# lambdaclass/lambdaworks_kzg

Hardware: AMD Instinct MI355X
Metric: blob_to_kzg_commitment ops/sec (4096-elem blobs) (higher is better)
Workload: dtype u32

## Files before the change

### lambdaworks_kzg_amd/csrc/direct.hip

```cpp
#include <stdlib.h>
#include <chrono>
#include "kernels.h"
#include "knobs.h"

namespace lwk {

template <int C>
struct DirectPlan {
    static constexpr int NW = (255 + C - 1) / C;
    static constexpr int H = 1 << (C - 1);
    static constexpr int WTOP = 255 - C * (NW - 1);
    static constexpr int HTOP = 1 << WTOP;
    static constexpr size_t TOP_BASE = (size_t)(NW - 1) * kBlobElems * H;
    static constexpr size_t ENTRIES = TOP_BASE + (size_t)kBlobElems * HTOP;
};

struct DirectPlanRt {
    int c, nw, wtop;
    uint32_t h, htop;
    size_t top_base, entries;
};

static DirectPlanRt make_plan(int bits) {
    DirectPlanRt p{};
    if (bits < kDirectMinBits || bits > kDirectMaxBits) return p;
    p.c = bits;
    p.nw = (255 + bits - 1) / bits;
    p.wtop = 255 - bits * (p.nw - 1);
    p.h = 1u << (bits - 1);
    p.htop = 1u << p.wtop;
    p.top_base = (size_t)(p.nw - 1) * kBlobElems * p.h;
    p.entries = p.top_base + (size_t)kBlobElems * p.htop;
    return p;
}

template <int C>
struct PlanOf {
    __host__ __device__ static constexpr DirectPlanRt get() {
        return DirectPlanRt{C, DirectPlan<C>::NW, DirectPlan<C>::WTOP, (uint32_t)DirectPlan<C>::H, (uint32_t)DirectPlan<C>::HTOP,
                            DirectPlan<C>::TOP_BASE, DirectPlan<C>::ENTRIES};
    }
};

size_t direct_table_entries(int bits) { return make_plan(bits).entries; }
int direct_num_windows(int bits) { return make_plan(bits).nw; }


__global__ __launch_bounds__(64) void k_direct_qbase(const G1Affine *__restrict__ points, G1Affine29 *__restrict__ qbase, int C,
                                                     int NW) {
    int i = blockIdx.x * blockDim.x + threadIdx.x;
    if (i >= kBlobElems) return;
    G1Affine29 a = affine_to_29(points[i]);
    qbase[i] = a;
    G1Xyzz29 cur = G1Xyzz29::from_affine(a.x, a.y);
    for (int j = 1; j < NW; j++) {
        for (int d = 0; d < C; d++) cur = xyzz_dbl(cur);
        qbase[(size_t)j * kBlobElems + i] = xyzz29_to_affine29(cur);
    }
}


constexpr int kChunk = 64;

__global__ __launch_bounds__(256) void k_direct_build(const G1Affine29 *__restrict__ qbase_win0, G1Affine29 *__restrict__ out_win0,
                                                      size_t n_pairs, F29<2> *__restrict__ scratch, size_t n_threads, int M,
                                                      size_t row_bytes) {
    const int K = M < kChunk ? M : kChunk;
    const size_t kChunksPerPair = (size_t)(M / K);
    const size_t gid = (size_t)blockIdx.x * blockDim.x + threadIdx.x;
    const size_t n_work = n_pairs * kChunksPerPair;
    auto slot = [&](int m, int f) -> F29<2> & { return scratch[((size_t)m * 5 + f) * n_threads + gid]; };
    for (size_t w = gid; w < n_work; w += n_threads) {
        const size_t pair = w / kChunksPerPair;
        const uint32_t s0 = (uint32_t)(w % kChunksPerPair) * K + 1;
        const G1Affine29 q = qbase_win0[pair];
        G1Xyzz29 cur = G1Xyzz29::infinity();
        for (int bit = 16; bit >= 0; bit--) {
            cur = xyzz_dbl(cur);
            if ((s0 >> bit) & 1) cur = xyzz_madd(cur, q.x, q.y);
        }
        F29<2> pref = F29<2>::one();
        const F29<1> one = F29<1>::one();
        for (int m = 0; m < K; m++) {
            F29<2> t = cur.zz * cur.zzz;
            pref = (m == 0) ? t : F29<2>(pref * t);
            slot(m, 0) = cur.x * one;
            slot(m, 1) = cur.y * one;
            slot(m, 2) = cur.zz;
            slot(m, 3) = cur.zzz;
            slot(m, 4) = pref;
            if (m < K - 1) cur = xyzz_madd(cur, q.x, q.y);
        }
        F29<2> inv = f29_inv(pref);
        char *rows = (char *)out_win0 + (pair * (size_t)M + (s0 - 1)) * row_bytes;
        for (int m = K - 1; m >= 0; m--) {
            F29<2> zz = slot(m, 2), zzz = slot(m, 3);
            F29<2> tinv = (m > 0) ? F29<2>(inv * slot(m - 1, 4)) : inv;
            inv = inv * (zz * zzz);
            G1Affine29 r;
            r.x = slot(m, 0) * (tinv * zzz);
            r.y = slot(m, 1) * (tinv * zz);
            *(G1Affine29 *)(rows + (size_t)m * row_bytes) = r;
        }
    }
}

static double wall_ms() {
    return std::chrono::duration<double, std::milli>(std::chrono::steady_clock::now().time_since_epoch()).count();
}

void free_direct_table(DirectTable &t) {
    for (int j = 0; j < kDirectMaxWindows; j++)
        if (t.win[j]) {
            hipFree(t.win[j]);
            t.win[j] = nullptr;
        }
    if (t.win_dev) hipFree(t.win_dev);
    t.win_dev = nullptr;
    t.nw = 0;
    t.bytes = 0;
}

hipError_t build_direct_table(int bits, const G1Affine *points, DirectTable &t, size_t row_bytes, hipStream_t st, double *ms, bool in_place) {
    const DirectPlanRt P = make_plan(bits);
    if (!P.entries || P.nw > kDirectMaxWindows) return hipErrorInvalidValue;
    if (in_place && (t.nw != P.nw || t.bytes != P.entries * row_bytes || !t.win_dev)) return hipErrorInvalidValue;
    if (!in_place) free_direct_table(t);
    G1Affine29 *qbase = nullptr;
    F29<2> *scratch = nullptr;
    const double t0 = wall_ms();
    const size_t n_threads = bits >= 14 ? 256 * 1024 : 64 * 1024;
    hipError_t e = hipMalloc((void **)&qbase, (size_t)P.nw * kBlobElems * sizeof(G1Affine29));
    if (e == hipSuccess) e = hipMalloc((void **)&scratch, (size_t)kChunk * 5 * n_threads * sizeof(F29<2>));
    if (e == hipSuccess && !in_place) e = hipMalloc((void **)&t.win_dev, kDirectMaxWindows * sizeof(uint64_t));
    const double t1 = wall_ms();
    double malloc_ms = 0, t_last_malloc = t1;
    if (e == hipSuccess) {
        {
            ProfScope p("k_direct_qbase", st);
            hipLaunchKernelGGL(k_direct_qbase, dim3(kBlobElems / 64), dim3(64), 0, st, points, qbase, P.c, P.nw);
        }
        for (int j = 0; j < P.nw && e == hipSuccess; j++) {
            const bool top = j == P.nw - 1;
            const size_t rows = (size_t)kBlobElems * (top ? P.htop : P.h);
            if (!in_place) {
                const double a0 = wall_ms();
                e = hipMalloc(&t.win[j], rows * row_bytes);
                t_last_malloc = wall_ms();
                malloc_ms += t_last_malloc - a0;
                if (e != hipSuccess) break;
                t.bytes += rows * row_bytes;
            }
            ProfScope p("k_direct_build", st);
            hipLaunchKernelGGL(k_direct_build, dim3((unsigned)(n_threads / 256)), dim3(256), 0, st, qbase + (size_t)j * kBlobElems,
                               (G1Affine29 *)t.win[j], (size_t)kBlobElems, scratch, n_threads, (int)(top ? P.htop : P.h), row_bytes);
        }
        if (e == hipSuccess && !in_place) {
            uint64_t h[kDirectMaxWindows] = {};
            for (int j = 0; j < P.nw; j++) h[j] = (uint64_t)(uintptr_t)t.win[j];
            e = hipMemcpyAsync(t.win_dev, h, sizeof h, hipMemcpyHostToDevice, st);
        }
        const hipError_t es = hipStreamSynchronize(st);
        if (e == hipSuccess) e = es;
    }
    const double t2 = wall_ms();
    if (qbase) hipFree(qbase);
    if (scratch) hipFree(scratch);
    if (e != hipSuccess) {
        free_direct_table(t);
    } else {
        t.nw = P.nw;
    }
    if (ms) {
        ms[0] = t1 - t0;
        ms[1] = malloc_ms;
        ms[2] = t2 - t_last_malloc;
        ms[3] = wall_ms() - t2;
    }
    return e;
}


#ifndef LWK_DIR_THREADS
#define LWK_DIR_THREADS 256
#endif
constexpr int kDirThreads = LWK_DIR_THREADS;

__device__ __forceinline__ G1Xyzz29 wave_fold(const G1Xyzz29 &in, int lane, int width = 64) {
    G1Xyzz29i s = *(const G1Xyzz29i *)&in;
    for (int d = width / 2; d >= 1; d >>= 1) {
        G1Xyzz29i other;
#pragma unroll
        for (int k = 0; k < 14; k++) {
            other.x.l[k] = __shfl_down(s.x.l[k], d, 64);
            other.y.l[k] = __shfl_down(s.y.l[k], d, 64);
            other.zz.l[k] = __shfl_down(s.zz.l[k], d, 64);
            other.zzz.l[k] = __shfl_down(s.zzz.l[k], d, 64);
        }
        if (lane < d) s = xyzz_add(s, other);
    }
    return *(G1Xyzz29 *)&s;
}

template <int CT>
__global__ __launch_bounds__(kDirThreads) void k_direct_accumulate(const uint64_t *__restrict__ win_dev,
                                                                   const uint4 *__restrict__ scalars,
                                                                   G1Xyzz29 *__restrict__ partials, int scalars_per_lane,
                                                                   DirectPlanRt rt, uint32_t row_bytes,
                                                                   const uint32_t *__restrict__ redo) {
    if (redo && !redo[blockIdx.y]) return;
    const DirectPlanRt P = CT ? PlanOf<CT ? CT : 16>::get() : rt;
    const int C = P.c;
    __shared__ uint32_t limbs[8 * kDirThreads];
    __shared__ G1Xyzz29 wave_sum[kDirThreads / 64];
    __shared__ uint64_t win_base[kDirectMaxWindows];
    if (threadIdx.x < kDirectMaxWindows) win_base[threadIdx.x] = win_dev[threadIdx.x];
    __syncthreads();
    const int tid = threadIdx.x, lane = tid & 63, wave = tid >> 6;
    const size_t blob = blockIdx.y;
    const int lanes_per_blob = gridDim.x * kDirThreads;
    const int first = blockIdx.x * kDirThreads + tid;
    const uint4 *sc = scalars + blob * (size_t)kBlobElems * 2;
    const int wper = (P.nw + (int)gridDim.z - 1) / (int)gridDim.z;
    const int w_lo = (int)blockIdx.z * wper, w_hi = w_lo + wper;

    int q = 0, j = 0;
    uint32_t carry = 0, point = 0;
    auto advance = [&](bool &valid, uint32_t &neg, G1Affine29i &row) {
        valid = false;
        while (q < scalars_per_lane) {
            if (j == 0) {
                point = (uint32_t)(first + q * lanes_per_blob);
                uint4 lo = sc[2 * point], hi = sc[2 * point + 1];
                limbs[0 * kDirThreads + tid] = lo.x; limbs[1 * kDirThreads + tid] = lo.y;
                limbs[2 * kDirThreads + tid] = lo.z; limbs[3 * kDirThreads + tid] = lo.w;
                limbs[4 * kDirThreads + tid] = hi.x; limbs[5 * kDirThreads + tid] = hi.y;
                limbs[6 * kDirThreads + tid] = hi.z; limbs[7 * kDirThreads + tid] = hi.w;
                carry = 0;
            }
            const int o = j * C, limb = o >> 5, sh = o & 31;
            uint32_t v = limbs[limb * kDirThreads + tid] >> sh;
            if (sh + C > 32 && limb + 1 < 8) v |= limbs[(limb + 1) * kDirThreads + tid] << (32 - sh);
            const bool top = j == P.nw - 1;
            uint32_t raw = (v & ((top ? (1u << P.wtop) : (1u << C)) - 1u)) + carry;
            uint32_t ng = (!top && raw > P.h) ? 1u : 0u;
            uint32_t mag = ng ? (1u << C) - raw : raw;
            carry = ng;
            const char *wbase = (const char *)(uintptr_t)win_base[j];
            const size_t idx = (size_t)point * (top ? P.htop : P.h) + (mag - 1);
            j++;
            if (j == P.nw) {
                j = 0;
                q++;
            }
            const int jw = (j == 0 ? P.nw : j) - 1;
            if (mag && jw >= w_lo && jw < w_hi) {
                valid = true;
                neg = ng;
                row = *(const G1Affine29i *)(wbase + idx * row_bytes);
                return;
            }
        }
    };

    G1Xyzz29i acc = G1Xyzz29i::infinity();
    bool cv;
    uint32_t cn;
    G1Affine29i cr;
    advance(cv, cn, cr);
    while (cv) {
        const auto qy = cneg(cr.y, cn != 0);
        xyzz_madd_split(acc, cr.x, qy, [&]() { advance(cv, cn, cr); });
    }

    G1Xyzz29 s = wave_fold(*(G1Xyzz29 *)&acc, lane);
    if (lane == 0) wave_sum[wave] = s;
    __syncthreads();
    if (wave == 0) {
        G1Xyzz29 t = lane < kDirThreads / 64 ? wave_sum[lane] : G1Xyzz29::infinity();
        t = wave_fold(t, lane, kDirThreads / 64);
        if (lane == 0) partials[(blob * gridDim.z + blockIdx.z) * gridDim.x + blockIdx.x] = t;
    }
}

constexpr int kLaneWords = 56;

__global__ __launch_bounds__(kDirThreads) void k_direct_accumulate_asm(const uint64_t *__restrict__ win_dev,
                                                                       const uint4 *__restrict__ scalars,
                                                                       uint32_t *__restrict__ lane_out, uint32_t *__restrict__ redo,
                                                                       int scalars_per_lane, DirectPlanRt rt, uint32_t row_bytes) {
#if defined(__HIP_DEVICE_COMPILE__)
    const uint32_t tid = threadIdx.x;
    const uint32_t first = blockIdx.x * blockDim.x + tid;
    const uint4 *sc = scalars + (size_t)blockIdx.y * kBlobElems * 2;
    uint32_t *out = lane_out + ((size_t)blockIdx.y * gridDim.x + blockIdx.x) * (size_t)(blockDim.x * kLaneWords);
    uint32_t *flag = redo + blockIdx.y;
    const uint32_t lanes_per_blob = gridDim.x * blockDim.x;
    asm volatile(
#include "direct_asm.inc"
        :
        : "s"(win_dev), "s"(sc), "s"(out), "s"(flag), "s"(scalars_per_lane), "s"(lanes_per_blob), "s"(rt.c), "s"(rt.nw), "s"(rt.wtop),
          "s"(rt.h), "s"(rt.htop), "s"(row_bytes), "v"(first), "v"(tid)
        :
#include "direct_asm_clobbers.inc"
    );
#endif
}


#ifdef LWK_FOLD_CALL
constexpr bool kFoldInl = false;
typedef G1Xyzz29 FoldPoint;
#else
constexpr bool kFoldInl = true;
typedef G1Xyzz29i FoldPoint;
#endif

__device__ __forceinline__ FoldPoint load_lane_sum(const uint32_t *src) {
    F29<25, kFoldInl, 1> nx;
    F29<17, kFoldInl, 1> ny, zz, zzz;
    FoldPoint acc;
    const uint4 *s4 = (const uint4 *)src;
    uint32_t wds[kLaneWords];
#pragma unroll
    for (int k = 0; k < kLaneWords / 4; k++) {
        uint4 t = s4[k];
        wds[4 * k] = t.x; wds[4 * k + 1] = t.y; wds[4 * k + 2] = t.z; wds[4 * k + 3] = t.w;
    }
#pragma unroll
    for (int i = 0; i < 14; i++) {
        nx.l[i] = wds[i];
        ny.l[i] = wds[14 + i];
        zz.l[i] = wds[28 + i];
        zzz.l[i] = wds[42 + i];
    }
    const F29<1, kFoldInl> one = F29<1, kFoldInl>::one();
    const bool inf = zz.is_literal_zero();
    acc.x = neg(nx) * one;
    acc.y = neg(ny) * one;
    acc.zz = zz * one;
    acc.zzz = zzz * one;
    if (inf) acc = FoldPoint::infinity();
    return acc;
}

__global__ __launch_bounds__(64) void k_direct_fold_lanes(const uint32_t *__restrict__ lane_out, G1Xyzz29 *__restrict__ partials,
                                                          const uint32_t *__restrict__ redo, int lanes_per_block, int blocks_per_blob) {
    const int unit = blockIdx.x;
    if (redo[unit / blocks_per_blob]) return;
    const int kFoldPerThread = lanes_per_block / 64;
    __builtin_amdgcn_s_setprio(2);
    const int lane = threadIdx.x;
    const uint32_t *src = lane_out + ((size_t)unit * lanes_per_block + lane) * (size_t)kLaneWords;
    FoldPoint acc = load_lane_sum(src);
#pragma unroll 1
    for (int step = 1; step < kFoldPerThread + 6; step++) {
        FoldPoint other;
        bool take = true;
        if (step < kFoldPerThread) {
            other = load_lane_sum(src + (size_t)step * 64 * kLaneWords);
        } else {
            const int d = 32 >> (step - kFoldPerThread);
#pragma unroll
            for (int k = 0; k < 14; k++) {
                other.x.l[k] = __shfl_down(acc.x.l[k], d, 64);
                other.y.l[k] = __shfl_down(acc.y.l[k], d, 64);
                other.zz.l[k] = __shfl_down(acc.zz.l[k], d, 64);
                other.zzz.l[k] = __shfl_down(acc.zzz.l[k], d, 64);
            }
            take = lane < d;
        }
        if (take) acc = xyzz_add(acc, other);
    }
    if (lane == 0) partials[unit] = *(G1Xyzz29 *)&acc;
}

__global__ __launch_bounds__(64) void k_direct_fold_lanes_asm(const uint32_t *__restrict__ lane_out, G1Xyzz29 *__restrict__ partials,
                                                              uint32_t *__restrict__ redo, int lanes_per_block, int blocks_per_blob) {
#if defined(__HIP_DEVICE_COMPILE__)
    const uint32_t unit = blockIdx.x;
    uint32_t *flag = redo + unit / blocks_per_blob;
    if (*flag) return;
    const uint32_t *src = lane_out + (size_t)unit * lanes_per_block * kLaneWords;
    G1Xyzz29 *out = partials + unit;
    const uint32_t per = lanes_per_block / 64, lane = threadIdx.x, levels = 6;
    asm volatile(
#include "direct_fold_asm.inc"
        :
        : "s"(src), "s"(out), "s"(flag), "s"(per), "v"(lane), "s"(levels)
        :
#include "direct_fold_asm_clobbers.inc"
    );
#endif
}

__global__ __launch_bounds__(64) void k_direct_fold_lanes_asm_alone(const uint32_t *__restrict__ lane_out, G1Xyzz29 *__restrict__ partials,
                                                                    uint32_t *__restrict__ redo, int lanes_per_block, int blocks_per_blob) {
#if defined(__HIP_DEVICE_COMPILE__)
    const uint32_t unit = blockIdx.x;
    uint32_t *flag = redo + unit / blocks_per_blob;
    if (*flag) return;
    const uint32_t *src = lane_out + (size_t)unit * lanes_per_block * kLaneWords;
    G1Xyzz29 *out = partials + unit;
    const uint32_t per = lanes_per_block / 64, lane = threadIdx.x, levels = 6;
    asm volatile(
#include "direct_fold_asm.inc"
        :
        : "s"(src), "s"(out), "s"(flag), "s"(per), "v"(lane), "s"(levels)
        :
#include "direct_fold_asm_clobbers_pad.inc"
    );
#endif
}

__global__ __launch_bounds__(64) void k_direct_fold(const G1Xyzz29 *__restrict__ partials, G1Xyzz29 *__restrict__ sums,
                                                    int per_blob) {
    const size_t b = blockIdx.x;
    const int lane = threadIdx.x;
    __builtin_amdgcn_s_setprio(2);
    G1Xyzz29 s = lane < per_blob ? partials[b * per_blob + lane] : G1Xyzz29::infinity();
    s = wave_fold(s, lane);
    if (lane == 0) sums[b] = s;
}

struct CoopParams {
    uint32_t k[8];
    uint32_t pack;
    uint32_t wtop, row_bytes, n0;
    uint32_t part_words, ctr_words;
};

constexpr uint32_t kCoopUnitWords = 56;

static void coop_geometry(const DirectPlanRt &P, int rpq, uint32_t &n0, uint32_t &units, uint32_t &counters) {
    const uint32_t groups = (uint32_t)((P.nw + rpq - 1) / rpq);
    n0 = kBlobElems * groups / 16;
    units = 0;
    counters = 0;
    for (uint32_t n = n0; n > 1; n = (n + 15) / 16) {
        units += n;
        counters += (n + 15) / 16;
    }
}

__global__ __launch_bounds__(256) void k_coop_msm_asm(const uint64_t *__restrict__ win_dev, const uint4 *__restrict__ scalars,
                                                     uint32_t *__restrict__ partials, uint32_t *__restrict__ counters,
                                                     G1Xyzz29 *__restrict__ sums, uint32_t *__restrict__ redo, CoopParams prm) {
#if defined(__HIP_DEVICE_COMPILE__)
    const uint32_t blob = blockIdx.y, lane = threadIdx.x & 63;
    const uint32_t unit = blockIdx.x * 4 + __builtin_amdgcn_readfirstlane(threadIdx.x >> 6);
    const uint4 *sc = scalars + (size_t)blob * kBlobElems * 2;
    uint32_t *part = partials + (size_t)blob * prm.part_words;
    uint32_t *ctr = counters + (size_t)blob * prm.ctr_words;
    G1Xyzz29 *out = sums + blob;
    uint32_t *flag = redo + blob;
    asm volatile(
#include "coop_asm.inc"
        :
        : "s"(win_dev), "s"(sc), "s"(part), "s"(ctr), "s"(out), "s"(flag), "s"(prm.k[0]), "s"(prm.k[1]), "s"(prm.k[2]), "s"(prm.k[3]),
          "s"(prm.k[4]), "s"(prm.k[5]), "s"(prm.k[6]), "s"(prm.k[7]), "s"(prm.pack), "s"(prm.wtop), "s"(prm.row_bytes), "s"(prm.n0), "s"(unit),
          "v"(lane)
        :
#include "coop_asm_clobbers.inc"
    );
#endif
}

static int coop_max_blobs() { return knobs().coop == 0 ? 0 : knobs().coop_max; }
static int coop_rows_per_quad(int nw, size_t n_blobs) {
    const int env = knobs().coop_rpq < 0 ? 0 : knobs().coop_rpq > 32 ? 32 : knobs().coop_rpq;
    if (env) return env;
    const int groups = n_blobs >= 4 ? 1 : (int)(4 / n_blobs);
    return (nw + groups - 1) / groups;
}

static bool direct_asm_enabled() { return knobs().direct_asm; }

template <int CT>
static void launch_direct_t(const DirectPlanRt &plan, const uint64_t *table, size_t row_bytes, const uint32_t *scalars_raw,
                            G1Xyzz29 *lane_scratch, G1Xyzz29 *partials, uint32_t *redo, G1Xyzz29 *sums, size_t n_blobs, hipStream_t st,
                            int fill, uint32_t *redo_flag_out) {
    const int kFillEnv = knobs().direct_fill;
    const int kFill = kFillEnv ? kFillEnv : fill ? fill : 512;
    CoopParams prm{};
    const int rpq = coop_rows_per_quad(plan.nw, n_blobs ? n_blobs : 1);
    uint32_t units = 0, counters = 0;
    coop_geometry(plan, rpq, prm.n0, units, counters);
    const bool coop_fits = units <= (uint32_t)kBlobElems && 1 + counters <= (uint32_t)kNumBuckets + 1;
    if ((int)n_blobs <= coop_max_blobs() && !fill && coop_fits) {
        for (int j = 0; j + 1 < plan.nw; j++) {
            const int bit = plan.c * j;
            const uint64_t v = (uint64_t)(plan.h - 1) << (bit & 31);
            uint64_t carry = v;
            for (int w = bit >> 5; w < 8 && carry; w++) {
                carry += prm.k[w];
                prm.k[w] = (uint32_t)carry;
                carry >>= 32;
            }
        }
        prm.pack = (uint32_t)plan.c | ((uint32_t)plan.nw << 8) | ((uint32_t)rpq << 16) | (12u << 24);
        prm.wtop = (uint32_t)plan.wtop;
        prm.row_bytes = (uint32_t)row_bytes;
        prm.part_words = units * kCoopUnitWords;
        prm.ctr_words = counters;
        uint32_t *ctr = redo + n_blobs;
        if (redo_flag_out) {
            ProfScope p("k_coop_msm_asm", st);
            hipLaunchKernelGGL(k_coop_msm_asm, dim3(prm.n0 / 4, (unsigned)n_blobs), dim3(256), 0, st, table, (const uint4 *)scalars_raw,
                               (uint32_t *)lane_scratch, ctr, sums, redo_flag_out, prm);
            return;
        }
        hipMemsetAsync(redo, 0, n_blobs * (1 + (size_t)counters) * sizeof(uint32_t), st);
        {
            ProfScope p("k_coop_msm_asm", st);
            hipLaunchKernelGGL(k_coop_msm_asm, dim3(prm.n0 / 4, (unsigned)n_blobs), dim3(256), 0, st, table, (const uint4 *)scalars_raw,
                               (uint32_t *)lane_scratch, ctr, sums, redo, prm);
        }
        {
            ProfScope p("k_direct_redo", st);
            hipLaunchKernelGGL(k_direct_accumulate<CT>, dim3(1, (unsigned)n_blobs, 1), dim3(kDirThreads), 0, st, table,
                               (const uint4 *)scalars_raw, sums, kBlobElems / kDirThreads, plan, (uint32_t)row_bytes, (const uint32_t *)redo);
        }
        return;
    }
    int blocks_per_blob = 1, wsplit = 1;
    while (blocks_per_blob < 16 && n_blobs * blocks_per_blob < (size_t)kFill) blocks_per_blob <<= 1;
    while (wsplit < 4 && n_blobs * blocks_per_blob * wsplit * 8 <= (size_t)kFill) wsplit <<= 1;
    const int scalars_per_lane = kBlobElems / (kDirThreads * blocks_per_blob);
    const int parts = blocks_per_blob * wsplit;
    G1Xyzz29 *dest = parts == 1 ? sums : partials;
    if (direct_asm_enabled() && wsplit == 1) {
        const int threads = kDirThreads;
        hipMemsetAsync(redo, 0, n_blobs * sizeof(uint32_t), st);
        {
            ProfScope p("k_direct_accumulate_asm", st);
            hipLaunchKernelGGL(k_direct_accumulate_asm, dim3(blocks_per_blob, (unsigned)n_blobs), dim3(threads), 0, st, table,
                               (const uint4 *)scalars_raw, (uint32_t *)lane_scratch, redo, kBlobElems / (threads * blocks_per_blob), plan,
                               (uint32_t)row_bytes);
        }
        {
            ProfScope p("k_direct_fold_lanes", st);
            const int n_units = (int)n_blobs * blocks_per_blob;
            const bool fold_asm = knobs().fold_asm;
            if (fold_asm) {
                if (n_units >= 1024 && !fill)
                    hipLaunchKernelGGL(k_direct_fold_lanes_asm_alone, dim3((unsigned)n_units), dim3(64), 0, st, (const uint32_t *)lane_scratch,
                                       dest, redo, threads, blocks_per_blob);
                else
                    hipLaunchKernelGGL(k_direct_fold_lanes_asm, dim3((unsigned)n_units), dim3(64), 0, st, (const uint32_t *)lane_scratch, dest,
                                       redo, threads, blocks_per_blob);
            } else {
                hipLaunchKernelGGL(k_direct_fold_lanes, dim3((unsigned)n_units), dim3(64), 0, st, (const uint32_t *)lane_scratch, dest,
                                   (const uint32_t *)redo, threads, blocks_per_blob);
            }
        }
        {
            ProfScope p("k_direct_redo", st);
            hipLaunchKernelGGL(k_direct_accumulate<CT>, dim3(blocks_per_blob, (unsigned)n_blobs, 1), dim3(kDirThreads), 0, st, table,
                               (const uint4 *)scalars_raw, dest, scalars_per_lane, plan, (uint32_t)row_bytes, (const uint32_t *)redo);
        }
    } else {
        ProfScope p("k_direct_accumulate", st);
        hipLaunchKernelGGL(k_direct_accumulate<CT>, dim3(blocks_per_blob, (unsigned)n_blobs, wsplit), dim3(kDirThreads), 0, st,
                           table, (const uint4 *)scalars_raw, dest, scalars_per_lane, plan, (uint32_t)row_bytes, (const uint32_t *)nullptr);
    }
    if (parts > 1) {
        ProfScope p("k_direct_fold", st);
        hipLaunchKernelGGL(k_direct_fold, dim3((unsigned)n_blobs), dim3(64), 0, st, partials, sums, parts);
    }
}

void launch_direct_msm(int bits, const uint64_t *table, size_t row_bytes, const uint32_t *scalars_raw, G1Xyzz29 *lane_scratch,
                       G1Xyzz29 *partials, uint32_t *redo, G1Xyzz29 *sums, size_t n_blobs, hipStream_t st, int fill, uint32_t *redo_flag_out) {
    const DirectPlanRt plan = make_plan(bits);
    if (!plan.entries) return;
    switch (bits) {
        case 14: launch_direct_t<14>(plan, table, row_bytes, scalars_raw, lane_scratch, partials, redo, sums, n_blobs, st, fill, redo_flag_out); break;
        case 15: launch_direct_t<15>(plan, table, row_bytes, scalars_raw, lane_scratch, partials, redo, sums, n_blobs, st, fill, redo_flag_out); break;
        case 16: launch_direct_t<16>(plan, table, row_bytes, scalars_raw, lane_scratch, partials, redo, sums, n_blobs, st, fill, redo_flag_out); break;
        default: launch_direct_t<0>(plan, table, row_bytes, scalars_raw, lane_scratch, partials, redo, sums, n_blobs, st, fill, redo_flag_out); break;
    }
}
uint32_t direct_one_blob_counter_words(int bits) {
    const DirectPlanRt plan = make_plan(bits);
    if (!plan.entries || coop_max_blobs() < 1) return 0;
    CoopParams prm{};
    uint32_t units = 0, counters = 0;
    coop_geometry(plan, coop_rows_per_quad(plan.nw, 1), prm.n0, units, counters);
    if (!(units <= (uint32_t)kBlobElems && 1 + counters <= (uint32_t)kNumBuckets + 1)) return 0;
    return counters;
}
template <int CT>
static void launch_direct_only_t(const DirectPlanRt &plan, const uint64_t *table, size_t row_bytes, const uint32_t *scalars_raw, G1Xyzz29 *sums,
                                 const uint32_t *only_if, size_t n_blobs, hipStream_t st) {
    ProfScope p("k_direct_redo", st);
    hipLaunchKernelGGL(k_direct_accumulate<CT>, dim3(1, (unsigned)n_blobs, 1), dim3(kDirThreads), 0, st, table, (const uint4 *)scalars_raw, sums,
                       kBlobElems / kDirThreads, plan, (uint32_t)row_bytes, only_if);
}

void launch_direct_msm_only(int bits, const uint64_t *table, size_t row_bytes, const uint32_t *scalars_raw, G1Xyzz29 *sums, const uint32_t *only_if,
                            size_t n_blobs, hipStream_t st) {
    const DirectPlanRt plan = make_plan(bits);
    if (!plan.entries) return;
    switch (bits) {
        case 14: launch_direct_only_t<14>(plan, table, row_bytes, scalars_raw, sums, only_if, n_blobs, st); break;
        case 15: launch_direct_only_t<15>(plan, table, row_bytes, scalars_raw, sums, only_if, n_blobs, st); break;
        case 16: launch_direct_only_t<16>(plan, table, row_bytes, scalars_raw, sums, only_if, n_blobs, st); break;
        default: launch_direct_only_t<0>(plan, table, row_bytes, scalars_raw, sums, only_if, n_blobs, st); break;
    }
}

}
```

### lambdaworks_kzg_amd/csrc/engine.h

```cpp
#pragma once
#include <hip/hip_runtime.h>
#include <atomic>
#include <condition_variable>
#include <deque>
#include <functional>
#include <mutex>
#include <string>
#include <thread>
#include <vector>
#include "../../include/lambdaworks_kzg_amd.h"
#include "kernels.h"
#include "front.h"

namespace lwk {

constexpr uint64_t kCtxMagic = 0x4c574b5a47414d44ull;
constexpr size_t kMaxChunk = 1024;
static_assert(kMaxChunk == kPlanMaxChunk, "plan.h plans in the engine's chunks");
constexpr int kMaxSplit = 8;

void set_error(const char *fmt, ...);
const char *get_error();

#define LWK_HIP(expr)                                                                         \
    do {                                                                                      \
        hipError_t _e = (expr);                                                               \
        if (_e != hipSuccess) {                                                               \
            lwk::set_error("%s failed: %s (%s:%d)", #expr, hipGetErrorString(_e), __FILE__, __LINE__); \
            return C_KZG_ERROR;                                                               \
        }                                                                                     \
    } while (0)

struct SideWorker;
SideWorker *side_worker_acquire();
void side_worker_run(SideWorker *w, std::function<void()> fn);
void side_worker_wait(SideWorker *w);
bool side_workers_on();
struct SideTask {
    SideWorker *w = nullptr;
    std::thread t;
    SideTask() = default;
    template <class F>
    explicit SideTask(F &&f) { start(static_cast<F &&>(f)); }
    template <class F>
    void start(F &&f) {
        join();
        if (!side_workers_on()) {
            try {
                t = std::thread(f);
            } catch (...) {
                f();
            }
            return;
        }
        w = side_worker_acquire();
        if (w) side_worker_run(w, std::function<void()>(f));
        else f();
    }
    void join() {
        if (w) side_worker_wait(w);
        w = nullptr;
        if (t.joinable()) t.join();
    }
    ~SideTask() { join(); }
    SideTask(const SideTask &) = delete;
    SideTask &operator=(const SideTask &) = delete;
};

struct Workspace {
    size_t cap = 0;
    uint8_t *blobs = nullptr;
    uint32_t *scalars = nullptr;
    uint32_t *scalars2 = nullptr;
    Fr *fr = nullptr;
    uint32_t *sorted = nullptr;
    uint32_t *bucket_start = nullptr;
    uint32_t *perm = nullptr;
    G1Xyzz29 *buckets = nullptr;
    G1Xyzz29 *sums = nullptr;
    uint8_t *out48 = nullptr;
    uint8_t *comm48 = nullptr;
    uint8_t *canon48 = nullptr;
    uint8_t *zbytes = nullptr;
    uint8_t *ybytes = nullptr;
    Fr *z = nullptr;
    int32_t *status = nullptr;
    G1Affine29 *val_pts = nullptr;
    int32_t *val_kind = nullptr;
    uint32_t *val_verdict = nullptr;
    size_t long_cap = 0;
    Fr *z_long = nullptr;
    uint8_t *canon_long = nullptr;
    int32_t *status_long = nullptr;
    G1Affine29 *val_pts_long = nullptr;
    int32_t *val_kind_long = nullptr;
    uint32_t *val_verdict_long = nullptr;
};

constexpr size_t kVerifyApartMax = 8192;
struct VerifyBuffers {
    G1Affine29 *pts_c = nullptr, *pts_p = nullptr;
    G1Affine29 *mult_c = nullptr, *mult_p = nullptr;
    int32_t *kind_c = nullptr, *kind_p = nullptr;
    uint8_t *proof_in = nullptr;
    uint8_t *comm_in = nullptr, *canon_dev = nullptr;
    int32_t *status_all = nullptr;
    uint32_t *verdict_c = nullptr, *verdict_p = nullptr;
    uint8_t *d_r = nullptr, *d_rz = nullptr, *d_aff = nullptr;
    G1Xyzz29 *d_part = nullptr;
    int32_t *d_inf = nullptr;
    uint8_t *vm_base = nullptr;
    G1Affine29 *tab_p = nullptr, *tab_c = nullptr;
    G1Xyzz29 *vm_tmp = nullptr, *vm_partial = nullptr, *vm_bsum = nullptr;
    F29<2> *vm_pre = nullptr;
    uint32_t *sc_a = nullptr, *sc_b = nullptr;
    Fr *vm_pw = nullptr;
    uint8_t *d_rec = nullptr;
    uint8_t *h_rec = nullptr;
    size_t rec_cap = 0;
    uint8_t *h_pin = nullptr;
    hipEvent_t vm_done = nullptr;
    std::vector<G1Affine29> h_aff;
    std::vector<int32_t> h_kind;
    std::unique_lock<std::mutex> hold;
    bool owned = false;
};
void verify_buffers_free(VerifyBuffers &v);

size_t host_small_batch_limit();
int64_t host_last_active_ns();
int64_t host_now_ns();
void host_pool_warm();

constexpr int kCombineLanes = 2;
constexpr size_t kCombineSlots = 128;
constexpr size_t kCombineMaxBatch = 64;

struct CombineReq {
    enum State { QUEUED, TAKEN, DONE };
    int slot = -1;
    int mode = 0;
    uint8_t *out48 = nullptr;
    int rc = C_KZG_OK;
    State state = QUEUED;
};

struct Combiner {
    LaneFront<CombineReq, kCombineLanes> front;
    std::mutex init_m;
    uint8_t *pinned_blobs = nullptr;
    uint8_t *pinned_out[kCombineLanes] = {nullptr, nullptr};
    int32_t *pinned_status[kCombineLanes] = {nullptr, nullptr};
    bool ready = false, failed = false;
};

struct ProofReq {
    enum State { QUEUED, TAKEN, DONE };
    const uint8_t *blob = nullptr, *second = nullptr;
    uint8_t *out = nullptr, *y_out = nullptr;
    int mode = 0;
    int rc = C_KZG_OK;
    State state = QUEUED;
};
typedef LeaderFront<ProofReq> ProofFront;

struct BuildTiming {
    int bits = 0;
    size_t row_bytes = 0, table_bytes = 0;
    double free_old_ms = 0, table_malloc_ms = 0, scratch_malloc_ms = 0, kernels_ms = 0, scratch_free_ms = 0, total_ms = 0;
    bool in_place = false;
};
struct LoadTiming {
    double context_ms = 0;
    double points_and_tables_ms = 0;
    double g2_and_fft_ms = 0;
    double default_table_ms = 0;
    double total_ms = 0;
};

struct SmallProofHost {
    uint8_t *blobs = nullptr, *comm = nullptr, *canon = nullptr, *dig = nullptr;
    int32_t *code = nullptr;
    size_t cap = 0;
    static constexpr int kChunks = 16;
    hipEvent_t chunk_done[kChunks] = {};
    hipEvent_t hashed[kChunks] = {};
};

struct LagrangeForm {
    bool ready = false;
    G1Affine *points = nullptr;
    G1Affine29 *table = nullptr;
    G1Affine29 *direct_table = nullptr;
    DirectTable direct_tab;
    int direct_bits = 0;
    size_t direct_row_bytes = 0;
};

struct DevStage {
    uint8_t *slot[2] = {nullptr, nullptr};
    hipEvent_t copied[2] = {nullptr, nullptr}, parsed[2] = {nullptr, nullptr};
    bool ready = false, failed = false;
};

struct Ctx {
    FFTSettings fs;
    uint64_t magic;
    uint64_t generation = 0;
    int device;
    hipStream_t stream;
    hipStream_t vstream;
    hipStream_t aux[kMaxSplit];
    hipEvent_t ev_fork, ev_join[kMaxSplit];
    hipEvent_t ws_done;
    hipStream_t ws_last;
    std::atomic<bool> ws_recorded{false};
    hipEvent_t lane_done[kCombineLanes];
    Combiner comb;
    ProofFront blob_proof_front, point_proof_front;
    std::atomic<Ctx *> twin{nullptr};
    bool is_twin = false;
    std::atomic<bool> reserved{false};
    Ctx *primary = nullptr;
    hipEvent_t heavy_done = nullptr;
    std::mutex heavy_mu;
    G1Affine *points;
    G1Affine29 *table;
    G1Affine29 *direct_table;
    DirectTable direct_tab;
    int direct_bits;
    size_t direct_row_bytes;
    LagrangeForm lag;
    std::atomic<bool> lag_ready{false};
    bool lag_failed = false;
    Fr *tw_fwd, *tw_inv;
    Fr28 *tw28_fwd, *tw28_inv;
    Workspace ws;
    SmallProofHost sph;
    DevStage stage;
    uint8_t *one_pin = nullptr;
    hipStream_t prio_copy = nullptr;
    uint8_t *vblobs = nullptr;
    size_t vblobs_cap = 0;
    uint8_t *host_res = nullptr;
    size_t host_res_cap = 0;
    void *each_lines = nullptr;
    uint8_t *each_buf = nullptr;
    size_t each_cap = 0;
    VerifyBuffers vs;
    size_t vs_cap;
    std::mutex verify_mu;
    std::mutex mu;
    std::atomic<int> mode_override{-1};
    BuildTiming last_build;
    LoadTiming load_timing;
};

struct WsUse {
    Ctx *c;
    hipStream_t st;
    WsUse(Ctx *c_, hipStream_t st_) : c(c_), st(st_) {
        if (c->ws_last != st) hipStreamWaitEvent(st, c->ws_done, 0);
        for (int k = 0; k < kCombineLanes; k++) hipStreamWaitEvent(st, c->lane_done[k], 0);
    }
    ~WsUse() {
        hipEventRecord(c->ws_done, st);
        c->ws_last = st;
        c->ws_recorded.store(true, std::memory_order_release);
    }
};

Ctx *ctx_of(const KZGSettings *s);
bool ctx_is_live(const Ctx *c, uint64_t gen);

int mode_of(const KZGSettings *s);

C_KZG_RET ctx_reserve(Ctx *c, size_t n);
C_KZG_RET map_rc(C_KZG_RET rc, int mode);
void ensure_lagrange(Ctx *c, int mode);

void msm_stages(Ctx *c, const uint32_t *scalars_raw, uint8_t *out48, size_t n, hipStream_t st, size_t base = 0, bool shared_chip = false,
                bool lagrange = false);
bool coefficients_to_msm_form(Ctx *c, int mode, size_t n, hipStream_t st, size_t base = 0);

C_KZG_RET commit_batch_device(Ctx *c, uint8_t *out48, const uint8_t *blobs, size_t n, int mode, hipStream_t st,
                              int32_t *status);
C_KZG_RET blob_proof_batch_device(Ctx *c, uint8_t *out48, const uint8_t *blobs, const uint8_t *comm48, size_t n, int mode,
                                  hipStream_t st, int32_t *status);
C_KZG_RET point_proof_batch_device(Ctx *c, uint8_t *proof48, uint8_t *y32, const uint8_t *blobs, const uint8_t *z32,
                                   size_t n, int mode, hipStream_t st, int32_t *status, const G1Xyzz29 **sums_out = nullptr);
C_KZG_RET msm_scalars_raw_device(Ctx *c, uint8_t *out48, const uint32_t *scalars_raw, size_t n, hipStream_t st);

C_KZG_RET verify_prepare_host(Ctx *c, const uint8_t *blobs, const uint8_t *comm48, const uint8_t *proofs48, size_t n,
                              int mode, uint8_t *z32, uint8_t *y32, uint8_t *canon_c, uint8_t *canon_p, VerifyBuffers &vb,
                              const uint8_t *trusted_canon_c = nullptr);
C_KZG_RET verify_prepare_device(Ctx *c, const uint8_t *d_blobs, const uint8_t *d_comm, const uint8_t *d_proofs, size_t n, int mode,
                                uint8_t *z32, uint8_t *y32, uint8_t *canon_c, uint8_t *canon_p, VerifyBuffers &vb, hipStream_t caller,
                                uint8_t *records_out = nullptr, bool keep = false);
C_KZG_RET verify_openings_prepare_device(Ctx *c, const uint8_t *d_comm, const uint8_t *d_proofs, const uint8_t *d_z, const uint8_t *d_y,
                                         size_t n, int mode, VerifyBuffers &vb);
C_KZG_RET lincomb3_device_host(Ctx *c, VerifyBuffers &vb, const uint8_t *sc_r, const uint8_t *sc_rz, size_t n,
                               uint8_t sums[3][96], int infs[3]);
bool vmsm_ready(const VerifyBuffers &vb);
C_KZG_RET vmsm_begin(Ctx *c, VerifyBuffers &vb, const Fr *pw33, int le, size_t n);
C_KZG_RET vmsm_finish(Ctx *c, VerifyBuffers &vb, uint8_t sums[3][96], int infs[3]);

int host_validate_commitment(const uint8_t in48[48], uint8_t canon48[48], G1Affine29 *aff = nullptr);
void host_validate_commitments(const uint8_t *in48, uint8_t *canon48, int *rc, size_t n, G1Affine29 *aff = nullptr);

bool g2_fill_values(g2_t *out65, const uint8_t *g2_bytes, size_t n2);

}
```

### lambdaworks_kzg_amd/csrc/engine.hip

```cpp
#include "engine.h"
#include "knobs.h"
#include "hostfp.h"

#include <stdarg.h>
#include <stdio.h>
#include <stdlib.h>
#include <string.h>

#include <atomic>
#include <chrono>
#include <map>
#include <set>
#include <thread>
#include <vector>

namespace lwk {


static thread_local char g_err[512] = "";

void set_error(const char *fmt, ...) {
    va_list ap;
    va_start(ap, fmt);
    vsnprintf(g_err, sizeof g_err, fmt, ap);
    va_end(ap);
    if (knobs().verbose) fprintf(stderr, "[lambdaworks_kzg_amd] %s\n", g_err);
}
const char *get_error() { return g_err; }


struct ProfRec {
    const char *name;
    hipEvent_t e0, e1;
};
static std::atomic<bool> g_prof_on{false};
static std::mutex g_prof_mu;
static std::vector<ProfRec> g_prof_pending;
struct ProfAgg {
    uint64_t launches = 0;
    double total_ms = 0;
};
static std::map<std::string, ProfAgg> g_prof_agg;

ProfScope::ProfScope(const char *n, hipStream_t s) : name(n), st(s), e0(nullptr), e1(nullptr), on(g_prof_on.load(std::memory_order_relaxed)) {
    if (!on) return;
    if (hipEventCreate(&e0) != hipSuccess || hipEventCreate(&e1) != hipSuccess) {
        on = false;
        return;
    }
    hipEventRecord(e0, st);
}
ProfScope::~ProfScope() {
    if (!on) return;
    hipEventRecord(e1, st);
    std::lock_guard<std::mutex> lk(g_prof_mu);
    g_prof_pending.push_back({name, e0, e1});
}

static void prof_drain() {
    std::lock_guard<std::mutex> lk(g_prof_mu);
    for (auto &r : g_prof_pending) {
        float ms = 0;
        if (hipEventSynchronize(r.e1) == hipSuccess && hipEventElapsedTime(&ms, r.e0, r.e1) == hipSuccess) {
            auto &a = g_prof_agg[r.name];
            a.launches++;
            a.total_ms += ms;
        }
        hipEventDestroy(r.e0);
        hipEventDestroy(r.e1);
    }
    g_prof_pending.clear();
}


static std::mutex g_reg_mu;
struct RegEntry {
    Ctx *ctx;
    uint64_t digest;
};
static std::map<const void *, RegEntry> g_registry;
static std::set<const void *> g_live_fs;
static std::atomic<int> g_default_device{0};
thread_local int tl_device_override = -1;

static uint64_t g1_values_digest(const g1_t *g1) {
    uint64_t h = 0xcbf29ce484222325ull;
    const uint8_t *a = (const uint8_t *)&g1[0], *b = (const uint8_t *)&g1[kBlobElems - 1];
    for (size_t i = 0; i < sizeof(g1_t); i++) h = (h ^ a[i]) * 0x100000001b3ull;
    for (size_t i = 0; i < sizeof(g1_t); i++) h = (h ^ b[i]) * 0x100000001b3ull;
    return h;
}

static bool peer_busy(const Ctx *c) {
    const Ctx *p = c->is_twin ? c->primary : c->primary->twin.load(std::memory_order_acquire);
    if (!p || !p->ws_recorded.load(std::memory_order_acquire)) return false;
    const bool busy = hipEventQuery(p->ws_done) != hipSuccess;
    (void)hipGetLastError();
    return busy;
}

struct WsLaneUse {
    Ctx *c;
    int lane;
    WsLaneUse(Ctx *c_, int lane_) : c(c_), lane(lane_) { hipStreamWaitEvent(c->aux[lane], c->ws_done, 0); }
    ~WsLaneUse() {
        hipEventRecord(c->lane_done[lane], c->aux[lane]);
        c->ws_last = nullptr;
    }
};

static C_KZG_RET dev_alloc(void **p, size_t bytes) {
    LWK_HIP(hipMalloc(p, bytes));
    return C_KZG_OK;
}

template <class T>
static void dev_free(T *&p) {
    if (p) hipFree(p);
    p = nullptr;
}

static void ws_free(Workspace &w) {
    dev_free(w.blobs);
    dev_free(w.scalars);
    dev_free(w.scalars2);
    dev_free(w.fr);
    dev_free(w.sorted);
    dev_free(w.bucket_start);
    dev_free(w.perm);
    dev_free(w.buckets);
    dev_free(w.sums);
    dev_free(w.out48);
    dev_free(w.comm48);
    dev_free(w.canon48);
    dev_free(w.zbytes);
    dev_free(w.ybytes);
    dev_free(w.z);
    dev_free(w.status);
    dev_free(w.val_pts);
    dev_free(w.val_kind);
    dev_free(w.val_verdict);
    w.cap = 0;
}

static void ws_long_free(Workspace &w) {
    dev_free(w.z_long);
    dev_free(w.canon_long);
    dev_free(w.status_long);
    w.long_cap = 0;
    dev_free(w.val_pts_long);
    dev_free(w.val_kind_long);
    dev_free(w.val_verdict_long);
}

C_KZG_RET ctx_reserve(Ctx *c, size_t n) {
    if (n > kMaxChunk) n = kMaxChunk;
    if (n == 0) n = 1;
    Workspace &w = c->ws;
    if (w.cap >= n) return C_KZG_OK;
    LWK_HIP(hipSetDevice(c->device));
    LWK_HIP(hipDeviceSynchronize());
    ws_free(w);
    size_t cap = 1;
    while (cap < n) cap <<= 1;
    C_KZG_RET rc;
#define WS_ALLOC(field, bytes)                                  \
    if ((rc = dev_alloc((void **)&w.field, (bytes))) != C_KZG_OK) { \
        ws_free(w);                                             \
        return C_KZG_MALLOC;                                    \
    }
    WS_ALLOC(blobs, cap * (size_t)kBlobBytes);
    WS_ALLOC(scalars, cap * (size_t)kBlobBytes);
    WS_ALLOC(scalars2, cap * (size_t)kBlobBytes);
    WS_ALLOC(fr, cap * (size_t)kBlobBytes);
    WS_ALLOC(sorted, cap * (size_t)kMaxEntries * 4);
    WS_ALLOC(bucket_start, cap * (size_t)(kNumBuckets + 1) * 4);
    WS_ALLOC(perm, cap * (size_t)(kNumBuckets + 1) * 4);
    WS_ALLOC(buckets, cap * (size_t)kNumBuckets * sizeof(G1Xyzz29));
    WS_ALLOC(sums, (cap + 1) * sizeof(G1Xyzz29));
    WS_ALLOC(out48, cap * 48);
    WS_ALLOC(comm48, cap * 48);
    WS_ALLOC(canon48, cap * 48);
    WS_ALLOC(zbytes, cap * 32);
    WS_ALLOC(ybytes, cap * 32);
    WS_ALLOC(z, cap * sizeof(Fr));
    WS_ALLOC(status, cap * 4);
    WS_ALLOC(val_pts, cap * sizeof(G1Affine29));
    WS_ALLOC(val_kind, cap * 4);
    WS_ALLOC(val_verdict, cap * 4);
#undef WS_ALLOC
    w.cap = cap;
    return C_KZG_OK;
}

static void vs_free(Ctx *c);
void direct_from_env(const KZGSettings *s);

static void sph_free(SmallProofHost &h) {
    if (h.blobs) hipHostFree(h.blobs);
    if (h.comm) hipHostFree(h.comm);
    if (h.canon) hipHostFree(h.canon);
    if (h.dig) hipHostFree(h.dig);
    if (h.code) hipHostFree(h.code);
    for (hipEvent_t e : h.chunk_done)
        if (e) hipEventDestroy(e);
    for (hipEvent_t e : h.hashed)
        if (e) hipEventDestroy(e);
    h = SmallProofHost();
}

static std::atomic<int> g_last_proof_schedule{-1};
static size_t small_proof_host_limit() {
    const size_t x = knobs().small_proof_host;
    return x > kMaxChunk ? kMaxChunk : x;
}

static bool sph_reserve(Ctx *c, size_t n, bool at_reserve = false) {
    SmallProofHost &h = c->sph;
    if (h.cap >= n) return true;
    if (!at_reserve && c->primary->reserved.load(std::memory_order_acquire)) return false;
    hipDeviceSynchronize();
    sph_free(h);
    size_t cap = 16;
    while (cap < n) cap <<= 1;
    const bool ok = hipHostMalloc((void **)&h.blobs, cap * (size_t)kBlobBytes) == hipSuccess && hipHostMalloc((void **)&h.comm, cap * 48) == hipSuccess &&
                    hipHostMalloc((void **)&h.canon, cap * 48) == hipSuccess && hipHostMalloc((void **)&h.dig, cap * 32) == hipSuccess &&
                    hipHostMalloc((void **)&h.code, cap * 4) == hipSuccess;
    bool ev_ok = ok;
    for (int k = 0; ev_ok && k < SmallProofHost::kChunks; k++)
        ev_ok = hipEventCreateWithFlags(&h.chunk_done[k], hipEventDisableTiming) == hipSuccess &&
                hipEventCreateWithFlags(&h.hashed[k], hipEventDisableTiming) == hipSuccess;
    if (!ev_ok) {
        (void)hipGetLastError();
        sph_free(h);
        return false;
    }
    h.cap = cap;
    return true;
}

static size_t mid_proof_chunks() {
    const size_t x = knobs().mid_proof_chunks;
    return x < 1 ? 1 : x > (size_t)SmallProofHost::kChunks ? (size_t)SmallProofHost::kChunks : x;
}
static size_t mid_proof_host_limit() {
    const size_t x = knobs().mid_proof_host;
    return x > kMaxChunk ? kMaxChunk : x;
}

static PlanKnobs plan_knobs() {
    PlanKnobs k;
    k.small_proof_host = small_proof_host_limit();
    k.mid_proof_host = mid_proof_host_limit();
    k.mid_proof_chunks = mid_proof_chunks();
    k.mid_proof_pipe = knobs().mid_proof_pipe;
    k.mid_proof_pipe_min = knobs().mid_proof_pipe_min;
    k.mid_proof_parts = knobs().mid_proof_parts;
    k.heavy_serial = knobs().heavy_serial;
    return k;
}

static std::atomic<int64_t> g_wake_requested_ns{0};
static void host_warm_fn(void *);
static bool host_assist_warm() {
    const int64_t window_ns = (int64_t)(knobs().host_warm_ms < 0 ? 0 : knobs().host_warm_ms) * 1000000;
    const int64_t last = host_last_active_ns(), woken = g_wake_requested_ns.load(std::memory_order_acquire), now = host_now_ns();
    return (last != 0 && now - last <= window_ns) || (woken != 0 && now - woken <= window_ns);
}
static void launch_host_wake(Ctx *c) {
    g_wake_requested_ns.store(host_now_ns(), std::memory_order_release);
    if (hipLaunchHostFunc(c->aux[1], host_warm_fn, nullptr) != hipSuccess) (void)hipGetLastError();
}
static void host_warm_fn(void *) {
    try {
        host_pool_warm();
    } catch (...) {
    }
}

struct ChunkHashArgs {
    SmallProofHost *h;
    size_t first, count;
};
static void chunk_midstate_host_fn(void *p) {
    ChunkHashArgs *a = (ChunkHashArgs *)p;
    SmallProofHost &h = *a->h;
    try {
        challenge_midstates_host((uint32_t *)(h.dig + 32 * a->first), h.blobs + a->first * (size_t)kBlobBytes, a->count);
    } catch (...) {
        memset(h.dig + 32 * a->first, 0, 32 * a->count);
    }
    delete a;
}
static void chunk_hash_host_fn(void *p) {
    ChunkHashArgs *a = (ChunkHashArgs *)p;
    SmallProofHost &h = *a->h;
    try {
        challenge_digests_host(h.dig + 32 * a->first, h.blobs + a->first * (size_t)kBlobBytes, h.comm + 48 * a->first, a->count);
    } catch (...) {
        memset(h.dig + 32 * a->first, 0, 32 * a->count);
    }
    delete a;
}

static C_KZG_RET chunk_host_functions(Ctx *c, const uint8_t *blobs, size_t n, hipStream_t sc, hipStream_t sf, hipStream_t join,
                                      void (*fn)(void *), const char *prof_name, bool record_hashed = false) {
    SmallProofHost &h = c->sph;
    const size_t per = (n + mid_proof_chunks() - 1) / mid_proof_chunks();
    std::vector<ChunkHashArgs *> args;
    for (size_t first = 0; first < n; first += per) {
        ChunkHashArgs *a = new (std::nothrow) ChunkHashArgs{&h, first, n - first < per ? n - first : per};
        if (!a) {
            for (ChunkHashArgs *b : args) delete b;
            return C_KZG_MALLOC;
        }
        args.push_back(a);
    }
    for (size_t k = 0; k < args.size(); k++) {
        const size_t first = args[k]->first, cnt = args[k]->count;
        hipError_t e = hipMemcpyAsync(h.blobs + first * (size_t)kBlobBytes, blobs + first * (size_t)kBlobBytes, cnt * (size_t)kBlobBytes,
                                      hipMemcpyDeviceToHost, sc);
        if (e == hipSuccess) e = hipEventRecord(h.chunk_done[k], sc);
        if (e == hipSuccess) e = hipStreamWaitEvent(sf, h.chunk_done[k], 0);
        bool queued = false;
        if (e == hipSuccess) {
            ProfScope p(prof_name, sf);
            e = hipLaunchHostFunc(sf, fn, args[k]);
            queued = e == hipSuccess;
        }
        if (e == hipSuccess && record_hashed) e = hipEventRecord(h.hashed[k], sf);
        if (e != hipSuccess) {
            for (size_t j = queued ? k + 1 : k; j < args.size(); j++) delete args[j];
            set_error("host-assisted challenge: %s", hipGetErrorString(e));
            (void)hipGetLastError();
            if (hipEventRecord(c->ev_join[kMaxSplit - 2], sc) == hipSuccess) hipStreamWaitEvent(join, c->ev_join[kMaxSplit - 2], 0);
            if (sf != join && hipEventRecord(c->ev_join[kMaxSplit - 3], sf) == hipSuccess) hipStreamWaitEvent(join, c->ev_join[kMaxSplit - 3], 0);
            return C_KZG_ERROR;
        }
    }
    return C_KZG_OK;
}

struct SmallProofArgs {
    SmallProofHost *h;
    size_t n;
    int32_t bad;
};

static void small_proof_host_fn(void *p) {
    SmallProofArgs *a = (SmallProofArgs *)p;
    SmallProofHost &h = *a->h;
    try {
        challenge_digests_host(h.dig, h.blobs, h.comm, a->n);
        std::vector<int> vrc(a->n);
        host_validate_commitments(h.comm, h.canon, vrc.data(), a->n);
        for (size_t i = 0; i < a->n; i++) h.code[i] = vrc[i] == 2 ? a->bad : 0;
    } catch (...) {
        for (size_t i = 0; i < a->n; i++) h.code[i] = kStatusError;
    }
    delete a;
}


static void ctx_destroy(Ctx *c) {
    if (!c) return;
    hipSetDevice(c->device);
    hipDeviceSynchronize();
    if (Ctx *t = c->twin.load(std::memory_order_acquire)) {
        ctx_destroy(t);
        c->twin.store(nullptr, std::memory_order_release);
    }
    ws_free(c->ws);
// ... 6 lines not shown
        c->direct_tab = DirectTable();
        c->lag = LagrangeForm();
        c->tw_fwd = c->tw_inv = nullptr;
        c->tw28_fwd = c->tw28_inv = nullptr;
    }
    dev_free(c->points);
    dev_free(c->table);
    free_direct_table(c->direct_tab);
    c->direct_table = nullptr;
    free_direct_table(c->lag.direct_tab);
    dev_free(c->lag.points);
    dev_free(c->lag.table);
    dev_free(c->tw_fwd);
    dev_free(c->tw_inv);
    dev_free(c->tw28_fwd);
    dev_free(c->tw28_inv);
    if (c->stream) hipStreamDestroy(c->stream);
    if (c->vstream) hipStreamDestroy(c->vstream);
    for (int k = 0; k < kMaxSplit; k++) {
        if (c->aux[k]) hipStreamDestroy(c->aux[k]);
        if (c->ev_join[k]) hipEventDestroy(c->ev_join[k]);
    }
    if (c->ev_fork) hipEventDestroy(c->ev_fork);
    if (c->ws_done) hipEventDestroy(c->ws_done);
    if (c->heavy_done) hipEventDestroy(c->heavy_done);
    for (int k = 0; k < kCombineLanes; k++) {
        if (c->lane_done[k]) hipEventDestroy(c->lane_done[k]);
        if (c->comb.pinned_out[k]) hipHostFree(c->comb.pinned_out[k]);
        if (c->comb.pinned_status[k]) hipHostFree(c->comb.pinned_status[k]);
    }
    if (c->comb.pinned_blobs) hipHostFree(c->comb.pinned_blobs);
    dev_free(c->host_res);
    dev_free(c->vblobs);
    dev_free(c->each_lines);
    dev_free(c->each_buf);
    if (c->prio_copy) hipStreamDestroy(c->prio_copy);
    if (c->one_pin) hipHostFree(c->one_pin);
    for (int k = 0; k < 2; k++) {
        dev_free(c->stage.slot[k]);
        if (c->stage.copied[k]) hipEventDestroy(c->stage.copied[k]);
        if (c->stage.parsed[k]) hipEventDestroy(c->stage.parsed[k]);
    }
    sph_free(c->sph);
    free(c->fs.expanded_roots_of_unity);
    free(c->fs.reverse_roots_of_unity);
    free(c->fs.roots_of_unity);
    c->magic = 0;
    {
        std::lock_guard<std::mutex> lk(g_reg_mu);
        g_live_fs.erase((const void *)c);
    }
    delete c;
}

static bool gpu_available() {
    int n = 0;
    if (hipGetDeviceCount(&n) != hipSuccess || n <= 0) {
        set_error("no HIP device available: this library has no CPU fallback (hipGetDeviceCount)");
        return false;
    }
    return true;
}

static void fr_raw_to_blst(blst_fr *o, const uint32_t raw[8]) {
    for (int k = 0; k < 4; k++) o->l[3 - k] = (uint64_t)raw[2 * k] | ((uint64_t)raw[2 * k + 1] << 32);
}

static C_KZG_RET ctx_new(Ctx **out, const Ctx *twin_of = nullptr) {
    if (!gpu_available()) return C_KZG_ERROR;
    Ctx *c = new Ctx();
    memset(&c->fs, 0, sizeof c->fs);
    c->magic = kCtxMagic;
    c->device = twin_of ? twin_of->device : tl_device_override >= 0 ? tl_device_override : g_default_device.load();
    c->is_twin = twin_of != nullptr;
    c->primary = twin_of ? const_cast<Ctx *>(twin_of) : c;
    c->stream = nullptr;
    c->ws_done = nullptr;
    c->ws_last = nullptr;
    for (int k = 0; k < kCombineLanes; k++) c->lane_done[k] = nullptr;
    c->vstream = nullptr;
    c->ev_fork = nullptr;
    for (int k = 0; k < kMaxSplit; k++) {
        c->aux[k] = nullptr;
        c->ev_join[k] = nullptr;
    }
    c->points = nullptr;
    c->table = nullptr;
    c->direct_table = nullptr;
    c->direct_bits = 0;
    c->direct_row_bytes = kDirectRowPacked;
    c->vs_cap = 0;
    c->tw_fwd = c->tw_inv = nullptr;
    c->tw28_fwd = c->tw28_inv = nullptr;
    hipError_t e = hipSetDevice(c->device);
    if (e == hipSuccess) e = hipStreamCreate(&c->stream);
    if (e == hipSuccess) e = hipStreamCreateWithFlags(&c->vstream, hipStreamNonBlocking);
    if (e == hipSuccess) e = hipEventCreateWithFlags(&c->ev_fork, hipEventDisableTiming);
    if (e == hipSuccess) e = hipEventCreateWithFlags(&c->ws_done, hipEventDisableTiming);
    if (e == hipSuccess && !twin_of) e = hipEventCreateWithFlags(&c->heavy_done, hipEventDisableTiming);
    for (int k = 0; k < kCombineLanes && e == hipSuccess; k++) e = hipEventCreateWithFlags(&c->lane_done[k], hipEventDisableTiming);
    for (int k = 0; k < kMaxSplit && e == hipSuccess; k++) {
        e = hipStreamCreateWithFlags(&c->aux[k], hipStreamNonBlocking);
        if (e == hipSuccess) e = hipEventCreateWithFlags(&c->ev_join[k], hipEventDisableTiming);
    }
    if (twin_of) {
        c->points = twin_of->points;
        c->table = twin_of->table;
        c->direct_table = twin_of->direct_table;
        c->direct_tab.win_dev = twin_of->direct_tab.win_dev;
        c->direct_bits = twin_of->direct_bits;
        c->direct_row_bytes = twin_of->direct_row_bytes;
        c->lag = twin_of->lag;
        c->lag.direct_tab = DirectTable();
        c->lag.direct_tab.win_dev = twin_of->lag.direct_tab.win_dev;
        c->tw_fwd = twin_of->tw_fwd;
        c->tw_inv = twin_of->tw_inv;
        c->tw28_fwd = twin_of->tw28_fwd;
        c->tw28_inv = twin_of->tw28_inv;
    } else {
        if (e == hipSuccess) e = hipMalloc((void **)&c->points, (size_t)kBlobElems * sizeof(G1Affine));
        if (e == hipSuccess) e = hipMalloc((void **)&c->table, (size_t)kTablePoints * sizeof(G1Affine29));
        if (e == hipSuccess) e = hipMalloc((void **)&c->tw_fwd, (size_t)(kBlobElems / 2) * sizeof(Fr));
        if (e == hipSuccess) e = hipMalloc((void **)&c->tw_inv, (size_t)(kBlobElems / 2) * sizeof(Fr));
        if (e == hipSuccess) e = hipMalloc((void **)&c->tw28_fwd, (size_t)(kBlobElems / 2 + kBlobElems) * sizeof(Fr28));
        if (e == hipSuccess) e = hipMalloc((void **)&c->tw28_inv, (size_t)(kBlobElems / 2) * sizeof(Fr28));
    }
    if (e != hipSuccess) {
        set_error("device context allocation failed: %s", hipGetErrorString(e));
        ctx_destroy(c);
        return C_KZG_MALLOC;
    }
    static std::atomic<uint64_t> next_generation{1};
    c->generation = next_generation.fetch_add(1);
    if (!twin_of) {
        std::lock_guard<std::mutex> lk(g_reg_mu);
        g_live_fs.insert((const void *)c);
    }
    *out = c;
    return C_KZG_OK;
}

static bool twin_off() {
    return !knobs().twin;
}

static Ctx *pick_ctx(Ctx *c, hipStream_t st) {
    if (twin_off() || !st || st == c->stream) return c;
    std::lock_guard<std::mutex> lk(c->mu);
    if (c->ws_last == st || c->ws_last == nullptr || hipEventQuery(c->ws_done) == hipSuccess) {
        (void)hipGetLastError();
        return c;
    }
    (void)hipGetLastError();
    if (!c->twin.load(std::memory_order_acquire)) {
        Ctx *t = nullptr;
        if (ctx_new(&t, c) != C_KZG_OK) return c;
        c->twin.store(t, std::memory_order_release);
    }
    return c->twin.load(std::memory_order_acquire);
}

static C_KZG_RET ctx_finish_fft(Ctx *c) {
    launch_build_twiddles(c->tw_fwd, c->tw_inv, c->stream);
    launch_twiddles_to28(c->tw_fwd, c->tw28_fwd, c->stream);
    launch_twiddles_to28(c->tw_inv, c->tw28_inv, c->stream);
    launch_roots_brp28(c->tw28_fwd, c->tw28_fwd + kBlobElems / 2, c->stream);
    const int n = kBlobElems;
    std::vector<Fr> h_f(n / 2), h_i(n / 2);
    LWK_HIP(hipMemcpyAsync(h_f.data(), c->tw_fwd, (n / 2) * sizeof(Fr), hipMemcpyDeviceToHost, c->stream));
    LWK_HIP(hipMemcpyAsync(h_i.data(), c->tw_inv, (n / 2) * sizeof(Fr), hipMemcpyDeviceToHost, c->stream));
    LWK_HIP(hipStreamSynchronize(c->stream));
    c->fs.max_width = n;
    c->fs.expanded_roots_of_unity = (fr_t *)calloc(n + 1, sizeof(fr_t));
    c->fs.reverse_roots_of_unity = (fr_t *)calloc(n + 1, sizeof(fr_t));
    c->fs.roots_of_unity = (fr_t *)calloc(n, sizeof(fr_t));
    if (!c->fs.expanded_roots_of_unity || !c->fs.reverse_roots_of_unity || !c->fs.roots_of_unity) return C_KZG_MALLOC;
    for (int k = 0; k <= n; k++) {
        int kk = k % n;
        Fr f = h_f[kk % (n / 2)], b = h_i[kk % (n / 2)];
        if (kk >= n / 2) {
            f = neg(f);
            b = neg(b);
        }
        uint32_t raw[8];
        fe_to_raw<FrParams>(raw, f);
        fr_raw_to_blst(&c->fs.expanded_roots_of_unity[k], raw);
        fe_to_raw<FrParams>(raw, b);
        fr_raw_to_blst(&c->fs.reverse_roots_of_unity[k], raw);
    }
    for (int k = 0; k < n; k++) {
        unsigned r = 0;
        for (int b = 0; b < 12; b++) r |= ((k >> b) & 1u) << (11 - b);
        c->fs.roots_of_unity[k] = c->fs.expanded_roots_of_unity[r];
    }
    return C_KZG_OK;
}

bool ctx_is_live(const Ctx *c, uint64_t gen) {
    std::lock_guard<std::mutex> lk(g_reg_mu);
    return c && g_live_fs.count((const void *)c) && c->generation == gen;
}

Ctx *ctx_of(const KZGSettings *s) {
    if (!s) {
        set_error("KZGSettings pointer is NULL");
        return nullptr;
    }
    if (s->fs) {
        std::lock_guard<std::mutex> lk(g_reg_mu);
        if (g_live_fs.count((const void *)s->fs)) return (Ctx *)s->fs;
    }
    if (!s->g1_values) {
        set_error("KZGSettings has neither an engine context nor g1_values");
        return nullptr;
    }
    const uint64_t digest = g1_values_digest(s->g1_values);
    Ctx *stale = nullptr;
    {
        std::lock_guard<std::mutex> lk(g_reg_mu);
        auto it = g_registry.find(s->g1_values);
        if (it != g_registry.end()) {
            if (it->second.digest == digest) return it->second.ctx;
            stale = it->second.ctx;
            g_registry.erase(it);
        }
    }
    if (stale) ctx_destroy(stale);
    Ctx *c = nullptr;
    if (ctx_new(&c) != C_KZG_OK) return nullptr;
    uint64_t *d_blst = nullptr;
    int32_t *d_status = nullptr;
    std::vector<int32_t> h_status(kBlobElems);
    bool ok = hipMalloc((void **)&d_blst, (size_t)kBlobElems * 144) == hipSuccess &&
              hipMalloc((void **)&d_status, (size_t)kBlobElems * 4) == hipSuccess &&
              hipMemcpyAsync(d_blst, s->g1_values, (size_t)kBlobElems * 144, hipMemcpyHostToDevice, c->stream) == hipSuccess;
    if (ok) {
        launch_g1_from_blst(d_blst, c->points, d_status, kBlobElems, c->stream);
        launch_build_table(c->points, c->table, c->stream);
        ok = hipMemcpyAsync(h_status.data(), d_status, (size_t)kBlobElems * 4, hipMemcpyDeviceToHost, c->stream) == hipSuccess &&
             hipStreamSynchronize(c->stream) == hipSuccess;
    }
    if (d_blst) hipFree(d_blst);
    if (d_status) hipFree(d_status);
    if (ok)
        for (int i = 0; i < kBlobElems; i++)
            if (h_status[i] != 0) {
                set_error("g1_values[%d] is not a point on the curve", i);
                ok = false;
                break;
            }
    if (ok) ok = ctx_finish_fft(c) == C_KZG_OK;
    if (!ok) {
        if (!get_error()[0]) set_error("building a device context from g1_values failed");
        ctx_destroy(c);
        return nullptr;
    }
    bool ours = true;
    {
        std::lock_guard<std::mutex> lk(g_reg_mu);
        auto it = g_registry.find(s->g1_values);
        if (it != g_registry.end()) {
            Ctx *first = it->second.ctx;
            if (it->second.digest == digest) {
                stale = c;
                c = first;
                ours = false;
            } else {
                stale = first;
                it->second = {c, digest};
            }
        } else {
            stale = nullptr;
            g_registry[s->g1_values] = {c, digest};
        }
    }
    if (stale) ctx_destroy(stale);
    if (ours) direct_from_env(s);
    return c;
}


static G1Xyzz29 *msm_sums_stage(Ctx *c, const uint32_t *scalars_raw, size_t n, hipStream_t st, size_t base = 0, bool shared_chip = false,
                                bool lagrange = false, G1Xyzz29 *sums_out = nullptr, uint32_t *redo_flag_out = nullptr) {
    Workspace &w = c->ws;
    uint32_t *sorted = w.sorted + base * (size_t)kMaxEntries;
    uint32_t *bstart = w.bucket_start + base * (size_t)(kNumBuckets + 1);
    uint32_t *perm = w.perm + base * (size_t)(kNumBuckets + 1);
    G1Xyzz29 *buckets = w.buckets + base * (size_t)kNumBuckets;
    G1Xyzz29 *sums = sums_out ? sums_out : w.sums + base;
    const G1Affine29 *direct = lagrange ? c->lag.direct_table : c->direct_table;
    if (direct) {
        launch_direct_msm(lagrange ? c->lag.direct_bits : c->direct_bits, lagrange ? c->lag.direct_tab.win_dev : c->direct_tab.win_dev,
                          lagrange ? c->lag.direct_row_bytes : c->direct_row_bytes, scalars_raw, buckets, (G1Xyzz29 *)sorted, bstart, sums, n,
                          st, (shared_chip || peer_busy(c)) ? 2048 : 0, redo_flag_out);
        return sums;
    }
    launch_digit_sort(scalars_raw, sorted, bstart, perm, n, st);
    launch_bucket_accumulate(lagrange ? c->lag.table : c->table, sorted, bstart, perm, buckets, n, st);
    launch_bucket_reduce(buckets, sums, n, st);
    return sums;
}

void msm_stages(Ctx *c, const uint32_t *scalars_raw, uint8_t *out48, size_t n, hipStream_t st, size_t base, bool shared_chip,
                bool lagrange) {
    launch_finalize_compress(msm_sums_stage(c, scalars_raw, n, st, base, shared_chip, lagrange), out48, n, st);
}

static size_t host_finish_limit() {
    const size_t x = knobs().host_finish;
    return x > kCombineMaxBatch ? kCombineMaxBatch : x;
}

static HFp hfp_from_limbs28(const uint32_t *l) {
    uint64_t w[7] = {0, 0, 0, 0, 0, 0, 0};
    for (int i = 0; i < 14; i++) {
        const int bit = P29::W * i, k = bit >> 6, sh = bit & 63;
        unsigned __int128 v = (unsigned __int128)l[i] << sh;
        for (int j = k; j < 7 && v; j++) {
            v += w[j];
            w[j] = (uint64_t)v;
            v >>= 64;
        }
    }
    for (int shift = 16; shift >= 0; shift--) {
        uint64_t kp[7], d[7];
        for (int j = 0; j < 7; j++) {
            const uint64_t lo = j < 6 ? HFpPar::P[j] : 0, below = j > 0 ? HFpPar::P[j - 1] : 0;
            kp[j] = shift ? (lo << shift) | (below >> (64 - shift)) : lo;
        }
        unsigned __int128 br = 0;
        for (int j = 0; j < 7; j++) {
            const unsigned __int128 v = (unsigned __int128)w[j] - kp[j] - (uint64_t)br;
            d[j] = (uint64_t)v;
            br = (v >> 64) & 1;
        }
        if (!br)
            for (int j = 0; j < 7; j++) w[j] = d[j];
    }
    HFp r;
    for (int j = 0; j < 6; j++) r.l[j] = w[j];
    return r;
}

static void host_finish_compress(uint8_t out[48], const G1Xyzz29 &sum) {
    if (sum.is_inf()) {
        memset(out, 0, 48);
        out[0] = 0xc0;
        return;
    }
    const HFp X = hfp_from_limbs28(sum.x.l), Y = hfp_from_limbs28(sum.y.l), ZZ = hfp_from_limbs28(sum.zz.l), ZZZ = hfp_from_limbs28(sum.zzz.l);
    const HFp i = inv(ZZ * ZZZ);
    G1Affine a;
    a.x = (X * (i * ZZZ)).to_fe();
    a.y = (Y * (i * ZZ)).to_fe();
    g1_compress_affine(out, a);
}

static bool commit_on_lagrange(const Ctx *c, int mode) {
    return mode == LWKZG_MODE_CKZG && c->lag.ready && (c->lag.direct_table || !c->direct_table);
}
static bool proof_on_lagrange(const Ctx *c, int mode) {
    return mode == LWKZG_MODE_CKZG && c->lag.ready && c->lag.direct_table && !c->direct_table;
}
static bool proof_in_evaluation_form(const Ctx *c, int mode) {
    return knobs().ckzg_eval_proofs && mode == LWKZG_MODE_CKZG && c->lag.ready && (c->lag.direct_table || !c->direct_table);
}
static void quotient_stage(Ctx *c, int mode, const uint32_t *in, const Fr *z, uint32_t *quot, uint8_t *y_out, int le, size_t n, hipStream_t st,
                           const uint32_t *only_if = nullptr) {
    if (proof_in_evaluation_form(c, mode)) launch_eval_quotient_evalform(in, z, c->tw28_fwd + kBlobElems / 2, quot, y_out, le, n, st, only_if);
    else launch_eval_quotient(in, z, quot, y_out, le, n, st, only_if);
}
static bool quotient_to_msm_form(Ctx *c, int mode, size_t n, hipStream_t st, size_t base = 0) {
    if (proof_in_evaluation_form(c, mode)) return true;
    return coefficients_to_msm_form(c, mode, n, st, base);
}
bool coefficients_to_msm_form(Ctx *c, int mode, size_t n, hipStream_t st, size_t base) {
    if (!proof_on_lagrange(c, mode)) return false;
    Workspace &w = c->ws;
    const size_t so = base * (size_t)kBlobElems;
    launch_coefficients_to_evaluations(w.scalars2 + so * 8, w.fr + so, (Fr *)(w.scalars + so * 8), c->tw28_fwd, n, st);
    return true;
}

static bool coefficients_stage(Ctx *c, const uint8_t *blobs, size_t n, int mode, int32_t *status, hipStream_t st,
                               size_t base = 0, bool evaluations_ok = false, uint32_t *zero = nullptr, uint32_t zero_words = 0) {
    Workspace &w = c->ws;
    uint32_t *scalars = w.scalars + base * (size_t)kBlobElems * 8;
    if (mode == LWKZG_MODE_REFERENCE) {
        launch_parse_be_reduce(blobs, scalars, n * kBlobElems, st, zero, zero_words);
    } else if (evaluations_ok ? commit_on_lagrange(c, mode) : proof_in_evaluation_form(c, mode)) {
        launch_copy_le_check(blobs, scalars, status, n, st);
        return true;
    } else {
        launch_blob_evaluations_to_coefficients(blobs, scalars, c->tw28_inv, status, n, st);
    }
    return false;
}

static int split_ways(bool direct) {
    const int v = knobs().split < 0 ? 0 : knobs().split > kMaxSplit ? kMaxSplit : knobs().split;
    return v ? v : (direct ? 1 : 2);
}

C_KZG_RET msm_scalars_raw_device(Ctx *c, uint8_t *out48, const uint32_t *scalars_raw, size_t n, hipStream_t st) {
    for (size_t off = 0; off < n; off += kMaxChunk) {
        size_t m = n - off < kMaxChunk ? n - off : kMaxChunk;
        msm_stages(c, scalars_raw + off * (size_t)kBlobElems * 8, out48 + 48 * off, m, st);
    }
    return C_KZG_OK;
}

C_KZG_RET commit_batch_device(Ctx *c, uint8_t *out48, const uint8_t *blobs, size_t n, int mode, hipStream_t st,
                              int32_t *status) {
    C_KZG_RET rc = ctx_reserve(c, n);
    if (rc != C_KZG_OK) return rc;
    for (size_t off = 0; off < n; off += kMaxChunk) {
        size_t m = n - off < kMaxChunk ? n - off : kMaxChunk;
        int32_t *stt = status ? status + off : c->ws.status;
        LWK_HIP(hipMemsetAsync(stt, 0, m * 4, st));
        const int ways = m >= 256 ? split_ways((commit_on_lagrange(c, mode) ? c->lag.direct_table : c->direct_table) != nullptr) : 1;
        if (ways == 1) {
            const bool lg = coefficients_stage(c, blobs + off * (size_t)kBlobBytes, m, mode, stt, st, 0, true);
            msm_stages(c, c->ws.scalars, out48 + 48 * off, m, st, 0, false, lg);
            continue;
        }
        LWK_HIP(hipEventRecord(c->ev_fork, st));
        for (int k = 0; k < ways; k++) {
            size_t lo = m * k / ways, hi = m * (k + 1) / ways;
            hipStream_t sk = c->aux[k];
            LWK_HIP(hipStreamWaitEvent(sk, c->ev_fork, 0));
            const bool lg = coefficients_stage(c, blobs + (off + lo) * (size_t)kBlobBytes, hi - lo, mode, stt + lo, sk, lo, true);
            msm_stages(c, c->ws.scalars + lo * (size_t)kBlobElems * 8, out48 + 48 * (off + lo), hi - lo, sk, lo, false, lg);
            LWK_HIP(hipEventRecord(c->ev_join[k], sk));
            LWK_HIP(hipStreamWaitEvent(st, c->ev_join[k], 0));
        }
    }
    return C_KZG_OK;
}

static C_KZG_RET ws_long_reserve(Ctx *c, size_t n) {
    Workspace &w = c->ws;
    if (w.long_cap >= n) return C_KZG_OK;
    LWK_HIP(hipDeviceSynchronize());
    ws_long_free(w);
    size_t cap = 2 * kMaxChunk;
    while (cap < n) cap <<= 1;
    if (hipMalloc((void **)&w.z_long, cap * sizeof(Fr)) != hipSuccess || hipMalloc((void **)&w.canon_long, cap * 48) != hipSuccess ||
        hipMalloc((void **)&w.status_long, cap * 4) != hipSuccess || hipMalloc((void **)&w.val_pts_long, cap * sizeof(G1Affine29)) != hipSuccess ||
        hipMalloc((void **)&w.val_kind_long, cap * 4) != hipSuccess || hipMalloc((void **)&w.val_verdict_long, cap * 4) != hipSuccess) {
        (void)hipGetLastError();
        ws_long_free(w);
        set_error("proof batch of %zu blobs: out of device memory for the challenges", n);
        return C_KZG_MALLOC;
    }
    w.long_cap = cap;
    return C_KZG_OK;
}

C_KZG_RET blob_proof_batch_device(Ctx *c, uint8_t *out48, const uint8_t *blobs, const uint8_t *comm48, size_t n, int mode,
                                  hipStream_t st, int32_t *status) {
    C_KZG_RET rc = ctx_reserve(c, n);
    if (rc != C_KZG_OK) return rc;
    const bool longcall = n > kMaxChunk;
    if (longcall) {
        rc = ws_long_reserve(c, n);
        if (rc != C_KZG_OK) return rc;
    }
    Workspace &w = c->ws;
    const int le = mode == LWKZG_MODE_CKZG;
    int32_t *stt = status ? status : longcall ? w.status_long : w.status;
    Fr *z = longcall ? w.z_long : w.z;
    uint8_t *canon = longcall ? w.canon_long : w.canon48;
    LWK_HIP(hipMemsetAsync(stt, 0, n * 4, st));
    const bool evf = proof_in_evaluation_form(c, mode);
    const bool msm_direct = evf ? c->lag.direct_table != nullptr : c->direct_table && !proof_on_lagrange(c, mode);
    const bool warm = host_assist_warm(), busy = peer_busy(c);
    const PlanKnobs pk = plan_knobs();
    ProofPlan plan = plan_proof_call(n, warm, busy, msm_direct, true, pk);
    const int forced = knobs().proof_schedule;
    if (forced >= 0 && forced <= kProofGpuChains && n <= kMaxChunk) {
        PlanKnobs fk = pk;
        fk.small_proof_host = forced == kProofSmallHost ? kMaxChunk : 0;
        fk.mid_proof_host = forced == kProofSmallHost || forced == kProofGpuChains ? 0 : kMaxChunk;
        fk.mid_proof_pipe = forced == kProofMidPiped;
        fk.mid_proof_pipe_min = 0;
        plan = plan_proof_call(n, forced != kProofMidCold, false, forced == kProofMidPiped ? msm_direct : false, true, fk);
    }
    SmallProofArgs *host_args = nullptr;
    if (plan.needs_staging()) {
        bool ok = sph_reserve(c, n);
        if (ok && plan.schedule == kProofSmallHost) {
            host_args = new (std::nothrow) SmallProofArgs{&c->sph, n, le ? kStatusBadArgs : kStatusError};
            ok = host_args != nullptr;
        }
        if (!ok) plan = plan_proof_call(n, warm, busy, msm_direct, false, pk);
    }
    g_last_proof_schedule.store((int)plan.schedule, std::memory_order_relaxed);
    const bool piped = plan.schedule == kProofMidPiped;
    switch (plan.schedule) {
    case kProofSmallHost: {
        SmallProofHost &h = c->sph;
        LWK_HIP(hipMemcpyAsync(h.blobs, blobs, n * (size_t)kBlobBytes, hipMemcpyDeviceToHost, st));
        LWK_HIP(hipMemcpyAsync(h.comm, comm48, n * 48, hipMemcpyDeviceToHost, st));
        {
            ProfScope p("host_challenge_and_validate", st);
            hipError_t e = hipLaunchHostFunc(st, small_proof_host_fn, host_args);
            if (e != hipSuccess) {
                delete host_args;
                set_error("hipLaunchHostFunc failed: %s", hipGetErrorString(e));
                return C_KZG_ERROR;
            }
        }
        LWK_HIP(hipMemcpyAsync(stt, h.code, n * 4, hipMemcpyHostToDevice, st));
        LWK_HIP(hipMemcpyAsync(w.zbytes, h.dig, n * 32, hipMemcpyHostToDevice, st));
        LWK_HIP(hipMemcpyAsync(canon, h.canon, n * 48, hipMemcpyHostToDevice, st));
        launch_z_from_bytes(w.zbytes, z, nullptr, le, n, st);
        launch_challenge(blobs, canon, z, le, n, st, comm48);
        break;
    }
    case kProofMidCold: {
        LWK_HIP(hipEventRecord(c->ev_fork, st));
        LWK_HIP(hipStreamWaitEvent(c->vstream, c->ev_fork, 0));
        launch_validate_commitments(comm48, canon, stt, le ? kStatusBadArgs : kStatusError, n, c->vstream, longcall ? w.val_pts_long : w.val_pts,
                                    longcall ? w.val_kind_long : w.val_kind, longcall ? w.val_verdict_long : w.val_verdict);
        LWK_HIP(hipEventRecord(c->ev_join[0], c->vstream));
        launch_host_wake(c);
        launch_challenge(blobs, comm48, z, le, n, st);
        LWK_HIP(hipStreamWaitEvent(st, c->ev_join[0], 0));
        launch_challenge(blobs, canon, z, le, n, st, comm48);
        break;
    }
    case kProofMidHost:
    case kProofMidPiped: {
        SmallProofHost &h = c->sph;
        hipStream_t sc = c->aux[0], sh = c->aux[1];
        const size_t chunks = plan.chunks;
        LWK_HIP(hipEventRecord(c->ev_fork, st));
        LWK_HIP(hipStreamWaitEvent(c->vstream, c->ev_fork, 0));
        LWK_HIP(hipStreamWaitEvent(sc, c->ev_fork, 0));
        if (piped) LWK_HIP(hipStreamWaitEvent(sh, c->ev_fork, 0));
        launch_validate_commitments(comm48, canon, stt, le ? kStatusBadArgs : kStatusError, n, c->vstream, longcall ? w.val_pts_long : w.val_pts,
                                    longcall ? w.val_kind_long : w.val_kind, longcall ? w.val_verdict_long : w.val_verdict);
        LWK_HIP(hipEventRecord(c->ev_join[0], c->vstream));
        LWK_HIP(hipMemcpyAsync(h.comm, comm48, n * 48, hipMemcpyDeviceToHost, sc));
        {
            const C_KZG_RET rch = chunk_host_functions(c, blobs, n, sc, piped ? sh : st, st, chunk_hash_host_fn, "host_challenge_chunk", piped);
            if (rch != C_KZG_OK) {
                hipStreamWaitEvent(st, c->ev_join[0], 0);
                return rch;
            }
        }
        if (piped) {
            const size_t per = plan.per_chunk;
            const size_t parts = plan.parts;
            const size_t cps = chunks / parts;
            uint32_t *differs = w.perm;
            hipStream_t s2 = c->aux[2];
            LWK_HIP(hipStreamWaitEvent(s2, c->ev_fork, 0));
            for (size_t j = 0; j < parts; j++) {
                const size_t off = j * cps * per, end_ = (j + 1) * cps * per < n ? (j + 1) * cps * per : n;
                if (off >= end_) continue;
                const size_t m = end_ - off;
                hipStream_t sk = (j & 1) ? s2 : st;
                LWK_HIP(hipStreamWaitEvent(sk, h.hashed[(j + 1) * cps - 1], 0));
                LWK_HIP(hipMemcpyAsync(w.zbytes + 32 * off, h.dig + 32 * off, m * 32, hipMemcpyHostToDevice, sk));
                launch_z_from_bytes(w.zbytes + 32 * off, z + off, nullptr, le, m, sk);
                coefficients_stage(c, blobs + off * (size_t)kBlobBytes, m, mode, stt + off, sk, off);
                quotient_stage(c, mode, w.scalars + off * (size_t)kBlobElems * 8, z + off, w.scalars2 + off * (size_t)kBlobElems * 8, nullptr, le, m, sk);
                (void)msm_sums_stage(c, w.scalars2 + off * (size_t)kBlobElems * 8, m, sk, off, false, evf);
            }
            LWK_HIP(hipEventRecord(c->ev_join[2], s2));
            LWK_HIP(hipStreamWaitEvent(st, c->ev_join[2], 0));
            LWK_HIP(hipStreamWaitEvent(st, c->ev_join[0], 0));
            launch_flag_differs48(canon, comm48, differs, n, st);
            launch_challenge(blobs, canon, z, le, n, st, comm48);
            quotient_stage(c, mode, w.scalars, z, w.scalars2, nullptr, le, n, st, differs);
            launch_direct_msm_only(evf ? c->lag.direct_bits : c->direct_bits, evf ? c->lag.direct_tab.win_dev : c->direct_tab.win_dev,
                                   evf ? c->lag.direct_row_bytes : c->direct_row_bytes, w.scalars2, w.sums, differs, n, st);
            launch_finalize_compress(w.sums, out48, n, st);
            return C_KZG_OK;
        }
        LWK_HIP(hipMemcpyAsync(w.zbytes, h.dig, n * 32, hipMemcpyHostToDevice, st));
        launch_z_from_bytes(w.zbytes, z, nullptr, le, n, st);
        LWK_HIP(hipStreamWaitEvent(st, c->ev_join[0], 0));
        launch_challenge(blobs, canon, z, le, n, st, comm48);
        break;
    }
    case kProofGpuChains: {
        LWK_HIP(hipEventRecord(c->ev_fork, st));
        LWK_HIP(hipStreamWaitEvent(c->vstream, c->ev_fork, 0));
        launch_validate_commitments(comm48, canon, stt, le ? kStatusBadArgs : kStatusError, n, c->vstream, longcall ? w.val_pts_long : w.val_pts,
                                    longcall ? w.val_kind_long : w.val_kind, longcall ? w.val_verdict_long : w.val_verdict);
        LWK_HIP(hipEventRecord(c->ev_join[0], c->vstream));
        launch_challenge(blobs, comm48, z, le, n, st);
        LWK_HIP(hipStreamWaitEvent(st, c->ev_join[0], 0));
        launch_challenge(blobs, canon, z, le, n, st, comm48);
        break;
    }
    }
    Ctx *pr = c->primary;
    const bool heavy_serial = plan.heavy_serial;
    if (heavy_serial) {
        std::lock_guard<std::mutex> hk(pr->heavy_mu);
        LWK_HIP(hipStreamWaitEvent(st, pr->heavy_done, 0));
    }
    for (size_t off = 0; off < n; off += kMaxChunk) {
        size_t m = n - off < kMaxChunk ? n - off : kMaxChunk;
        coefficients_stage(c, blobs + off * (size_t)kBlobBytes, m, mode, stt + off, st);
        quotient_stage(c, mode, w.scalars, z + off, w.scalars2, nullptr, le, m, st);
        G1Xyzz29 *sums = msm_sums_stage(c, w.scalars2, m, st, 0, false, quotient_to_msm_form(c, mode, m, st));
        if (heavy_serial && off + kMaxChunk >= n) {
            std::lock_guard<std::mutex> hk(pr->heavy_mu);
            LWK_HIP(hipEventRecord(pr->heavy_done, st));
        }
        launch_finalize_compress(sums, out48 + 48 * off, m, st);
    }
    return C_KZG_OK;
}

C_KZG_RET commit_and_prove_batch_device(Ctx *c, uint8_t *comm_out48, uint8_t *proof_out48, const uint8_t *blobs, size_t n, int mode,
                                        hipStream_t st, int32_t *status) {
    C_KZG_RET rc = ctx_reserve(c, n);
    if (rc != C_KZG_OK) return rc;
    const bool longcall = n > kMaxChunk;
    if (longcall) {
        rc = ws_long_reserve(c, n);
        if (rc != C_KZG_OK) return rc;
    }
    Workspace &w = c->ws;
    const int le = mode == LWKZG_MODE_CKZG;
    int32_t *stt = status ? status : longcall ? w.status_long : w.status;
    Fr *z = longcall ? w.z_long : w.z;
    uint32_t *mid = (uint32_t *)(longcall ? w.canon_long : w.canon48);
    LWK_HIP(hipMemsetAsync(stt, 0, n * 4, st));
    LWK_HIP(hipEventRecord(c->ev_fork, st));
    LWK_HIP(hipStreamWaitEvent(c->vstream, c->ev_fork, 0));
    const bool host_cold = n <= mid_proof_host_limit() && !peer_busy(c) && !host_assist_warm();
    if (host_cold) launch_host_wake(c);
    const bool host_mid = !host_cold && n <= mid_proof_host_limit() && !peer_busy(c) && sph_reserve(c, n);
    if (host_mid) {
        SmallProofHost &h = c->sph;
        hipStream_t sc = c->aux[0];
        LWK_HIP(hipStreamWaitEvent(sc, c->ev_fork, 0));
        {
            const C_KZG_RET rch = chunk_host_functions(c, blobs, n, sc, c->vstream, st, chunk_midstate_host_fn, "host_midstate_chunk");
            if (rch != C_KZG_OK) return rch;
        }
        LWK_HIP(hipMemcpyAsync(mid, h.dig, n * 32, hipMemcpyHostToDevice, c->vstream));
    } else {
        launch_challenge_midstate(blobs, mid, n, c->vstream);
    }
    LWK_HIP(hipEventRecord(c->ev_join[0], c->vstream));
    for (size_t off = 0; off < n; off += kMaxChunk) {
        const size_t m = n - off < kMaxChunk ? n - off : kMaxChunk;
        const uint8_t *b = blobs + off * (size_t)kBlobBytes;
        if (coefficients_stage(c, b, m, mode, stt + off, st)) {
            msm_stages(c, w.scalars, comm_out48 + 48 * off, m, st, 0, off == 0 && !host_mid, true);
        } else if (proof_on_lagrange(c, mode)) {
            launch_copy_le_check(b, (uint32_t *)w.fr, nullptr, m, st);
            msm_stages(c, (const uint32_t *)w.fr, comm_out48 + 48 * off, m, st, 0, off == 0 && !host_mid, true);
        } else {
            msm_stages(c, w.scalars, comm_out48 + 48 * off, m, st, 0, off == 0 && !host_mid);
        }
        if (off == 0) LWK_HIP(hipStreamWaitEvent(st, c->ev_join[0], 0));
        launch_challenge_finish(b, comm_out48 + 48 * off, mid + 8 * off, z + off, le, m, st);
        quotient_stage(c, mode, w.scalars, z + off, w.scalars2, nullptr, le, m, st);
        msm_stages(c, w.scalars2, proof_out48 + 48 * off, m, st, 0, false, quotient_to_msm_form(c, mode, m, st));
    }
    return C_KZG_OK;
}

C_KZG_RET point_proof_batch_device(Ctx *c, uint8_t *proof48, uint8_t *y32, const uint8_t *blobs, const uint8_t *z32,
                                   size_t n, int mode, hipStream_t st, int32_t *status, const G1Xyzz29 **sums_out) {
    C_KZG_RET rc = ctx_reserve(c, n);
    if (rc != C_KZG_OK) return rc;
    Workspace &w = c->ws;
    const int le = mode == LWKZG_MODE_CKZG;
    for (size_t off = 0; off < n; off += kMaxChunk) {
        size_t m = n - off < kMaxChunk ? n - off : kMaxChunk;
        int32_t *stt = status ? status + off : w.status;
        LWK_HIP(hipMemsetAsync(stt, 0, m * 4, st));
        coefficients_stage(c, blobs + off * (size_t)kBlobBytes, m, mode, stt, st);
        launch_z_from_bytes(z32 + 32 * off, w.z, stt, le, m, st);
        quotient_stage(c, mode, w.scalars, w.z, w.scalars2, y32 + 32 * off, le, m, st);
        const bool lg = quotient_to_msm_form(c, mode, m, st);
        if (sums_out && n <= kMaxChunk) *sums_out = msm_sums_stage(c, w.scalars2, m, st, 0, false, lg);
        else msm_stages(c, w.scalars2, proof48 + 48 * off, m, st, 0, false, lg);
    }
    return C_KZG_OK;
}


static C_KZG_RET first_status(Ctx *c, const int32_t *d_status, size_t n, hipStream_t st) {
    std::vector<int32_t> h(n);
    LWK_HIP(hipMemcpyAsync(h.data(), d_status, n * 4, hipMemcpyDeviceToHost, st));
    LWK_HIP(hipStreamSynchronize(st));
    for (size_t i = 0; i < n; i++)
        if (h[i] != 0) {
            set_error("input %zu rejected (status %d)", i, h[i]);
            return (C_KZG_RET)h[i];
        }
    return C_KZG_OK;
}

void verify_buffers_free(VerifyBuffers &v) {
    dev_free(v.pts_c);
    dev_free(v.pts_p);
    dev_free(v.mult_c);
    dev_free(v.mult_p);
    dev_free(v.kind_c);
    dev_free(v.kind_p);
    dev_free(v.proof_in);
    dev_free(v.comm_in);
    dev_free(v.canon_dev);
    dev_free(v.status_all);
    dev_free(v.verdict_c);
    dev_free(v.verdict_p);
    dev_free(v.d_r);
    dev_free(v.d_rz);
    dev_free(v.d_aff);
    dev_free(v.d_part);
    dev_free(v.d_inf);
    dev_free(v.vm_base);
    dev_free(v.d_rec);
    if (v.h_rec) {
        (void)hipHostFree(v.h_rec);
// ... 500 lines not shown
            LWK_HIP(hipMemcpyAsync(vb.d_rz + 32 * off, w.zbytes, m * 32, hipMemcpyDeviceToDevice, st));
        LWK_HIP(hipMemcpyAsync(z32 + 32 * off, w.zbytes, m * 32, hipMemcpyDeviceToHost, st));
        LWK_HIP(hipMemcpyAsync(y32 + 32 * off, w.ybytes, m * 32, hipMemcpyDeviceToHost, st));
        rc = first_status(c, w.status, m, st);
        if (rc != C_KZG_OK) return rc;
        if (proofs48 && !host_validate)
            LWK_HIP(hipStreamWaitEvent(st, c->ev_join[2], 0));
    }
    drain.armed = false;
    return C_KZG_OK;
}

C_KZG_RET verify_prepare_device(Ctx *c, const uint8_t *d_blobs, const uint8_t *d_comm, const uint8_t *d_proofs, size_t n, int mode,
                                uint8_t *z32, uint8_t *y32, uint8_t *canon_c, uint8_t *canon_p, VerifyBuffers &vb, hipStream_t caller,
                                uint8_t *records_out, bool keep) {
    if (!vb.owned) vb.hold = std::unique_lock<std::mutex>(c->verify_mu);
    std::lock_guard<std::mutex> lk(c->mu);
    LWK_HIP(hipSetDevice(c->device));
    const int le = mode == LWKZG_MODE_CKZG;
    const int bad = le ? kStatusBadArgs : kStatusError;
    hipStream_t st = c->stream, sv = c->vstream, sc = c->aux[0];
    if (caller && caller != st) {
        LWK_HIP(hipEventRecord(c->ev_join[3], caller));
        LWK_HIP(hipStreamWaitEvent(st, c->ev_join[3], 0));
    }
    WsUse wsu(c, st);
    struct SideDrain {
        Ctx *c;
        bool armed = true;
        ~SideDrain() {
            if (!armed) return;
            hipStreamSynchronize(c->vstream);
            hipStreamSynchronize(c->aux[0]);
        }
    } drain{c};
    if (vb.owned) {
        if (!vb.pts_c) {
            C_KZG_RET rcv = verify_buffers_alloc(vb, n < 64 ? 64 : n);
            if (rcv != C_KZG_OK) return rcv;
        }
    } else {
        C_KZG_RET rcv = vs_reserve(c, n);
        if (rcv != C_KZG_OK) return rcv;
        verify_buffers_lend(vb, c->vs);
    }
    C_KZG_RET rc = ctx_reserve(c, n < kMaxChunk ? n : kMaxChunk);
    if (rc != C_KZG_OK) return rc;
    if (n > kMaxChunk && (rc = ws_long_reserve(c, n)) != C_KZG_OK) return rc;
    Workspace &w = c->ws;
    Fr *z = n > kMaxChunk ? w.z_long : w.z;
    LWK_HIP(hipMemsetAsync(vb.status_all, 0, n * 4, st));
    LWK_HIP(hipEventRecord(c->ev_fork, st));
    LWK_HIP(hipStreamWaitEvent(sv, c->ev_fork, 0));
    LWK_HIP(hipStreamWaitEvent(sc, c->ev_fork, 0));
    const bool apart = n <= kVerifyApartMax;
    const bool fused = knobs().verify_fused || knobs().verify_msm;
    const bool hash_first = fused ? (apart != (knobs().verify_order != 0)) : knobs().verify_order != 0;
    if (hash_first) launch_challenge(d_blobs, d_comm, z, le, n, st);
    if (fused) {
        launch_decompress_points2(d_proofs, vb.pts_p, vb.kind_p, d_comm, vb.pts_c, vb.kind_c, n, sv, apart);
        LWK_HIP(hipEventRecord(c->ev_join[2], sv));
        launch_subgroup_canon2(vb.pts_p, vb.kind_p, vb.canon_dev + 48 * n, vb.verdict_p, vb.pts_c, vb.kind_c, vb.canon_dev, vb.verdict_c,
                               vb.status_all, bad, n, sv, apart);
        LWK_HIP(hipEventRecord(c->ev_join[0], sv));
        LWK_HIP(hipStreamWaitEvent(sc, c->ev_join[2], 0));
        launch_verify_rows(vb, n, sc, apart);
        LWK_HIP(hipEventRecord(c->ev_join[1], sc));
    } else {
        launch_validate_commitments(d_proofs, vb.canon_dev + 48 * n, vb.status_all, bad, n, sv, vb.pts_p, vb.kind_p, vb.verdict_p);
        launch_point_multiples(vb.pts_p, vb.kind_p, vb.mult_p, n, sv);
        LWK_HIP(hipEventRecord(c->ev_join[0], sv));
        launch_validate_commitments(d_comm, vb.canon_dev, vb.status_all, bad, n, sc, vb.pts_c, vb.kind_c, vb.verdict_c);
        launch_point_multiples(vb.pts_c, vb.kind_c, vb.mult_c, n, sc);
        LWK_HIP(hipEventRecord(c->ev_join[1], sc));
    }
    if (!apart && fused) {
        LWK_HIP(hipStreamWaitEvent(st, c->ev_join[0], 0));
        LWK_HIP(hipStreamWaitEvent(st, c->ev_join[1], 0));
    }
    if (!hash_first) launch_challenge(d_blobs, d_comm, z, le, n, st);
    LWK_HIP(hipStreamWaitEvent(st, c->ev_join[0], 0));
    LWK_HIP(hipStreamWaitEvent(st, c->ev_join[1], 0));
    drain.armed = false;
    launch_challenge(d_blobs, vb.canon_dev, z, le, n, st, d_comm);
    if (mode == LWKZG_MODE_REFERENCE) {
        launch_eval_y_from_blobs_be(d_blobs, z, vb.d_r, n, st);
        launch_fr_mont_to_bytes(z, vb.d_rz, le, n, st);
    } else if (proof_in_evaluation_form(c, mode)) {
        launch_eval_y_from_blobs_evalform(d_blobs, z, c->tw28_fwd + kBlobElems / 2, vb.d_r, vb.status_all, n, st);
        launch_fr_mont_to_bytes(z, vb.d_rz, le, n, st);
    } else {
        for (size_t off = 0; off < n; off += kMaxChunk) {
            const size_t m = n - off < kMaxChunk ? n - off : kMaxChunk;
            coefficients_stage(c, d_blobs + off * (size_t)kBlobBytes, m, mode, vb.status_all + off, st);
            quotient_stage(c, mode, w.scalars, z + off, nullptr , vb.d_r + 32 * off, le, m, st);
            launch_fr_mont_to_bytes(z + off, vb.d_rz + 32 * off, le, m, st);
        }
    }
    if (keep) return C_KZG_OK;
    if (records_out && vb.d_rec && vb.h_rec && vb.rec_cap >= n) {
        uint32_t *d_flag = (uint32_t *)(vb.d_rec + 160 * n);
        LWK_HIP(hipMemsetAsync(d_flag, 0xff, 4, st));
        launch_verify_records(vb.canon_dev, vb.d_rz, vb.d_r, vb.canon_dev + 48 * n, vb.status_all, vb.d_rec, d_flag, n, st);
        LWK_HIP(hipMemcpyAsync(vb.h_rec, vb.d_rec, 160 * n + 4, hipMemcpyDeviceToHost, st));
        LWK_HIP(hipStreamSynchronize(st));
        uint32_t first_bad;
        memcpy(&first_bad, vb.h_rec + 160 * n, 4);
        if (first_bad != 0xffffffffu) {
            int32_t code = 0;
            LWK_HIP(hipMemcpy(&code, vb.status_all + first_bad, 4, hipMemcpyDeviceToHost));
            set_error("input %zu rejected (status %d)", (size_t)first_bad, code);
            return (C_KZG_RET)code;
        }
        memcpy(records_out, vb.h_rec, 160 * n);
        return C_KZG_OK;
    }
    LWK_HIP(hipMemcpyAsync(canon_c, vb.canon_dev, n * 48, hipMemcpyDeviceToHost, st));
    LWK_HIP(hipMemcpyAsync(canon_p, vb.canon_dev + 48 * n, n * 48, hipMemcpyDeviceToHost, st));
    LWK_HIP(hipMemcpyAsync(z32, vb.d_rz, n * 32, hipMemcpyDeviceToHost, st));
    LWK_HIP(hipMemcpyAsync(y32, vb.d_r, n * 32, hipMemcpyDeviceToHost, st));
    return first_status(c, vb.status_all, n, st);
}

C_KZG_RET verify_openings_prepare_device(Ctx *c, const uint8_t *d_comm, const uint8_t *d_proofs, const uint8_t *d_z, const uint8_t *d_y,
                                         size_t n, int mode, VerifyBuffers &vb) {
    vb.hold = std::unique_lock<std::mutex>(c->verify_mu);
    std::lock_guard<std::mutex> lk(c->mu);
    LWK_HIP(hipSetDevice(c->device));
    const int le = mode == LWKZG_MODE_CKZG;
    const int bad = le ? kStatusBadArgs : kStatusError;
    hipStream_t st = c->stream;
    WsUse wsu(c, st);
    C_KZG_RET rc = vs_reserve(c, n);
    if (rc != C_KZG_OK) return rc;
    verify_buffers_lend(vb, c->vs);
    LWK_HIP(hipMemsetAsync(vb.status_all, 0, n * 4, st));
    launch_decompress_points2(d_proofs, vb.pts_p, vb.kind_p, d_comm, vb.pts_c, vb.kind_c, n, st);
    launch_subgroup_canon2(vb.pts_p, vb.kind_p, vb.canon_dev + 48 * n, vb.verdict_p, vb.pts_c, vb.kind_c, vb.canon_dev, vb.verdict_c,
                           vb.status_all, bad, n, st);
    launch_each_openings(d_z, d_y, vb.d_rz, vb.d_r, vb.status_all, bad, le, n, st);
    LWK_HIP(hipGetLastError());
    return C_KZG_OK;
}

C_KZG_RET lincomb3_device_host(Ctx *c, VerifyBuffers &vb, const uint8_t *sc_r, const uint8_t *sc_rz, size_t n,
                               uint8_t sums[3][96], int infs[3]) {
    std::lock_guard<std::mutex> lk(c->mu);
    LWK_HIP(hipSetDevice(c->device));
    hipStream_t st = c->stream;
    const size_t nblk = lincomb3_blocks(n);
    if (!(vb.hold.owns_lock() || vb.owned) || !vb.d_r) {
        set_error("lincomb3_device_host: called without a prepared verification");
        return C_KZG_ERROR;
    }
    uint8_t *d_r = vb.d_r, *d_rz = vb.d_rz, *d_aff = vb.d_aff;
    G1Xyzz29 *d_part = vb.d_part;
    int32_t *d_inf = vb.d_inf;
    uint8_t h_aff[3 * 96];
    int32_t h_inf[3];
    bool ok = true;
    if (ok) ok = hipMemcpyAsync(d_r, sc_r, 32 * n, hipMemcpyHostToDevice, st) == hipSuccess &&
                 hipMemcpyAsync(d_rz, sc_rz, 32 * n, hipMemcpyHostToDevice, st) == hipSuccess;
    if (ok) {
        launch_lincomb3(vb.pts_p, vb.kind_p, vb.mult_p, vb.pts_c, vb.kind_c, vb.mult_c, d_r, d_rz, d_part, n, st);
        G1Xyzz29 *totals = d_part + 3 * nblk;
        for (int k = 0; k < 3; k++) launch_sum_points(d_part + k * nblk, nblk, totals + k, 0, st);
        launch_xyzz29_to_affine_be(totals, d_aff, d_inf, 3, st);
        ok = hipMemcpyAsync(h_aff, d_aff, sizeof h_aff, hipMemcpyDeviceToHost, st) == hipSuccess &&
             hipMemcpyAsync(h_inf, d_inf, sizeof h_inf, hipMemcpyDeviceToHost, st) == hipSuccess &&
             hipStreamSynchronize(st) == hipSuccess;
    }
    if (!ok) {
        set_error("lincomb3_device_host: device work failed: %s", hipGetErrorString(hipGetLastError()));
        return C_KZG_ERROR;
    }
    for (int k = 0; k < 3; k++) {
        memcpy(sums[k], h_aff + 96 * k, 96);
        infs[k] = h_inf[k];
    }
    return C_KZG_OK;
}

bool vmsm_ready(const VerifyBuffers &vb) { return knobs().verify_msm && vb.tab_p && vb.h_pin && vb.vm_done; }

C_KZG_RET vmsm_begin(Ctx *c, VerifyBuffers &vb, const Fr *pw33, int le, size_t n) {
    std::lock_guard<std::mutex> lk(c->mu);
    LWK_HIP(hipSetDevice(c->device));
    hipStream_t st = c->stream;
    if (!(vb.hold.owns_lock() || vb.owned) || !vmsm_ready(vb) || !vb.d_rz) {
        set_error("vmsm_begin: called without a prepared verification");
        return C_KZG_ERROR;
    }
    memcpy(vb.h_pin, pw33, 33 * sizeof(Fr));
    LWK_HIP(hipMemcpyAsync(vb.vm_pw, vb.h_pin, 33 * sizeof(Fr), hipMemcpyHostToDevice, st));
    launch_vmsm_scalars(vb.d_rz, le, vb.vm_pw, vb.sc_a, vb.sc_b, n, st);
    launch_vmsm_accumulate(vb.sc_a, vb.sc_b, vb.tab_p, vb.kind_p, vb.tab_c, vb.kind_c, vb.vm_partial, n, st);
    launch_vmsm_reduce(vb.vm_partial, vb.vm_bsum, vb.d_aff, vb.d_inf, n, st);
    LWK_HIP(hipMemcpyAsync(vb.h_pin + 33 * sizeof(Fr), vb.d_aff, 3 * 96, hipMemcpyDeviceToHost, st));
    LWK_HIP(hipMemcpyAsync(vb.h_pin + 33 * sizeof(Fr) + 3 * 96, vb.d_inf, 3 * 4, hipMemcpyDeviceToHost, st));
    LWK_HIP(hipEventRecord(vb.vm_done, st));
    return C_KZG_OK;
}

C_KZG_RET vmsm_finish(Ctx *c, VerifyBuffers &vb, uint8_t sums[3][96], int infs[3]) {
    LWK_HIP(hipSetDevice(c->device));
    if (hipEventSynchronize(vb.vm_done) != hipSuccess) {
        set_error("vmsm_finish: device work failed: %s", hipGetErrorString(hipGetLastError()));
        return C_KZG_ERROR;
    }
    const uint8_t *res = vb.h_pin + 33 * sizeof(Fr);
    for (int k = 0; k < 3; k++) {
        memcpy(sums[k], res + 96 * k, 96);
        int32_t f;
        memcpy(&f, res + 3 * 96 + 4 * k, 4);
        infs[k] = f;
    }
    return C_KZG_OK;
}

}


using namespace lwk;

static std::atomic<int> g_mode{-1};

static int mode_now() {
    int m = g_mode.load(std::memory_order_relaxed);
    if (m < 0) {
        m = knobs().mode ? LWKZG_MODE_CKZG : LWKZG_MODE_REFERENCE;
        int expect = -1;
        if (!g_mode.compare_exchange_strong(expect, m)) m = expect;
    }
    return m;
}

namespace lwk {
int mode_of(const KZGSettings *s) {
    if (s) {
        std::lock_guard<std::mutex> lk(g_reg_mu);
        Ctx *c = nullptr;
        if (s->fs && g_live_fs.count((const void *)s->fs)) c = (Ctx *)s->fs;
        else if (s->g1_values) {
            auto it = g_registry.find(s->g1_values);
            if (it != g_registry.end()) c = it->second.ctx;
        }
        if (c) {
            const int m = c->mode_override.load(std::memory_order_relaxed);
            if (m >= 0) return m;
        }
    }
    return mode_now();
}
}

extern "C" {

int lwkzg_set_mode(int mode) {
    int prev = mode_now();
    if (mode != LWKZG_MODE_REFERENCE && mode != LWKZG_MODE_CKZG) return -1;
    g_mode.store(mode);
    return prev;
}
int lwkzg_get_mode(void) { return mode_now(); }

static void settings_follow_mode(Ctx *c, int mode);
int lwkzg_settings_set_mode(const KZGSettings *s, int mode) {
    if (mode != LWKZG_MODE_REFERENCE && mode != LWKZG_MODE_CKZG && mode != -1) return -1;
    Ctx *c = ctx_of(s);
    if (!c) return -1;
    const int prev = lwk::mode_of(s);
    c->mode_override.store(mode, std::memory_order_relaxed);
    const int now = lwk::mode_of(s);
    if (now != prev && gpu_available()) settings_follow_mode(c, now);
    return prev;
}
int lwkzg_settings_get_mode(const KZGSettings *s) { return lwk::mode_of(s); }

int lwkzg_device_count(void) {
    int n = 0;
    if (hipGetDeviceCount(&n) != hipSuccess) return 0;
    return n;
}
int lwkzg_set_device(int ordinal) {
    int n = lwkzg_device_count();
    if (ordinal < 0 || ordinal >= n) {
        set_error("lwkzg_set_device(%d): %d device(s) visible", ordinal, n);
        return -1;
    }
    g_default_device.store(ordinal);
    return 0;
}
const char *lwkzg_version(void) { return "lambdaworks_kzg_amd 0.2 (gfx950; direct-table MSM, 10..16-bit windows; bucket fallback c=13, 20 windows)"; }
const char *lwkzg_last_error(void) { return get_error(); }
int lwkzg_msm_window_bits(void) { return kWindowBits; }
int lwkzg_msm_num_windows(void) { return kNumWindows; }

void lwkzg_profile_enable(int on) {
    if (!on) prof_drain();
    g_prof_on.store(on != 0);
}
void lwkzg_profile_reset(void) {
    prof_drain();
    std::lock_guard<std::mutex> lk(g_prof_mu);
    g_prof_agg.clear();
}
size_t lwkzg_profile_report(char *buf, size_t cap) {
    prof_drain();
    std::string s = "{";
    {
        std::lock_guard<std::mutex> lk(g_prof_mu);
        bool first = true;
        for (auto &kv : g_prof_agg) {
            char line[256];
            snprintf(line, sizeof line, "%s\"%s\": {\"launches\": %llu, \"total_ms\": %.6f}", first ? "" : ", ",
                     kv.first.c_str(), (unsigned long long)kv.second.launches, kv.second.total_ms);
            s += line;
            first = false;
        }
    }
    s += "}";
    if (buf && cap) {
        size_t k = s.size() < cap - 1 ? s.size() : cap - 1;
        memcpy(buf, s.data(), k);
        buf[k] = 0;
    }
    return s.size() + 1;
}

__global__ void k_runtime_init(int *p) {
    if (p) *p = 1;
}

extern "C" int lwkzg_last_proof_schedule(void) { return g_last_proof_schedule.load(std::memory_order_relaxed); }

extern "C" int lwkzg_runtime_init(void) {
    if (!gpu_available()) return -1;
    if (hipSetDevice(g_default_device.load()) != hipSuccess || hipFree(nullptr) != hipSuccess) return -1;
    hipFuncAttributes attr;
    if (hipFuncGetAttributes(&attr, (const void *)k_runtime_init) != hipSuccess) {
        (void)hipGetLastError();
        return -1;
    }
    return 0;
}

__global__ __launch_bounds__(256) void k_clock_probe(unsigned long long *out, uint32_t iters, uint32_t seed) {
    uint64_t acc = seed + threadIdx.x;
    const uint32_t a = (seed * 2654435761u) | 1u, b = seed ^ 0x9e3779b9u;
    const long long c0 = clock64(), w0 = wall_clock64();
    for (uint32_t i = 0; i < iters; i++) {
#pragma unroll
        for (int k = 0; k < 64; k++) acc = (uint64_t)(uint32_t)acc * a + (acc >> 32) + b;
    }
    const long long c1 = clock64(), w1 = wall_clock64();
    if ((threadIdx.x & 63) == 0) {
        const unsigned w = (blockIdx.x * blockDim.x + threadIdx.x) >> 6;
        out[3 * w] = (unsigned long long)(c1 - c0);
        out[3 * w + 1] = (unsigned long long)(w1 - w0);
        out[3 * w + 2] = acc;
    }
}

extern "C" C_KZG_RET lwkzg_clock_probe_mhz(double *mhz) {
    if (!mhz) return C_KZG_BADARGS;
    *mhz = 0;
    if (!gpu_available()) {
        set_error("no GPU: lambdaworks_kzg_amd has no CPU fallback");
        return C_KZG_ERROR;
    }
    LWK_HIP(hipSetDevice(g_default_device.load()));
    const unsigned wgs = 256, waves = wgs * 4;
    unsigned long long *d = nullptr;
    hipStream_t st = nullptr;
    LWK_HIP(hipStreamCreateWithFlags(&st, hipStreamNonBlocking));
    if (hipMalloc((void **)&d, waves * 3 * sizeof(unsigned long long)) != hipSuccess) {
        hipStreamDestroy(st);
        return C_KZG_MALLOC;
    }
    std::vector<unsigned long long> h(waves * 3);
    hipError_t e = hipSuccess;
    for (int rep = 0; rep < 3 && e == hipSuccess; rep++) {
        hipLaunchKernelGGL(k_clock_probe, dim3(wgs), dim3(256), 0, st, d, 250u, 12345u + rep);
        e = hipStreamSynchronize(st);
    }
    if (e == hipSuccess) e = hipMemcpy(h.data(), d, h.size() * sizeof(unsigned long long), hipMemcpyDeviceToHost);
    hipFree(d);
    hipStreamDestroy(st);
    if (e != hipSuccess) {
        set_error("lwkzg_clock_probe_mhz: %s", hipGetErrorString(e));
        return C_KZG_ERROR;
    }
    double clk = 0, wall = 0;
    for (unsigned w = 0; w < waves; w++) {
        clk += (double)h[3 * w];
        wall += (double)h[3 * w + 1];
    }
    if (wall > 0) *mhz = clk / wall * 100.0;
    return C_KZG_OK;
}

extern "C" size_t lwkzg_timing_report(const KZGSettings *s, char *buf, size_t cap) {
    Ctx *c = ctx_of(s);
    char tmp[1024];
    int k = 0;
    if (c) {
        std::lock_guard<std::mutex> lk(c->mu);
        const LoadTiming &l = c->load_timing;
        const BuildTiming &b = c->last_build;
        k = snprintf(tmp, sizeof tmp,
                     "{\"load\": {\"context_ms\": %.3f, \"points_and_tables_ms\": %.3f, \"g2_and_fft_ms\": %.3f, \"default_table_ms\": %.3f, "
                     "\"total_ms\": %.3f}, \"last_table_build\": {\"bits\": %d, \"row_bytes\": %zu, \"table_bytes\": %zu, \"free_old_ms\": %.3f, "
                     "\"table_malloc_ms\": %.3f, \"scratch_malloc_ms\": %.3f, \"kernels_ms\": %.3f, \"scratch_free_ms\": %.3f, \"total_ms\": %.3f, \"in_place\": %d}}",
                     l.context_ms, l.points_and_tables_ms, l.g2_and_fft_ms, l.default_table_ms, l.total_ms, b.bits, b.row_bytes, b.table_bytes,
                     b.free_old_ms, b.table_malloc_ms, b.scratch_malloc_ms, b.kernels_ms, b.scratch_free_ms, b.total_ms, (int)b.in_place);
    } else {
        k = snprintf(tmp, sizeof tmp, "{}");
    }
    if (buf && cap) {
        size_t n = (size_t)k < cap - 1 ? (size_t)k : cap - 1;
        memcpy(buf, tmp, n);
        buf[n] = 0;
    }
    return (size_t)k + 1;
}


static C_KZG_RET setup_from_bytes(KZGSettings *out, const uint8_t *g1_bytes, const uint8_t *g2_bytes) {
    Ctx *c = nullptr;
    auto wall = [] { return std::chrono::duration<double, std::milli>(std::chrono::steady_clock::now().time_since_epoch()).count(); };
    const double t_start = wall();
    C_KZG_RET rc = ctx_new(&c);
    if (rc != C_KZG_OK) return rc;
    LoadTiming lt;
    lt.context_ms = wall() - t_start;
    double t_mark = wall();
    const size_t n1 = kBlobElems, n2 = TRUSTED_SETUP_NUM_G2_POINTS;
    uint8_t *d_in = nullptr;
    int32_t *d_status = nullptr;
    uint64_t *d_blst = nullptr;
    g1_t *g1v = (g1_t *)malloc(n1 * sizeof(g1_t));
    g2_t *g2v = (g2_t *)malloc(n2 * sizeof(g2_t));
    std::vector<int32_t> h_status(n1);
    rc = C_KZG_ERROR;
    do {
        if (!g1v || !g2v) { rc = C_KZG_MALLOC; break; }
        if (hipMalloc((void **)&d_in, n1 * 48) != hipSuccess || hipMalloc((void **)&d_status, n1 * 4) != hipSuccess ||
            hipMalloc((void **)&d_blst, n1 * 144) != hipSuccess) { rc = C_KZG_MALLOC; set_error("hipMalloc failed in setup load"); break; }
        if (hipMemcpyAsync(d_in, g1_bytes, n1 * 48, hipMemcpyHostToDevice, c->stream) != hipSuccess) { set_error("H2D of g1 bytes failed"); break; }
        launch_g1_decompress(d_in, c->points, d_status, n1, 1, c->stream);
        launch_g1_to_blst(c->points, d_status, d_blst, n1, c->stream);
        launch_build_table(c->points, c->table, c->stream);
        if (hipMemcpyAsync(h_status.data(), d_status, n1 * 4, hipMemcpyDeviceToHost, c->stream) != hipSuccess ||
            hipMemcpyAsync(g1v, d_blst, n1 * 144, hipMemcpyDeviceToHost, c->stream) != hipSuccess ||
            hipStreamSynchronize(c->stream) != hipSuccess) { set_error("setup kernels failed: %s", hipGetErrorString(hipGetLastError())); break; }
        bool good = true;
        for (size_t i = 0; i < n1; i++) {
            if (h_status[i] == 2) { set_error("g1 point %zu: invalid compressed point or not in the subgroup", i); good = false; break; }
            if (h_status[i] == 1) { set_error("g1 point %zu is the point at infinity: the reference cannot read such a setup back (srs.rs:155-172)", i); good = false; break; }
        }
        if (!good) break;
        lt.points_and_tables_ms = wall() - t_mark;
        t_mark = wall();
        if (!g2_fill_values(g2v, g2_bytes, n2)) { if (!get_error()[0]) set_error("invalid g2 point in trusted setup"); break; }
        rc = ctx_finish_fft(c);
        lt.g2_and_fft_ms = wall() - t_mark;
    } while (0);
    if (d_in) hipFree(d_in);
    if (d_status) hipFree(d_status);
    if (d_blst) hipFree(d_blst);
    if (rc != C_KZG_OK) {
        free(g1v);
        free(g2v);
        ctx_destroy(c);
        return rc;
    }
    out->fs = &c->fs;
    out->g1_values = g1v;
    out->g2_values = g2v;
    t_mark = wall();
    direct_from_env(out);
    lt.default_table_ms = wall() - t_mark;
    lt.total_ms = wall() - t_start;
    c->load_timing = lt;
    return C_KZG_OK;
}

C_KZG_RET load_trusted_setup(KZGSettings *out, const uint8_t *g1_bytes, size_t n1, const uint8_t *g2_bytes, size_t n2) {
    if (!out || !g1_bytes || !g2_bytes) return C_KZG_BADARGS;
    if (n1 != TRUSTED_SETUP_NUM_G1_POINTS || n2 != TRUSTED_SETUP_NUM_G2_POINTS) return C_KZG_BADARGS;
    return setup_from_bytes(out, g1_bytes, g2_bytes);
}

static int hexv(int ch) {
    if (ch >= '0' && ch <= '9') return ch - '0';
    if (ch >= 'a' && ch <= 'f') return ch - 'a' + 10;
    if (ch >= 'A' && ch <= 'F') return ch - 'A' + 10;
    return -1;
}

C_KZG_RET load_trusted_setup_file(KZGSettings *out, FILE *in) {
    if (!out || !in) return C_KZG_BADARGS;
    std::string text;
    char buf[64 * 1024];
    size_t got;
    while ((got = fread(buf, 1, sizeof buf, in)) > 0) text.append(buf, got);
    std::vector<std::pair<size_t, size_t>> lines;
    size_t pos = 0;
    while (pos < text.size()) {
        size_t e = text.find('\n', pos);
        if (e == std::string::npos) e = text.size();
        size_t len = e - pos;
        if (len && text[pos + len - 1] == '\r') len--;
        lines.push_back({pos, len});
        pos = e + 1;
    }
    auto parse_count = [&](size_t li, size_t *v) -> bool {
        if (li >= lines.size()) return false;
        size_t o = lines[li].first, l = lines[li].second, k = 0;
        if (l && text[o] == '+') k = 1;
        if (k == l) return false;
        size_t acc = 0;
        for (; k < l; k++) {
            char ch = text[o + k];
            if (ch < '0' || ch > '9') return false;
            acc = acc * 10 + (size_t)(ch - '0');
            if (acc > (1u << 24)) return false;
        }
        *v = acc;
        return true;
    };
    size_t n1 = 0, n2 = 0;
    if (!parse_count(0, &n1) || !parse_count(1, &n2)) {
        set_error("trusted setup file: bad header");
        return C_KZG_ERROR;
    }
    if (n1 != TRUSTED_SETUP_NUM_G1_POINTS || n2 != TRUSTED_SETUP_NUM_G2_POINTS) {
        set_error("trusted setup file announces %zu/%zu points; this engine needs 4096/65", n1, n2);
        return C_KZG_BADARGS;
    }
    if (lines.size() < 2 + n1 + n2) {
        set_error("trusted setup file: %zu point lines, expected %zu", lines.size() - 2, n1 + n2);
        return C_KZG_ERROR;
    }
    std::vector<uint8_t> g1(n1 * 48), g2(n2 * 96);
    for (size_t i = 0; i < n1 + n2; i++) {
        size_t nb = i < n1 ? 48 : 96;
        uint8_t *dst = i < n1 ? &g1[i * 48] : &g2[(i - n1) * 96];
        size_t o = lines[2 + i].first, l = lines[2 + i].second;
        if (l != 2 * nb) {
            set_error("trusted setup file: line %zu has %zu characters, expected %zu", i + 3, l, 2 * nb);
            return C_KZG_ERROR;
        }
        for (size_t k = 0; k < nb; k++) {
            int h = hexv(text[o + 2 * k]), lo = hexv(text[o + 2 * k + 1]);
            if (h < 0 || lo < 0) {
                set_error("trusted setup file: line %zu is not hex", i + 3);
                return C_KZG_ERROR;
            }
            dst[k] = (uint8_t)(h * 16 + lo);
        }
    }
    return setup_from_bytes(out, g1.data(), g2.data());
}

C_KZG_RET free_trusted_setup(KZGSettings *s) {
    if (!s) return C_KZG_OK;
    Ctx *c = nullptr;
    {
        std::lock_guard<std::mutex> lk(g_reg_mu);
        if (s->fs && g_live_fs.count((const void *)s->fs)) {
            c = (Ctx *)s->fs;
        } else {
            auto it = g_registry.find(s->g1_values);
            if (it != g_registry.end()) {
                c = it->second.ctx;
                g_registry.erase(it);
            }
        }
    }
    ctx_destroy(c);
    free(s->g1_values);
    free(s->g2_values);
    s->fs = nullptr;
    s->g1_values = nullptr;
    s->g2_values = nullptr;
    return C_KZG_OK;
}

C_KZG_RET lwkzg_release_context(const KZGSettings *s) {
    if (!s) return C_KZG_BADARGS;
    Ctx *c = nullptr;
    {
        std::lock_guard<std::mutex> lk(g_reg_mu);
        if (s->fs && g_live_fs.count((const void *)s->fs)) return C_KZG_BADARGS;
        auto it = g_registry.find(s->g1_values);
        if (it == g_registry.end()) return C_KZG_OK;
        c = it->second.ctx;
        g_registry.erase(it);
    }
    ctx_destroy(c);
    return C_KZG_OK;
}


static C_KZG_RET collect_status(Ctx *c, const int32_t *d_status, size_t n, size_t base, size_t *first_bad) {
// ... 1262 lines not shown
```

### lambdaworks_kzg_amd/csrc/g1.cuh

```cuda
#pragma once
#include "field.cuh"
#include "field29.cuh"

namespace lwk {


LWK_HD bool literal_zero(const Fp &a) { return a.is_zero(); }
template <int B, bool I>
LWK_HD bool literal_zero(const F29<B, I> &a) { return a.is_literal_zero(); }

template <class FX, class FY>
struct alignas(16) AffineT {
    FX x;
    FY y;
};

template <class FX, class FY, class FZ>
struct alignas(16) XyzzT {
    FX x;
    FY y;
    FZ zz, zzz;

    LWK_HD static XyzzT infinity() {
        XyzzT r;
        r.x = FX::zero();
        r.y = FY::zero();
        r.zz = FZ::zero();
        r.zzz = FZ::zero();
        return r;
    }
    LWK_HD bool is_inf() const { return literal_zero(zz); }
    template <class QX, class QY>
    LWK_HD static XyzzT from_affine(const QX &qx, const QY &qy) {
        XyzzT r;
        r.x = qx;
        r.y = qy;
        r.zz = FZ::one();
        r.zzz = FZ::one();
        return r;
    }
};

typedef AffineT<Fp, Fp> G1Affine;
typedef XyzzT<Fp, Fp, Fp> G1Xyzz;
typedef AffineT<F29<2>, F29<2>> G1Affine29;
typedef XyzzT<F29<14>, F29<6>, F29<2>> G1Xyzz29;
typedef AffineT<F29<2, true>, F29<2, true>> G1Affine29i;
typedef XyzzT<F29<14, true>, F29<6, true>, F29<2, true>> G1Xyzz29i;
static_assert(sizeof(G1Affine29i) == sizeof(G1Affine29) && sizeof(G1Xyzz29i) == sizeof(G1Xyzz29), "layout");

LWK_HD Fp fp_from_u32(uint32_t v) {
    uint32_t raw[12];
#pragma unroll
    for (int i = 0; i < 12; i++) raw[i] = (i == 0) ? v : 0u;
    return fe_from_raw<FpParams>(raw);
}

LWK_HD bool g1_on_curve(const G1Affine &p) {
    Fp l = sqr(p.y);
    Fp r = sqr(p.x) * p.x + fp_from_u32(4);
    return l == r;
}

template <class X, class QX, class QY>
LWK_HD X xyzz_dbl_affine(const QX &qx, const QY &qy) {
    if (qy.is_zero()) return X::infinity();
    auto u = dbl(qy);
    auto v = sqr(u);
    auto w = u * v;
    auto s = qx * v;
    auto xx = sqr(qx);
    auto m = dbl(xx) + xx;
    X r;
    auto x3 = normed(sqr(m) - dbl(s));
    r.x = x3;
    r.y = mul_sub(m, s - x3, w, qy);
    r.zz = v;
    r.zzz = w;
    return r;
}

template <class X>
LWK_HD X xyzz_dbl(const X &p) {
    if (p.is_inf() || p.y.is_zero()) return X::infinity();
    auto u = dbl(p.y);
    auto v = sqr(u);
    auto w = u * v;
    auto s = p.x * v;
    auto xx = sqr(p.x);
    auto m = dbl(xx) + xx;
    X r;
    auto x3 = normed(sqr(m) - dbl(s));
    r.x = x3;
    r.y = mul_sub(m, s - x3, w, p.y);
    r.zz = v * p.zz;
    r.zzz = w * p.zzz;
    return r;
}

template <class X, class QX, class QY>
LWK_HD X xyzz_madd(const X &acc, const QX &qx, const QY &qy) {
    if (acc.is_inf()) return X::from_affine(qx, qy);
    auto u2 = qx * acc.zz;
    auto s2 = qy * acc.zzz;
    auto pp_ = u2 - acc.x;
    auto rr = s2 - acc.y;
    if (pp_.is_zero()) {
        if (rr.is_zero()) return xyzz_dbl_affine<X>(qx, qy);
        return X::infinity();
    }
    auto pp = sqr(pp_);
    auto ppp = pp_ * pp;
    auto qq = acc.x * pp;
    X r;
    auto x3 = normed(sqr(rr) - ppp - dbl(qq));
    r.x = x3;
    r.y = mul_sub(rr, qq - x3, acc.y, ppp);
    r.zz = acc.zz * pp;
    r.zzz = acc.zzz * ppp;
    return r;
}

LWK_HD G1Xyzz xyzz_madd(const G1Xyzz &acc, const G1Affine &q) { return xyzz_madd(acc, q.x, q.y); }

template <class X, class QX, class QY, class F>
LWK_HD void xyzz_madd_split(X &acc, const QX &qx, const QY &qy, F &&row_is_dead) {
    bool done = false;
    decltype(qx * acc.zz) u2;
    decltype(qy * acc.zzz) s2;
    if (acc.is_inf()) {
        acc = X::from_affine(qx, qy);
        done = true;
    } else {
        u2 = qx * acc.zz;
        s2 = qy * acc.zzz;
        if ((u2 - acc.x).is_zero()) {
            if ((s2 - acc.y).is_zero()) acc = xyzz_dbl_affine<X>(qx, qy);
            else acc = X::infinity();
            done = true;
        }
    }
    row_is_dead();
    if (done) return;
    auto pp_ = u2 - acc.x;
    auto rr = s2 - acc.y;
    auto pp = sqr(pp_);
    auto ppp = pp_ * pp;
    auto qq = acc.x * pp;
    auto x3 = normed(sqr(rr) - ppp - dbl(qq));
    X r;
    r.x = x3;
    r.y = mul_sub(rr, qq - x3, acc.y, ppp);
    r.zz = acc.zz * pp;
    r.zzz = acc.zzz * ppp;
    acc = r;
}

template <class X>
LWK_HD X xyzz_add(const X &a, const X &b) {
    if (a.is_inf()) return b;
    if (b.is_inf()) return a;
    auto u1 = a.x * b.zz;
    auto u2 = b.x * a.zz;
    auto s1 = a.y * b.zzz;
    auto s2 = b.y * a.zzz;
    auto pp_ = u2 - u1;
    auto rr = s2 - s1;
    if (pp_.is_zero()) {
        if (rr.is_zero()) return xyzz_dbl(a);
        return X::infinity();
    }
    auto pp = sqr(pp_);
    auto ppp = pp_ * pp;
    auto qq = u1 * pp;
    X r;
    auto x3 = normed(sqr(rr) - ppp - dbl(qq));
    r.x = x3;
    r.y = mul_sub(rr, qq - x3, s1, ppp);
    r.zz = a.zz * b.zz * pp;
    r.zzz = a.zzz * b.zzz * ppp;
    return r;
}

LWK_HD G1Affine affine_neg(const G1Affine &p) {
    G1Affine r;
    r.x = p.x;
    r.y = neg(p.y);
    return r;
}

LWK_HD G1Affine xyzz_to_affine(const G1Xyzz &p) {
    Fp i = inv(p.zz * p.zzz);
    Fp izz = i * p.zzz;
    Fp izzz = i * p.zz;
    G1Affine r;
    r.x = p.x * izz;
    r.y = p.y * izzz;
    return r;
}

LWK_HD G1Affine xyzz_to_affine(const G1Xyzz29 &p) {
    auto i = f29_inv(p.zz * p.zzz);
    auto izz = i * p.zzz;
    auto izzz = i * p.zz;
    G1Affine r;
    r.x = f29_to_fp(p.x * izz);
    r.y = f29_to_fp(p.y * izzz);
    return r;
}

LWK_HD G1Affine29 xyzz29_to_affine29(const G1Xyzz29 &p) {
    auto i = f29_inv(p.zz * p.zzz);
    auto izz = i * p.zzz;
    auto izzz = i * p.zz;
    G1Affine29 r;
    r.x = p.x * izz;
    r.y = p.y * izzz;
    return r;
}

LWK_HD G1Affine29 affine_to_29(const G1Affine &p) {
    G1Affine29 r;
    r.x = f29_from_fp(p.x);
    r.y = f29_from_fp(p.y);
    return r;
}

template <class Root>
LWK_HD int g1_decompress29_nocheck_t(const uint8_t *in48, F29<2> &x, F29<2> &y, bool &want_greater, Root root) {
    uint8_t b[48];
    for (int k = 0; k < 48; k++) b[k] = in48[k];
    const uint8_t prefix = b[0] >> 5;
    want_greater = (prefix & 1) != 0;
    if (!(prefix & 4)) return 2;
    if (prefix & 2) return 1;
    b[0] &= 0x1f;
    uint32_t raw[12];
    raw_from_be<12>(raw, b);
    x = f29_from_raw32(raw);
    uint32_t four[12] = {4};
    F29<2> y2 = (sqr(x) * x + f29_from_raw32(four)) * F29<1>::one();
    const uint32_t e[12] = {0xffffeaabu, 0xee7fbfffu, 0xac54ffffu, 0x07aaffffu, 0x3dac3d89u, 0xd9cc34a8u,
                            0x3ce144afu, 0xd91dd2e1u, 0x90d2eb35u, 0x92c6e9edu, 0x8e5ff9a6u, 0x0680447au};
    F29<2> r = root(y2, e);
    if (!(sqr(r) - y2).is_zero()) return 2;
    uint32_t ry[12], half[12], one[12] = {1};
    f29_to_raw32(ry, r);
    raw_sub<12>(half, FpParams::MOD, one);
#pragma unroll
    for (int k = 0; k < 11; k++) half[k] = (half[k] >> 1) | (half[k + 1] << 31);
    half[11] >>= 1;
    const bool r_greater = !raw_geq<12>(half, ry);
    y = cneg(r, want_greater != r_greater) * F29<1>::one();
    return 0;
}
LWK_HD int g1_decompress29_nocheck(const uint8_t *in48, F29<2> &x, F29<2> &y, bool &want_greater) {
    return g1_decompress29_nocheck_t(in48, x, y, want_greater, [](const F29<2> &a, const uint32_t *e) { return f29_pow<12>(a, e); });
}

template <int NK>
LWK_HD G1Xyzz xyzz_mul_affine(const G1Affine &p, const uint32_t *k) {
    G1Xyzz acc = G1Xyzz::infinity();
    for (int i = NK * 32 - 1; i >= 0; i--) {
        acc = xyzz_dbl(acc);
        if ((k[i >> 5] >> (i & 31)) & 1) acc = xyzz_madd(acc, p.x, p.y);
    }
    return acc;
}

LWK_HD bool g1_in_subgroup_by_order(const G1Affine &p) {
    uint32_t r[8];
#pragma unroll
    for (int i = 0; i < 8; i++) r[i] = FrParams::MOD[i];
    return xyzz_mul_affine<8>(p, r).is_inf();
}

template <class X>
LWK_HD X xyzz_mul_by_z(const X &t) {
    X acc = t;
    for (int i = 62; i >= 0; i--) {
        acc = xyzz_dbl(acc);
        if (i == 62 || i == 60 || i == 57 || i == 48 || i == 16) acc = xyzz_add(acc, t);
    }
    return acc;
}

template <class X, class FX, class FY, class FB>
LWK_HD bool g1_in_subgroup_endo(const FX &px, const FY &py, const FB &beta) {
    X p = X::from_affine(px, py);
    X q = xyzz_mul_by_z(xyzz_mul_by_z(p));
    if (q.is_inf()) return false;
    auto dx = q.x - (beta * px) * q.zz;
    auto sy = q.y + py * q.zzz;
    return dx.is_zero() && sy.is_zero();
}

LWK_HD void g1_beta_raw(uint32_t raw[12]) {
    const uint32_t b[12] = {0xfffefffeu, 0x2e01ffffu, 0x620a0002u, 0xde17d813u, 0xe6f89688u, 0xddb3a93bu,
                            0x6a0f77eau, 0xba69c607u, 0xdf76ce51u, 0x5f19672fu, 0x00000000u, 0x00000000u};
#pragma unroll
    for (int i = 0; i < 12; i++) raw[i] = b[i];
}

LWK_HD bool g1_in_subgroup(const G1Affine &p) {
    uint32_t raw[12];
    g1_beta_raw(raw);
    return g1_in_subgroup_endo<G1Xyzz>(p.x, p.y, fe_from_raw<FpParams>(raw));
}

LWK_HD void g1_compress_affine(uint8_t out[48], const G1Affine &a) {
    uint32_t rx[12], ry[12], ryn[12];
    fe_to_raw<FpParams>(rx, a.x);
    fe_to_raw<FpParams>(ry, a.y);
    fe_to_raw<FpParams>(ryn, neg(a.y));
    raw_to_be<12>(out, rx);
    out[0] |= 0x80;
    if (!raw_geq<12>(ryn, ry)) out[0] |= 0x20;
}

template <class X>
LWK_HD void g1_compress(uint8_t out[48], const X &p) {
    if (p.is_inf()) {
        for (int i = 0; i < 48; i++) out[i] = 0;
        out[0] = 0xc0;
        return;
    }
    g1_compress_affine(out, xyzz_to_affine(p));
}

LWK_HD int g1_decompress_nocheck(G1Affine &out, const uint8_t in[48]) {
    uint8_t prefix = in[0] >> 5;
    if (!(prefix & 4)) return 2;
    if (prefix & 2) return 1;
    uint8_t b[48];
    for (int i = 0; i < 48; i++) b[i] = in[i];
    b[0] &= 0x1f;
    uint32_t raw[12];
    raw_from_be<12>(raw, b);
    Fp x = fe_from_raw<FpParams>(raw);
    Fp y2 = sqr(x) * x + fp_from_u32(4);
    const uint32_t e[12] = {0xffffeaabu, 0xee7fbfffu, 0xac54ffffu, 0x07aaffffu, 0x3dac3d89u, 0xd9cc34a8u,
                            0x3ce144afu, 0xd91dd2e1u, 0x90d2eb35u, 0x92c6e9edu, 0x8e5ff9a6u, 0x0680447au};
    Fp y = fe_pow<FpParams, 12>(y2, e);
    if (sqr(y) != y2) return 2;
    Fp yn = neg(y);
    uint32_t ry[12], ryn[12];
    fe_to_raw<FpParams>(ry, y);
    fe_to_raw<FpParams>(ryn, yn);
    bool y_greater = raw_geq<12>(ry, ryn);
    bool want_greater = (prefix & 1) != 0;
    out.x = x;
    out.y = (want_greater == y_greater) ? y : yn;
    return 0;
}

}
```

### lambdaworks_kzg_amd/csrc/kernels.h

```cpp
#pragma once
#include <hip/hip_runtime.h>
#include <stdint.h>
#include "g1.cuh"
#include "fr28.cuh"
#include "plan.h"

namespace lwk {

struct ProfScope {
    ProfScope(const char *name, hipStream_t st);
    ~ProfScope();
    const char *name;
    hipStream_t st;
    hipEvent_t e0, e1;
    bool on;
};

void launch_parse_be_reduce(const uint8_t *blobs, uint32_t *scalars_raw, size_t n_elems, hipStream_t st, uint32_t *zero = nullptr, uint32_t zero_words = 0);

void launch_digit_sort(const uint32_t *scalars_raw, uint32_t *sorted, uint32_t *bucket_start, uint32_t *perm,
                       size_t n_blobs, hipStream_t st);
void launch_bucket_accumulate(const G1Affine29 *table, const uint32_t *sorted, const uint32_t *bucket_start,
                              const uint32_t *perm, G1Xyzz29 *buckets, size_t n_blobs, hipStream_t st);
void launch_bucket_reduce(const G1Xyzz29 *buckets, G1Xyzz29 *sums, size_t n_blobs, hipStream_t st);
void launch_sum_points(const G1Xyzz29 *in, size_t n, G1Xyzz29 *total, int accumulate, hipStream_t st);
void launch_finalize_compress(const G1Xyzz29 *sums, uint8_t *out48, size_t n, hipStream_t st);

constexpr int kDirectMinBits = 10, kDirectMaxBits = 16;
constexpr size_t kDirectRowAligned = 128, kDirectRowPacked = 112;
constexpr size_t kDirectAlignedHeadroom = (size_t)8 << 30;
size_t direct_table_entries(int bits);
int direct_num_windows(int bits);
constexpr int kDirectMaxWindows = 26;
struct DirectTable {
    void *win[kDirectMaxWindows] = {};
    uint64_t *win_dev = nullptr;
    int nw = 0;
    size_t bytes = 0;
};
hipError_t build_direct_table(int bits, const G1Affine *points, DirectTable &table, size_t row_bytes, hipStream_t st, double *ms = nullptr,
                              bool in_place = false);
void free_direct_table(DirectTable &table);
void launch_direct_msm(int bits, const uint64_t *win_dev, size_t row_bytes, const uint32_t *scalars_raw, G1Xyzz29 *lane_scratch,
                       G1Xyzz29 *partials, uint32_t *redo, G1Xyzz29 *sums, size_t n_blobs, hipStream_t st, int fill = 0,
                       uint32_t *redo_flag_out = nullptr);
uint32_t direct_one_blob_counter_words(int bits);
void launch_direct_msm_only(int bits, const uint64_t *win_dev, size_t row_bytes, const uint32_t *scalars_raw, G1Xyzz29 *sums,
                            const uint32_t *only_if, size_t n_blobs, hipStream_t st);

void launch_g1_decompress(const uint8_t *in48, G1Affine *out, int32_t *status, size_t n, int subgroup_check,
                          hipStream_t st);
void launch_g1_from_blst(const uint64_t *blst_p1, G1Affine *out, int32_t *status, size_t n, hipStream_t st);
void launch_g1_to_blst(const G1Affine *in, const int32_t *status, uint64_t *blst_p1, size_t n, hipStream_t st);
void launch_build_table(const G1Affine *points, G1Affine29 *table, hipStream_t st);

void launch_build_twiddles(Fr *tw_fwd, Fr *tw_inv, hipStream_t st);
void launch_twiddles_to28(const Fr *tw, Fr28 *tw28, hipStream_t st);
void launch_ntt4096(const Fr *in, Fr *out, const Fr28 *tw28, int inverse_scale_to_raw, size_t n_blobs, hipStream_t st);
void launch_blob_evaluations_to_coefficients(const uint8_t *blobs, uint32_t *coeffs_raw, const Fr28 *tw28_inv, int32_t *status,
                                             size_t n_blobs, hipStream_t st);
void launch_bitrev_permute(const Fr *in, Fr *out, size_t n_blobs, hipStream_t st);
void launch_idft_columns(uint32_t *coeffs_raw, const Fr *tw_inv, uint32_t first, size_t n_rows, hipStream_t st);
void launch_copy_le_check(const uint8_t *blobs, uint32_t *scalars_raw, int32_t *status, size_t n_blobs, hipStream_t st);
void launch_coefficients_to_evaluations(uint32_t *coeffs_raw, Fr *scratch, Fr *scratch2, const Fr28 *tw28_fwd, size_t n_blobs, hipStream_t st);
void launch_fr_be_to_mont(const uint8_t *in_be, Fr *out, size_t n_elems, hipStream_t st);
void launch_fr_mont_to_be(const Fr *in, uint8_t *out_be, size_t n_elems, hipStream_t st);
void launch_raw_to_be(const uint32_t *raw, uint8_t *out_be, size_t n_elems, hipStream_t st);
void launch_fr_mont_to_bytes(const Fr *in, uint8_t *out, int le, size_t n, hipStream_t st);
void launch_eval_quotient(const uint32_t *coeffs_raw, const Fr *z_mont, uint32_t *quot_raw, uint8_t *y_out, int le,
                          size_t n_blobs, hipStream_t st, const uint32_t *only_if = nullptr);
void launch_eval_y_from_blobs_be(const uint8_t *blobs, const Fr *z_mont, uint8_t *y_out, size_t n_blobs, hipStream_t st);
void launch_eval_y_from_blobs_evalform(const uint8_t *blobs, const Fr *z_mont, const Fr28 *roots_brp28, uint8_t *y_out, int32_t *status,
                                       size_t n_blobs, hipStream_t st);
void launch_roots_brp28(const Fr28 *tw28_fwd, Fr28 *roots_brp28, hipStream_t st);
void launch_eval_quotient_evalform(const uint32_t *evals_raw, const Fr *z_mont, const Fr28 *roots_brp28, uint32_t *quot_raw, uint8_t *y_out, int le,
                                   size_t n_blobs, hipStream_t st, const uint32_t *only_if = nullptr);
void launch_flag_differs48(const uint8_t *a, const uint8_t *b, uint32_t *flags, size_t n, hipStream_t st);
void launch_z_from_bytes(const uint8_t *z_bytes, Fr *z_mont, int32_t *status, int le, size_t n, hipStream_t st);

void launch_validate_commitments(const uint8_t *comm48, uint8_t *canon48, int32_t *status, int bad_code, size_t n,
                                 hipStream_t st, G1Affine29 *aff_out = nullptr, int32_t *kind_out = nullptr, uint32_t *verdict_scratch = nullptr,
                                 bool apart = false);
size_t lincomb3_blocks(size_t n);
void launch_point_multiples(const G1Affine29 *pts, const int32_t *kind, G1Affine29 *mult, size_t n, hipStream_t st);
void launch_point_multiples2(const G1Affine29 *pts_a, const int32_t *kind_a, G1Affine29 *mult_a, const G1Affine29 *pts_b,
                             const int32_t *kind_b, G1Affine29 *mult_b, size_t n, hipStream_t st);
void launch_decompress_points(const uint8_t *in48, G1Affine29 *pts, int32_t *kind, size_t n, hipStream_t st, bool apart = false);
void launch_subgroup_canon(G1Affine29 *pts, int32_t *kind, uint8_t *canon48, int32_t *status, int bad_code, size_t n,
                           hipStream_t st, uint32_t *verdict_scratch = nullptr, bool apart = false);
void launch_decompress_points2(const uint8_t *in48_a, G1Affine29 *pts_a, int32_t *kind_a, const uint8_t *in48_b, G1Affine29 *pts_b,
                               int32_t *kind_b, size_t n, hipStream_t st, bool apart = false);
void launch_subgroup_canon2(G1Affine29 *pts_a, int32_t *kind_a, uint8_t *canon48_a, uint32_t *verdict_a, G1Affine29 *pts_b, int32_t *kind_b,
                            uint8_t *canon48_b, uint32_t *verdict_b, int32_t *status, int bad_code, size_t n, hipStream_t st, bool apart = false);
void launch_lincomb3(const G1Affine29 *proofs, const int32_t *proof_kind, const G1Affine29 *proof_mult, const G1Affine29 *comms,
                     const int32_t *comm_kind, const G1Affine29 *comm_mult, const uint8_t *sc_r_be, const uint8_t *sc_rz_be,
                     G1Xyzz29 *partial, size_t n, hipStream_t st);
constexpr int kVmsmDigits = 16;
constexpr int kVmsmRows = 2 * kVmsmDigits;
constexpr int kVmsmSteps = kVmsmDigits - 1;
constexpr int kVmsmMaxTerms = 64;
constexpr size_t kVmsmPinBytes = 33 * 32 + 3 * 96 + 3 * 4 + 52;
constexpr int kVmsmListCap = 24;
void launch_vmsm_multiples2(const G1Affine29 *pts_a, const int32_t *kind_a, G1Affine29 *tab_a, const G1Affine29 *pts_b,
                            const int32_t *kind_b, G1Affine29 *tab_b, G1Xyzz29 *tmp, F29<2> *pre, size_t n, hipStream_t st, bool apart = false);
void launch_vmsm_scalars(const uint8_t *z_bytes, int le, const Fr *pw, uint32_t *sc_a, uint32_t *sc_b, size_t n, hipStream_t st);
uint32_t vmsm_terms_per_slice(size_t n);
size_t vmsm_slices(size_t n);
size_t vmsm_max_slices(size_t cap);
void launch_vmsm_accumulate(const uint32_t *sc_a, const uint32_t *sc_b, const G1Affine29 *tab_p, const int32_t *kind_p,
                            const G1Affine29 *tab_c, const int32_t *kind_c, G1Xyzz29 *partial, size_t n, hipStream_t st);
void launch_vmsm_reduce(const G1Xyzz29 *partial, G1Xyzz29 *bsum, uint8_t *out96, int32_t *inf, size_t n, hipStream_t st);
void launch_verify_records(const uint8_t *canon_c, const uint8_t *z32, const uint8_t *y32, const uint8_t *canon_p, const int32_t *status,
                           uint8_t *records, uint32_t *first_bad, size_t n, hipStream_t st);
void launch_each_openings(const uint8_t *z_in, const uint8_t *y_in, uint8_t *z_out, uint8_t *y_out, int32_t *status, int bad_code, int le,
                          size_t n, hipStream_t st);
void launch_xyzz29_to_affine_be(const G1Xyzz29 *in, uint8_t *out96, int32_t *inf, size_t n, hipStream_t st);
void launch_challenge(const uint8_t *blobs, const uint8_t *canon48, Fr *z_mont, int le, size_t n, hipStream_t st,
                      const uint8_t *only_if_differs_from = nullptr);
void launch_challenge_midstate(const uint8_t *blobs, uint32_t *midstate, size_t n, hipStream_t st);
void launch_challenge_finish(const uint8_t *blobs, const uint8_t *canon48, const uint32_t *midstate, Fr *z_mont, int le, size_t n,
                             hipStream_t st);
void sha256_host(uint8_t out[32], const uint8_t *msg, size_t len);
void challenge_digests_host(uint8_t *digests32, const uint8_t *blobs, const uint8_t *comms48, size_t n);
double host_hash_rate();
void challenge_midstates_host(uint32_t *mid, const uint8_t *blobs, size_t n);
void sha256_blocks_portable(uint32_t h[8], const uint8_t *blocks, size_t n_blocks);

constexpr int kCellElems = 64;
constexpr int kCellsPerBlob = 128;
void launch_cells_extend(const uint32_t *coeffs_raw, const Fr *tw_fwd, const Fr28 *tw28_fwd, Fr *scratch, Fr *scratch2, uint8_t *cells,
                         int le, size_t n_blobs, hipStream_t st);
void launch_cells_quotients(const uint32_t *coeffs_raw, const Fr *tw_fwd, uint32_t *quot_raw, size_t n_cells, hipStream_t st);

}
```

### lambdaworks_kzg_amd/csrc/knobs.h

```cpp
#pragma once
#include <stddef.h>
#include <stdint.h>

namespace lwk {

struct Knobs {
    int mode = 0;
    bool has_direct_bits = false;
    int direct_bits = 0;
    int direct_row = 0;
    bool coalesce = true;
    bool twin = true;
    size_t small_proof_host = 64;
    size_t mid_proof_host = 384;
    int host_threads = 0;
    int host_warm_ms = 2000;
    size_t host_finish = 8;
    bool timing = false;
    bool verbose = false;
    bool experimental = false;

    bool direct_asm = true;
    bool fold_asm = true;
    bool bucket_asm = true;
    int direct_fill = 0;
    int coop = 1;
    int coop_max = 8;
    int coop_rpq = 0;
    bool sort_stage = true;
    int reduce_lanes = 0;
    bool hash_pairs = true;
    int hash_prio = 1;
    bool validate_coop = true;
    unsigned validate_lds_pad = 112u * 1024u;
    bool ckzg_eval_proofs = true;
    bool mid_proof_pipe = true;
    size_t mid_proof_pipe_min = 192;
    size_t mid_proof_parts = 0;
    size_t mid_proof_chunks = 4;
    int proof_schedule = -1;
    int heavy_serial = -1;
    int split = 0;
    size_t slice0 = 0;
    bool set_mode_in_place = true;
    int host_fp_portable = 0;
    int host_hash_grain = 4;
    int stage_streams[2] = {8, 0};
    int side_workers = 1;
    bool pairing_generic_sqr = false, pairing_naive = false, pairing_no_precomp = false, pairing_one_thread = false;
    int verify_msm = 1;
    int verify_fused = 1;
    int verify_pad_kb[3] = {60, 116, 116};
    int verify_order = 0;
    int verify_cu_mask = 0;
    int vmsm_list_cap = 0;
    bool zero_copy = true;
    bool host_stage = true;
};

const Knobs &knobs();

const char *knob_names_operational();
const char *knob_names_experimental();

}
```

### lambdaworks_kzg_amd/csrc/knobs.hip

```cpp
#include "knobs.h"

#include <mutex>
#include <stdio.h>
#include <stdlib.h>
#include <string.h>

namespace lwk {
namespace {

struct Reader {
    bool experimental;
    const char *get(const char *name, bool exp) const {
        const char *v = getenv(name);
        if (!v || !*v) return nullptr;
        if (exp && !experimental) {
            if (getenv("LWKZG_VERBOSE")) fprintf(stderr, "[lambdaworks_kzg_amd] %s ignored: experiment knobs need LWKZG_EXPERIMENTAL=1\n", name);
            return nullptr;
        }
        return v;
    }
    void flag(bool &dst, const char *name, bool exp) const {
        if (const char *v = get(name, exp)) dst = atoi(v) != 0;
    }
    void present(bool &dst, const char *name, bool exp) const {
        if (get(name, exp)) dst = true;
    }
    void num(int &dst, const char *name, bool exp) const {
        if (const char *v = get(name, exp)) dst = atoi(v);
    }
    void num(size_t &dst, const char *name, bool exp) const {
        if (const char *v = get(name, exp)) {
            const long x = atol(v);
            dst = x < 0 ? 0 : (size_t)x;
        }
    }
    void num(unsigned &dst, const char *name, bool exp) const {
        if (const char *v = get(name, exp)) dst = (unsigned)atoi(v);
    }
};

Knobs read_env() {
    Knobs k;
    {
        const char *e = getenv("LWKZG_EXPERIMENTAL");
        k.experimental = e && atoi(e) != 0;
    }
    const Reader r{k.experimental};
    constexpr bool OP = false, EXP = true;
    if (const char *e = r.get("LWKZG_MODE", OP))
        k.mode = (!strcmp(e, "ckzg") || !strcmp(e, "c") || !strcmp(e, "C") || !strcmp(e, "1")) ? 1 : 0;
    if (const char *e = r.get("LWKZG_DIRECT_BITS", OP)) {
        k.has_direct_bits = true;
        k.direct_bits = !strcmp(e, "auto") ? -1 : atoi(e);
    }
    r.num(k.direct_row, "LWKZG_DIRECT_ROW", OP);
    r.flag(k.coalesce, "LWKZG_COALESCE", OP);
    r.flag(k.twin, "LWKZG_TWIN", OP);
    r.num(k.small_proof_host, "LWKZG_SMALL_PROOF_HOST", OP);
    r.num(k.mid_proof_host, "LWKZG_MID_PROOF_HOST", OP);
    r.num(k.host_threads, "LWKZG_HOST_THREADS", OP);
    r.num(k.host_warm_ms, "LWKZG_HOST_WARM_MS", OP);
    r.num(k.host_finish, "LWKZG_HOST_FINISH", OP);
    r.present(k.timing, "LWKZG_TIMING", OP);
    r.present(k.verbose, "LWKZG_VERBOSE", OP);

    r.flag(k.direct_asm, "LWKZG_DIRECT_ASM", EXP);
    r.flag(k.fold_asm, "LWKZG_FOLD_ASM", EXP);
    r.flag(k.bucket_asm, "LWKZG_BUCKET_ASM", EXP);
    r.num(k.direct_fill, "LWKZG_DIRECT_FILL", EXP);
    r.num(k.coop, "LWKZG_COOP", EXP);
    r.num(k.coop_max, "LWKZG_COOP_MAX", EXP);
    if (k.coop_max < 1) k.coop_max = 1;
    if (k.coop_max > 8) k.coop_max = 8;
    r.num(k.coop_rpq, "LWKZG_COOP_RPQ", EXP);
    r.flag(k.sort_stage, "LWKZG_SORT_STAGE", EXP);
    r.num(k.reduce_lanes, "LWKZG_REDUCE_LANES", EXP);
    r.flag(k.hash_pairs, "LWKZG_HASH_PAIRS", EXP);
    r.num(k.hash_prio, "LWKZG_HASH_PRIO", EXP);
    r.flag(k.validate_coop, "LWKZG_VALIDATE_COOP", EXP);
    r.num(k.validate_lds_pad, "LWKZG_VALIDATE_LDS_PAD", EXP);
    r.flag(k.ckzg_eval_proofs, "LWKZG_CKZG_EVAL_PROOFS", EXP);
    r.flag(k.mid_proof_pipe, "LWKZG_MID_PROOF_PIPE", EXP);
    r.num(k.mid_proof_pipe_min, "LWKZG_MID_PROOF_PIPE_MIN", EXP);
    r.num(k.mid_proof_parts, "LWKZG_MID_PROOF_PARTS", EXP);
    r.num(k.mid_proof_chunks, "LWKZG_MID_PROOF_CHUNKS", EXP);
    r.num(k.heavy_serial, "LWKZG_HEAVY_SERIAL", EXP);
    r.num(k.proof_schedule, "LWKZG_PROOF_SCHEDULE", EXP);
    r.num(k.split, "LWKZG_SPLIT", EXP);
    r.num(k.slice0, "LWKZG_SLICE0", EXP);
    r.flag(k.set_mode_in_place, "LWKZG_SET_MODE_IN_PLACE", EXP);
    r.num(k.host_fp_portable, "LWKZG_HOST_FP_PORTABLE", EXP);
    r.num(k.side_workers, "LWKZG_SIDE_WORKERS", EXP);
    r.num(k.host_hash_grain, "LWKZG_HOST_HASH_GRAIN", EXP);
    r.present(k.pairing_generic_sqr, "LWKZG_PAIRING_GENERIC_SQR", EXP);
    r.present(k.pairing_naive, "LWKZG_PAIRING_NAIVE", EXP);
    r.present(k.pairing_no_precomp, "LWKZG_PAIRING_NO_PRECOMP", EXP);
    r.present(k.pairing_one_thread, "LWKZG_PAIRING_ONE_THREAD", EXP);
    r.num(k.verify_msm, "LWKZG_VERIFY_MSM", EXP);
    r.num(k.verify_fused, "LWKZG_VERIFY_FUSED", EXP);
    if (const char *e = r.get("LWKZG_VERIFY_PAD_KB", EXP)) {
        int a = 0, b = 0, c = 0;
        const int got = sscanf(e, "%d,%d,%d", &a, &b, &c);
        if (got >= 1) k.verify_pad_kb[0] = a;
        k.verify_pad_kb[1] = got >= 2 ? b : a;
        k.verify_pad_kb[2] = got >= 3 ? c : (got >= 2 ? b : a);
        for (int &p : k.verify_pad_kb) p = p < 0 ? 0 : (p > 150 ? 150 : p);
    }
    r.num(k.verify_order, "LWKZG_VERIFY_ORDER", EXP);
    r.num(k.verify_cu_mask, "LWKZG_VERIFY_CU_MASK", EXP);
    r.num(k.vmsm_list_cap, "LWKZG_VMSM_LIST_CAP", EXP);
    r.flag(k.zero_copy, "LWKZG_ZERO_COPY", EXP);
    r.flag(k.host_stage, "LWKZG_HOST_STAGE", EXP);
    if (const char *e = r.get("LWKZG_STAGE_STREAMS", EXP)) {
        int a = 8, b = 0;
        if (sscanf(e, "%d,%d", &a, &b) == 2 && a >= 0 && a <= 8 && b >= 0 && b < 8 && a != b) {
            k.stage_streams[0] = a;
            k.stage_streams[1] = b;
        }
    }
    return k;
}

}

const Knobs &knobs() {
    static const Knobs k = read_env();
    return k;
}

const char *knob_names_operational() {
    return "LWKZG_MODE LWKZG_DIRECT_BITS LWKZG_DIRECT_ROW LWKZG_COALESCE LWKZG_TWIN LWKZG_SMALL_PROOF_HOST LWKZG_MID_PROOF_HOST "
           "LWKZG_HOST_THREADS LWKZG_HOST_WARM_MS LWKZG_HOST_FINISH LWKZG_TIMING LWKZG_VERBOSE LWKZG_EXPERIMENTAL";
}

const char *knob_names_experimental() {
    return "LWKZG_DIRECT_ASM LWKZG_FOLD_ASM LWKZG_BUCKET_ASM LWKZG_DIRECT_FILL LWKZG_COOP LWKZG_COOP_MAX LWKZG_COOP_RPQ LWKZG_SORT_STAGE "
           "LWKZG_REDUCE_LANES LWKZG_HASH_PAIRS LWKZG_HASH_PRIO LWKZG_VALIDATE_COOP LWKZG_VALIDATE_LDS_PAD LWKZG_CKZG_EVAL_PROOFS "
           "LWKZG_MID_PROOF_PIPE LWKZG_MID_PROOF_PIPE_MIN LWKZG_MID_PROOF_PARTS LWKZG_MID_PROOF_CHUNKS LWKZG_HEAVY_SERIAL LWKZG_PROOF_SCHEDULE LWKZG_SPLIT "
           "LWKZG_SLICE0 LWKZG_SET_MODE_IN_PLACE LWKZG_PAIRING_GENERIC_SQR LWKZG_PAIRING_NAIVE LWKZG_PAIRING_NO_PRECOMP "
           "LWKZG_PAIRING_ONE_THREAD LWKZG_VERIFY_MSM LWKZG_VERIFY_FUSED LWKZG_VERIFY_PAD_KB LWKZG_VERIFY_ORDER LWKZG_VERIFY_CU_MASK LWKZG_VMSM_LIST_CAP "
           "LWKZG_HOST_STAGE LWKZG_ZERO_COPY LWKZG_HOST_FP_PORTABLE LWKZG_SIDE_WORKERS LWKZG_HOST_HASH_GRAIN LWKZG_STAGE_STREAMS";
}

}

extern "C" __attribute__((visibility("default"))) size_t lwkzg_knob_report(char *buf, size_t cap) {
    const lwk::Knobs &k = lwk::knobs();
    char tmp[4096];
    const int n = snprintf(
        tmp, sizeof tmp,
        "{\"experimental\": %s, \"mode\": %d, \"direct_bits\": %s%d, \"direct_row\": %d, \"coalesce\": %d, \"twin\": %d, "
        "\"small_proof_host\": %zu, \"mid_proof_host\": %zu, \"host_threads\": %d, \"host_warm_ms\": %d, \"host_finish\": %zu, "
        "\"timing\": %d, \"verbose\": %d, \"direct_asm\": %d, \"fold_asm\": %d, \"bucket_asm\": %d, \"coop\": %d, \"coop_max\": %d, "
        "\"hash_pairs\": %d, \"hash_prio\": %d, \"validate_coop\": %d, \"ckzg_eval_proofs\": %d, \"mid_proof_pipe\": %d, "
        "\"verify_msm\": %d, \"verify_fused\": %d, \"verify_pad_kb\": [%d, %d, %d], \"verify_order\": %d, \"vmsm_list_cap\": %d, "
        "\"host_stage\": %d, \"operational\": \"%s\", \"experimental_names\": \"%s\"}",
        k.experimental ? "true" : "false", k.mode, k.has_direct_bits ? "" : "null, \"direct_bits_unset_default\": ", k.direct_bits, k.direct_row,
        (int)k.coalesce, (int)k.twin, k.small_proof_host, k.mid_proof_host, k.host_threads, k.host_warm_ms, k.host_finish, (int)k.timing,
        (int)k.verbose, (int)k.direct_asm, (int)k.fold_asm, (int)k.bucket_asm, k.coop, k.coop_max, (int)k.hash_pairs, k.hash_prio,
        (int)k.validate_coop, (int)k.ckzg_eval_proofs, (int)k.mid_proof_pipe, k.verify_msm, k.verify_fused, k.verify_pad_kb[0],
        k.verify_pad_kb[1], k.verify_pad_kb[2], k.verify_order, k.vmsm_list_cap, (int)k.host_stage, lwk::knob_names_operational(),
        lwk::knob_names_experimental());
    const size_t need = (size_t)(n < 0 ? 0 : n) + 1;
    if (buf && cap) {
        const size_t c = need <= cap ? need - 1 : cap - 1;
        memcpy(buf, tmp, c);
        buf[c] = 0;
    }
    return need;
}
```

### lambdaworks_kzg_amd/csrc/msm.hip

```cpp
#include "kernels.h"
#include "knobs.h"

#include <stdlib.h>

namespace lwk {


__device__ __forceinline__ uint32_t bswap32(uint32_t v) { return __builtin_bswap32(v); }

__global__ __launch_bounds__(256) void k_parse_be_reduce(const uint4 *__restrict__ in, uint4 *__restrict__ out,
                                                         size_t n_elems, uint32_t *__restrict__ zero, uint32_t zero_words) {
    size_t i = (size_t)blockIdx.x * blockDim.x + threadIdx.x;
    if (i < zero_words) zero[i] = 0u;
    if (i >= n_elems) return;
    uint4 hi = in[2 * i], lo = in[2 * i + 1];
    uint32_t s[8];
    s[7] = bswap32(hi.x);
    s[6] = bswap32(hi.y);
    s[5] = bswap32(hi.z);
    s[4] = bswap32(hi.w);
    s[3] = bswap32(lo.x);
    s[2] = bswap32(lo.y);
    s[1] = bswap32(lo.z);
    s[0] = bswap32(lo.w);
#pragma unroll
    for (int k = 0; k < 2; k++) {
        uint32_t d[8];
        uint32_t br = raw_sub<8>(d, s, FrParams::MOD);
#pragma unroll
        for (int j = 0; j < 8; j++) s[j] = br ? s[j] : d[j];
    }
    out[2 * i] = make_uint4(s[0], s[1], s[2], s[3]);
    out[2 * i + 1] = make_uint4(s[4], s[5], s[6], s[7]);
}

void launch_parse_be_reduce(const uint8_t *blobs, uint32_t *scalars_raw, size_t n_elems, hipStream_t st, uint32_t *zero, uint32_t zero_words) {
    ProfScope p("k_parse_be_reduce", st);
    unsigned grid = (unsigned)((n_elems + 255) / 256);
    hipLaunchKernelGGL(k_parse_be_reduce, dim3(grid), dim3(256), 0, st, (const uint4 *)blobs, (uint4 *)scalars_raw,
                       n_elems, zero, zero_words < n_elems ? zero_words : (uint32_t)n_elems);
}


template <int J>
__device__ __forceinline__ uint32_t window_bits(const uint32_t *s) {
    constexpr int o = J * kWindowBits;
    constexpr int limb = o >> 5;
    constexpr int sh = o & 31;
    uint32_t v = s[limb] >> sh;
    if constexpr (sh + kWindowBits > 32 && limb + 1 < 8) v |= s[limb + 1] << (32 - sh);
    return v & ((1u << kWindowBits) - 1);
}

template <int J, class F>
__device__ __forceinline__ void for_each_digit(const uint32_t *s, uint32_t carry, F &&f) {
    if constexpr (J < kNumWindows) {
        uint32_t raw = window_bits<J>(s) + carry;
        uint32_t neg = raw > (1u << (kWindowBits - 1)) ? 1u : 0u;
        uint32_t mag = neg ? (1u << kWindowBits) - raw : raw;
        if (mag) f(J, mag - 1, neg);
        for_each_digit<J + 1>(s, neg, f);
    }
}

__device__ __forceinline__ uint32_t wave_inclusive_scan(uint32_t v, int lane) {
#pragma unroll
    for (int d = 1; d < 64; d <<= 1) {
        uint32_t t = __shfl_up(v, d, 64);
        if (lane >= d) v += t;
    }
    return v;
}

constexpr int kSortThreads = 1024;
constexpr int kHeavyThreshold = 64;
constexpr int kBucketsPerSortThread = kNumBuckets / kSortThreads;
constexpr int kScalarsPerSortThread = kBlobElems / kSortThreads;
constexpr int kStageEntries = 16384;
static_assert(kNumBuckets % kSortThreads == 0 && kBlobElems % kSortThreads == 0, "sort tiling");

template <bool staged>
__global__ __launch_bounds__(kSortThreads) void k_digit_sort(const uint4 *__restrict__ scalars,
                                                             uint32_t *__restrict__ sorted,
                                                             uint32_t *__restrict__ bucket_start,
                                                             uint32_t *__restrict__ perm) {
    __shared__ uint32_t cnt[kNumBuckets];
    __shared__ uint32_t wave_tot[kSortThreads / 64];
    __shared__ uint32_t pop_hist[256];
    __shared__ uint32_t pop_cur[256];
    __shared__ uint32_t bst[kNumBuckets + 1];
    __shared__ uint32_t stage[kStageEntries + kHeavyThreshold];

    const int tid = threadIdx.x;
    const int lane = tid & 63, wave = tid >> 6;
    const size_t blob = blockIdx.x;
    const uint4 *sc = scalars + blob * (size_t)kBlobElems * 2;

    for (int k = tid; k < kNumBuckets; k += kSortThreads) cnt[k] = 0;
    if (tid < 256) pop_hist[tid] = 0;
    __syncthreads();

    auto load_scalar = [&](int q, uint32_t *w) {
        const int e = q * kSortThreads + tid;
        const uint4 lo = sc[2 * e], hi = sc[2 * e + 1];
        w[0] = lo.x; w[1] = lo.y; w[2] = lo.z; w[3] = lo.w;
        w[4] = hi.x; w[5] = hi.y; w[6] = hi.z; w[7] = hi.w;
    };
#pragma unroll
    for (int q = 0; q < kScalarsPerSortThread; q++) {
        uint32_t s[8];
        load_scalar(q, s);
        for_each_digit<0>(s, 0u, [&](int, uint32_t b, uint32_t) { atomicAdd(&cnt[b], 1u); });
    }
    __syncthreads();

    uint32_t c[kBucketsPerSortThread];
    uint32_t local = 0;
#pragma unroll
    for (int k = 0; k < kBucketsPerSortThread; k++) {
        c[k] = cnt[tid * kBucketsPerSortThread + k];
        local += c[k];
    }
    uint32_t incl = wave_inclusive_scan(local, lane);
    if (lane == 63) wave_tot[wave] = incl;
    __syncthreads();
    if (wave == 0) {
        uint32_t t = lane < kSortThreads / 64 ? wave_tot[lane] : 0u;
        uint32_t ti = wave_inclusive_scan(t, lane);
        if (lane < kSortThreads / 64) wave_tot[lane] = ti - t;
    }
    __syncthreads();
    uint32_t base = wave_tot[wave] + incl - local;
    uint32_t *bs = bucket_start + blob * (size_t)(kNumBuckets + 1);
#pragma unroll
    for (int k = 0; k < kBucketsPerSortThread; k++) {
        int b = tid * kBucketsPerSortThread + k;
        bs[b] = base;
        cnt[b] = base;
        bst[b] = base;
        base += c[k];
        atomicAdd(&pop_hist[c[k] > 255u ? 255u : c[k]], 1u);
    }
    if (tid == kSortThreads - 1) {
        bs[kNumBuckets] = base;
        bst[kNumBuckets] = base;
    }
    __syncthreads();

    if (tid < 256) {
        uint32_t before = 0;
        for (int k = tid + 1; k < 256; k++) before += pop_hist[k];
        pop_cur[tid] = before;
        if (tid == kHeavyThreshold) perm[blob * (size_t)(kNumBuckets + 1) + kNumBuckets] = before;
    }
    __syncthreads();
    uint32_t *pm = perm + blob * (size_t)(kNumBuckets + 1);
#pragma unroll
    for (int k = 0; k < kBucketsPerSortThread; k++) {
        uint32_t pos = atomicAdd(&pop_cur[c[k] > 255u ? 255u : c[k]], 1u);
        pm[pos] = (uint32_t)(tid * kBucketsPerSortThread + k);
    }

    const uint32_t total = bst[kNumBuckets];
    uint32_t *out = sorted + blob * (size_t)kMaxEntries;
    if constexpr (!staged) {
#pragma unroll
        for (int q = 0; q < kScalarsPerSortThread; q++) {
            uint32_t s[8];
            load_scalar(q, s);
            const uint32_t e = (uint32_t)(q * kSortThreads + tid);
            for_each_digit<0>(s, 0u, [&](int j, uint32_t b, uint32_t neg) {
                out[atomicAdd(&cnt[b], 1u)] = ((uint32_t)j * kBlobElems + e) | (neg ? kEntryNegBit : 0u);
            });
        }
        return;
    }
    constexpr uint32_t kEmpty = 0xffffffffu;
    for (uint32_t p = 0; p * kStageEntries < total; p++) {
        __syncthreads();
        for (int k = tid; k < kStageEntries + kHeavyThreshold; k += kSortThreads) stage[k] = kEmpty;
        __syncthreads();
#pragma unroll
        for (int q = 0; q < kScalarsPerSortThread; q++) {
            uint32_t s[8];
            load_scalar(q, s);
#pragma unroll
            for (int k = 0; k < 8; k++) asm volatile("" : "+v"(s[k]));
            const uint32_t e = (uint32_t)(q * kSortThreads + tid);
            for_each_digit<0>(s, 0u, [&](int j, uint32_t b, uint32_t neg) {
                const uint32_t start = bst[b], size = bst[b + 1] - start;
                const uint32_t entry = ((uint32_t)j * kBlobElems + e) | (neg ? kEntryNegBit : 0u);
                if (size > (uint32_t)kHeavyThreshold) {
                    if (p == 0) out[atomicAdd(&cnt[b], 1u)] = entry;
                } else if (start / kStageEntries == p) {
                    stage[atomicAdd(&cnt[b], 1u) - p * kStageEntries] = entry;
                }
            });
        }
        __syncthreads();
        for (uint32_t k = tid; k < (uint32_t)(kStageEntries + kHeavyThreshold); k += kSortThreads) {
            const uint32_t w = stage[k];
            if (w != kEmpty) out[p * kStageEntries + k] = w;
        }
    }
}

void launch_digit_sort(const uint32_t *scalars_raw, uint32_t *sorted, uint32_t *bucket_start, uint32_t *perm,
                       size_t n_blobs, hipStream_t st) {
    ProfScope p("k_digit_sort", st);
    const bool staged = knobs().sort_stage;
    if (staged)
        hipLaunchKernelGGL(k_digit_sort<true>, dim3((unsigned)n_blobs), dim3(kSortThreads), 0, st, (const uint4 *)scalars_raw, sorted, bucket_start, perm);
    else
        hipLaunchKernelGGL(k_digit_sort<false>, dim3((unsigned)n_blobs), dim3(kSortThreads), 0, st, (const uint4 *)scalars_raw, sorted, bucket_start, perm);
}


constexpr int kAccThreads = 256;

template <class PX>
__device__ __forceinline__ PX wave_shfl_down(const PX &v, int d) {
    PX r;
#pragma unroll
    for (int i = 0; i < 14; i++) {
        r.x.l[i] = __shfl_down(v.x.l[i], d, 64);
        r.y.l[i] = __shfl_down(v.y.l[i], d, 64);
        r.zz.l[i] = __shfl_down(v.zz.l[i], d, 64);
        r.zzz.l[i] = __shfl_down(v.zzz.l[i], d, 64);
    }
    return r;
}

constexpr int kHeavyBlocks = 2;
constexpr int kLightBlocks = kNumBuckets / kAccThreads;

__device__ __forceinline__ void bucket_heavy_blocks(const G1Affine29 *__restrict__ table, const uint32_t *__restrict__ ent,
                                                    const uint32_t *__restrict__ bs, const uint32_t *__restrict__ pm, uint32_t n_heavy,
                                                    G1Xyzz29 *__restrict__ out, uint32_t heavy_block) {
    const int lane = threadIdx.x & 63;
    const uint32_t wave = heavy_block * (kAccThreads / 64) + (threadIdx.x >> 6);
    for (uint32_t h = wave; h < n_heavy; h += kHeavyBlocks * (kAccThreads / 64)) {
        const uint32_t b = pm[h];
        const uint32_t begin = bs[b], end = bs[b + 1];
        G1Xyzz29 acc = G1Xyzz29::infinity();
        for (uint32_t k = begin + lane; k < end; k += 64) {
            uint32_t e = ent[k];
            G1Affine29 p = table[e & ~kEntryNegBit];
            acc = xyzz_madd(acc, p.x, cneg(p.y, (e & kEntryNegBit) != 0));
        }
        for (int d = 32; d >= 1; d >>= 1) {
            G1Xyzz29 other = wave_shfl_down(acc, d);
            if (lane < d) acc = xyzz_add(acc, other);
        }
        if (lane == 0) out[b] = acc;
    }
}

struct BucketBlock {
    size_t blob;
    uint32_t block;
    bool heavy;
};
__device__ __forceinline__ BucketBlock bucket_block() {
    if (blockIdx.x < (uint32_t)kHeavyBlocks) return {blockIdx.y, blockIdx.x, true};
    return {blockIdx.y, blockIdx.x - kHeavyBlocks, false};
}

__device__ __forceinline__ void bucket_light_lane(const G1Affine29 *__restrict__ table, const uint32_t *__restrict__ ent,
                                                  const uint32_t *__restrict__ bs, uint32_t b, G1Xyzz29 *__restrict__ out) {
    const uint32_t begin = bs[b], end = bs[b + 1];
    const G1Affine29i *tab = (const G1Affine29i *)table;
    G1Xyzz29i acc = G1Xyzz29i::infinity();
    if (begin < end) {
        uint32_t e = ent[begin];
        uint32_t e1 = begin + 1 < end ? ent[begin + 1] : e;
        G1Affine29i p = tab[e & ~kEntryNegBit];
        for (uint32_t k = begin; k < end; k++) {
            const auto qy = cneg(p.y, (e & kEntryNegBit) != 0);
            xyzz_madd_split(acc, p.x, qy, [&]() {
                e = e1;
                if (k + 1 < end) p = tab[e & ~kEntryNegBit];
                if (k + 2 < end) e1 = ent[k + 2];
            });
        }
    }
    ((G1Xyzz29i *)out)[b] = acc;
}

__global__ __launch_bounds__(kAccThreads) void k_bucket_accumulate(const G1Affine29 *__restrict__ table,
                                                                   const uint32_t *__restrict__ sorted,
                                                                   const uint32_t *__restrict__ bucket_start,
                                                                   const uint32_t *__restrict__ perm,
                                                                   G1Xyzz29 *__restrict__ buckets) {
    const BucketBlock bb = bucket_block();
    const size_t blob = bb.blob;
    const uint32_t *pm = perm + blob * (size_t)(kNumBuckets + 1);
    const uint32_t n_heavy = pm[kNumBuckets];
    const uint32_t *bs = bucket_start + blob * (size_t)(kNumBuckets + 1);
    const uint32_t *ent = sorted + blob * (size_t)kMaxEntries;
    G1Xyzz29 *out = buckets + blob * (size_t)kNumBuckets;
    if (bb.heavy) {
        bucket_heavy_blocks(table, ent, bs, pm, n_heavy, out, bb.block);
        return;
    }
    const uint32_t t = bb.block * kAccThreads + threadIdx.x;
    if (t < n_heavy) return;
    bucket_light_lane(table, ent, bs, pm[t], out);
}

__global__ __launch_bounds__(kAccThreads) void k_bucket_accumulate_asm(const G1Affine29 *__restrict__ table,
                                                                       const uint32_t *__restrict__ sorted,
                                                                       const uint32_t *__restrict__ bucket_start,
                                                                       const uint32_t *__restrict__ perm,
                                                                       G1Xyzz29 *__restrict__ buckets) {
#if defined(__HIP_DEVICE_COMPILE__)
    const BucketBlock bb = bucket_block();
    const size_t blob = bb.blob;
    const uint32_t *pm = perm + blob * (size_t)(kNumBuckets + 1);
    const uint32_t n_heavy = pm[kNumBuckets];
    const uint32_t *bs = bucket_start + blob * (size_t)(kNumBuckets + 1);
    const uint32_t *ent = sorted + blob * (size_t)kMaxEntries;
    G1Xyzz29 *out = buckets + blob * (size_t)kNumBuckets;
    if (bb.heavy) {
        bucket_heavy_blocks(table, ent, bs, pm, n_heavy, out, bb.block);
        return;
    }
    const uint32_t rank = bb.block * kAccThreads + threadIdx.x;
    uint32_t trouble;
    asm volatile(
#include "bucket_asm.inc"
        : "=&v"(trouble)
        : "s"(table), "s"(ent), "s"(bs), "s"(pm), "s"(out), "s"(n_heavy), "v"(rank)
        :
#include "bucket_asm_clobbers.inc"
    );
    if (trouble && rank >= n_heavy) bucket_light_lane(table, ent, bs, pm[rank], out);
#endif
}

static bool bucket_asm_enabled() {
    return knobs().bucket_asm;
}

// ... 119 lines not shown
```

Measured before the change: 109,100.

## Fuse lane fold and G1 compression into a commit tail kernel with batched redo pass

```diff
diff --git a/lambdaworks_kzg_amd/csrc/direct.hip b/lambdaworks_kzg_amd/csrc/direct.hip
--- a/lambdaworks_kzg_amd/csrc/direct.hip
+++ b/lambdaworks_kzg_amd/csrc/direct.hip
@@ -203,12 +203,9 @@
 }
 
 template <int CT>
-__global__ __launch_bounds__(kDirThreads) void k_direct_accumulate(const uint64_t *__restrict__ win_dev,
-                                                                   const uint4 *__restrict__ scalars,
-                                                                   G1Xyzz29 *__restrict__ partials, int scalars_per_lane,
-                                                                   DirectPlanRt rt, uint32_t row_bytes,
-                                                                   const uint32_t *__restrict__ redo) {
-    if (redo && !redo[blockIdx.y]) return;
+__device__ __forceinline__ void direct_accumulate_blob(const uint64_t *__restrict__ win_dev, const uint4 *__restrict__ scalars,
+                                                       G1Xyzz29 *__restrict__ partials, int scalars_per_lane, DirectPlanRt rt,
+                                                       uint32_t row_bytes, const size_t blob) {
     const DirectPlanRt P = CT ? PlanOf<CT ? CT : 16>::get() : rt;
     const int C = P.c;
     __shared__ uint32_t limbs[8 * kDirThreads];
@@ -217,7 +214,6 @@
     if (threadIdx.x < kDirectMaxWindows) win_base[threadIdx.x] = win_dev[threadIdx.x];
     __syncthreads();
     const int tid = threadIdx.x, lane = tid & 63, wave = tid >> 6;
-    const size_t blob = blockIdx.y;
     const int lanes_per_blob = gridDim.x * kDirThreads;
     const int first = blockIdx.x * kDirThreads + tid;
     const uint4 *sc = scalars + blob * (size_t)kBlobElems * 2;
@@ -283,6 +279,27 @@
     }
 }
 
+template <int CT>
+__global__ __launch_bounds__(kDirThreads) void k_direct_accumulate(const uint64_t *__restrict__ win_dev,
+                                                                   const uint4 *__restrict__ scalars,
+                                                                   G1Xyzz29 *__restrict__ partials, int scalars_per_lane,
+                                                                   DirectPlanRt rt, uint32_t row_bytes,
+                                                                   const uint32_t *__restrict__ redo) {
+    if (redo && !redo[blockIdx.y]) return;
+    direct_accumulate_blob<CT>(win_dev, scalars, partials, scalars_per_lane, rt, row_bytes, blockIdx.y);
+}
+
+template <int CT>
+__global__ __launch_bounds__(kDirThreads) void k_direct_second_pass(const uint64_t *__restrict__ win_dev, const uint4 *__restrict__ scalars,
+                                                                    G1Xyzz29 *__restrict__ sums, DirectPlanRt rt, uint32_t row_bytes,
+                                                                    const uint32_t *__restrict__ redo, uint32_t n_blobs) {
+    for (uint32_t blob = blockIdx.y; blob < n_blobs; blob += gridDim.y) {
+        if (!redo[blob]) continue;
+        direct_accumulate_blob<CT>(win_dev, scalars, sums, kBlobElems / kDirThreads, rt, row_bytes, blob);
+        __syncthreads();
+    }
+}
+
 constexpr int kLaneWords = 56;
 
 __global__ __launch_bounds__(kDirThreads) void k_direct_accumulate_asm(const uint64_t *__restrict__ win_dev,
@@ -344,14 +361,7 @@
     return acc;
 }
 
-__global__ __launch_bounds__(64) void k_direct_fold_lanes(const uint32_t *__restrict__ lane_out, G1Xyzz29 *__restrict__ partials,
-                                                          const uint32_t *__restrict__ redo, int lanes_per_block, int blocks_per_blob) {
-    const int unit = blockIdx.x;
-    if (redo[unit / blocks_per_blob]) return;
-    const int kFoldPerThread = lanes_per_block / 64;
-    __builtin_amdgcn_s_setprio(2);
-    const int lane = threadIdx.x;
-    const uint32_t *src = lane_out + ((size_t)unit * lanes_per_block + lane) * (size_t)kLaneWords;
+__device__ __forceinline__ FoldPoint fold_lane_sums(const uint32_t *src, int lane, int kFoldPerThread) {
     FoldPoint acc = load_lane_sum(src);
 #pragma unroll 1
     for (int step = 1; step < kFoldPerThread + 6; step++) {
@@ -372,6 +382,17 @@
         }
         if (take) acc = xyzz_add(acc, other);
     }
+    return acc;
+}
+
+__global__ __launch_bounds__(64) void k_direct_fold_lanes(const uint32_t *__restrict__ lane_out, G1Xyzz29 *__restrict__ partials,
+                                                          const uint32_t *__restrict__ redo, int lanes_per_block, int blocks_per_blob) {
+    const int unit = blockIdx.x;
+    if (redo[unit / blocks_per_blob]) return;
+    __builtin_amdgcn_s_setprio(2);
+    const int lane = threadIdx.x;
+    const uint32_t *src = lane_out + ((size_t)unit * lanes_per_block + lane) * (size_t)kLaneWords;
+    const FoldPoint acc = fold_lane_sums(src, lane, lanes_per_block / 64);
     if (lane == 0) partials[unit] = *(G1Xyzz29 *)&acc;
 }
 
@@ -410,6 +431,50 @@
         :
 #include "direct_fold_asm_clobbers_pad.inc"
     );
+#endif
+}
+
+template <bool ALONE>
+__global__ __launch_bounds__(64) void k_commit_tail(const uint32_t *__restrict__ lane_out, G1Xyzz29 *__restrict__ sums,
+                                                    uint32_t *__restrict__ redo, uint8_t *__restrict__ out48, int lanes_per_block) {
+#if defined(__HIP_DEVICE_COMPILE__)
+    const uint32_t blob = blockIdx.x;
+    uint32_t *flag = redo + blob;
+    G1Xyzz29 *out = sums + blob;
+    const uint32_t lane = threadIdx.x;
+    __builtin_amdgcn_s_setprio(2);
+    if (!*flag) {
+        const uint32_t *src = lane_out + (size_t)blob * lanes_per_block * kLaneWords;
+        const uint32_t per = lanes_per_block / 64, levels = 6;
+        if (ALONE) {
+            asm volatile(
+#include "direct_fold_asm.inc"
+                :
+                : "s"(src), "s"(out), "s"(flag), "s"(per), "v"(lane), "s"(levels)
+                :
+#include "direct_fold_asm_clobbers_pad.inc"
+            );
+        } else {
+            asm volatile(
+#include "direct_fold_asm.inc"
+                :
+                : "s"(src), "s"(out), "s"(flag), "s"(per), "v"(lane), "s"(levels)
+                :
+#include "direct_fold_asm_clobbers.inc"
+            );
+        }
+        if (__hip_atomic_load(flag, __ATOMIC_RELAXED, __HIP_MEMORY_SCOPE_AGENT)) {
+            const FoldPoint acc = fold_lane_sums(src + (size_t)lane * kLaneWords, (int)lane, (int)per);
+            if (lane == 0) *out = *(const G1Xyzz29 *)&acc;
+            __builtin_amdgcn_fence(__ATOMIC_RELEASE, "agent");
+        }
+    }
+    uint32_t w[12];
+    g1_compress_words(w, *out);
+    if (lane != 0) return;
+    uint32_t *o = (uint32_t *)(out48 + 48 * (size_t)blob);
+#pragma unroll
+    for (int k = 0; k < 12; k++) o[k] = w[k];
 #endif
 }
 
@@ -474,12 +539,13 @@
     return (nw + groups - 1) / groups;
 }
 
+constexpr int kRedoRows = 256;
 static bool direct_asm_enabled() { return knobs().direct_asm; }
 
 template <int CT>
-static void launch_direct_t(const DirectPlanRt &plan, const uint64_t *table, size_t row_bytes, const uint32_t *scalars_raw,
+static bool launch_direct_t(const DirectPlanRt &plan, const uint64_t *table, size_t row_bytes, const uint32_t *scalars_raw,
                             G1Xyzz29 *lane_scratch, G1Xyzz29 *partials, uint32_t *redo, G1Xyzz29 *sums, size_t n_blobs, hipStream_t st,
-                            int fill, uint32_t *redo_flag_out) {
+                            int fill, uint32_t *redo_flag_out, uint8_t *out48 = nullptr, bool redo_cleared = false) {
     const int kFillEnv = knobs().direct_fill;
     const int kFill = kFillEnv ? kFillEnv : fill ? fill : 512;
     CoopParams prm{};
@@ -508,7 +574,7 @@
             ProfScope p("k_coop_msm_asm", st);
             hipLaunchKernelGGL(k_coop_msm_asm, dim3(prm.n0 / 4, (unsigned)n_blobs), dim3(256), 0, st, table, (const uint4 *)scalars_raw,
                                (uint32_t *)lane_scratch, ctr, sums, redo_flag_out, prm);
-            return;
+            return false;
         }
         hipMemsetAsync(redo, 0, n_blobs * (1 + (size_t)counters) * sizeof(uint32_t), st);
         {
@@ -521,7 +587,7 @@
             hipLaunchKernelGGL(k_direct_accumulate<CT>, dim3(1, (unsigned)n_blobs, 1), dim3(kDirThreads), 0, st, table,
                                (const uint4 *)scalars_raw, sums, kBlobElems / kDirThreads, plan, (uint32_t)row_bytes, (const uint32_t *)redo);
         }
-        return;
+        return false;
     }
     int blocks_per_blob = 1, wsplit = 1;
     while (blocks_per_blob < 16 && n_blobs * blocks_per_blob < (size_t)kFill) blocks_per_blob <<= 1;
@@ -529,6 +595,30 @@
     const int scalars_per_lane = kBlobElems / (kDirThreads * blocks_per_blob);
     const int parts = blocks_per_blob * wsplit;
     G1Xyzz29 *dest = parts == 1 ? sums : partials;
+    if (out48 && direct_asm_enabled() && wsplit == 1 && blocks_per_blob == 1 && knobs().fold_asm && knobs().commit_tail) {
+        if (!redo_cleared) hipMemsetAsync(redo, 0, n_blobs * sizeof(uint32_t), st);
+        {
+            ProfScope p("k_direct_accumulate_asm", st);
+            hipLaunchKernelGGL(k_direct_accumulate_asm, dim3(1, (unsigned)n_blobs), dim3(kDirThreads), 0, st, table, (const uint4 *)scalars_raw,
+                               (uint32_t *)lane_scratch, redo, kBlobElems / kDirThreads, plan, (uint32_t)row_bytes);
+        }
+        {
+            ProfScope p("k_direct_redo", st);
+            const unsigned rows = n_blobs < (size_t)kRedoRows ? (unsigned)n_blobs : (unsigned)kRedoRows;
+            hipLaunchKernelGGL(k_direct_second_pass<CT>, dim3(1, rows, 1), dim3(kDirThreads), 0, st, table, (const uint4 *)scalars_raw, sums,
+                               plan, (uint32_t)row_bytes, (const uint32_t *)redo, (uint32_t)n_blobs);
+        }
+        {
+            ProfScope p("k_commit_tail", st);
+            if (n_blobs >= 1024 && !fill)
+                hipLaunchKernelGGL(k_commit_tail<true>, dim3((unsigned)n_blobs), dim3(64), 0, st, (const uint32_t *)lane_scratch, sums, redo, out48,
+                                   kDirThreads);
+            else
+                hipLaunchKernelGGL(k_commit_tail<false>, dim3((unsigned)n_blobs), dim3(64), 0, st, (const uint32_t *)lane_scratch, sums, redo, out48,
+                                   kDirThreads);
+        }
+        return true;
+    }
     if (direct_asm_enabled() && wsplit == 1) {
         const int threads = kDirThreads;
         hipMemsetAsync(redo, 0, n_blobs * sizeof(uint32_t), st);
@@ -568,18 +658,32 @@
         ProfScope p("k_direct_fold", st);
         hipLaunchKernelGGL(k_direct_fold, dim3((unsigned)n_blobs), dim3(64), 0, st, partials, sums, parts);
     }
+    return false;
+}
+
+
+static bool launch_direct_any(int bits, const uint64_t *table, size_t row_bytes, const uint32_t *scalars_raw, G1Xyzz29 *lane_scratch,
+                              G1Xyzz29 *partials, uint32_t *redo, G1Xyzz29 *sums, size_t n_blobs, hipStream_t st, int fill, uint32_t *redo_flag_out,
+                              uint8_t *out48, bool redo_cleared) {
+    const DirectPlanRt plan = make_plan(bits);
+    if (!plan.entries) return false;
+    switch (bits) {
+        case 14: return launch_direct_t<14>(plan, table, row_bytes, scalars_raw, lane_scratch, partials, redo, sums, n_blobs, st, fill, redo_flag_out, out48, redo_cleared);
+        case 15: return launch_direct_t<15>(plan, table, row_bytes, scalars_raw, lane_scratch, partials, redo, sums, n_blobs, st, fill, redo_flag_out, out48, redo_cleared);
+        case 16: return launch_direct_t<16>(plan, table, row_bytes, scalars_raw, lane_scratch, partials, redo, sums, n_blobs, st, fill, redo_flag_out, out48, redo_cleared);
+        default: return launch_direct_t<0>(plan, table, row_bytes, scalars_raw, lane_scratch, partials, redo, sums, n_blobs, st, fill, redo_flag_out, out48, redo_cleared);
+    }
 }
 
 void launch_direct_msm(int bits, const uint64_t *table, size_t row_bytes, const uint32_t *scalars_raw, G1Xyzz29 *lane_scratch,
                        G1Xyzz29 *partials, uint32_t *redo, G1Xyzz29 *sums, size_t n_blobs, hipStream_t st, int fill, uint32_t *redo_flag_out) {
-    const DirectPlanRt plan = make_plan(bits);
-    if (!plan.entries) return;
-    switch (bits) {
-        case 14: launch_direct_t<14>(plan, table, row_bytes, scalars_raw, lane_scratch, partials, redo, sums, n_blobs, st, fill, redo_flag_out); break;
-        case 15: launch_direct_t<15>(plan, table, row_bytes, scalars_raw, lane_scratch, partials, redo, sums, n_blobs, st, fill, redo_flag_out); break;
-        case 16: launch_direct_t<16>(plan, table, row_bytes, scalars_raw, lane_scratch, partials, redo, sums, n_blobs, st, fill, redo_flag_out); break;
-        default: launch_direct_t<0>(plan, table, row_bytes, scalars_raw, lane_scratch, partials, redo, sums, n_blobs, st, fill, redo_flag_out); break;
-    }
+    (void)launch_direct_any(bits, table, row_bytes, scalars_raw, lane_scratch, partials, redo, sums, n_blobs, st, fill, redo_flag_out, nullptr, false);
+}
+
+bool launch_direct_msm_compressed(int bits, const uint64_t *table, size_t row_bytes, const uint32_t *scalars_raw, G1Xyzz29 *lane_scratch,
+                                  G1Xyzz29 *partials, uint32_t *redo, G1Xyzz29 *sums, uint8_t *out48, size_t n_blobs, hipStream_t st, int fill,
+                                  bool redo_cleared) {
+    return launch_direct_any(bits, table, row_bytes, scalars_raw, lane_scratch, partials, redo, sums, n_blobs, st, fill, nullptr, out48, redo_cleared);
 }
 uint32_t direct_one_blob_counter_words(int bits) {
     const DirectPlanRt plan = make_plan(bits);
diff --git a/lambdaworks_kzg_amd/csrc/engine.h b/lambdaworks_kzg_amd/csrc/engine.h
--- a/lambdaworks_kzg_amd/csrc/engine.h
+++ b/lambdaworks_kzg_amd/csrc/engine.h
@@ -280,7 +280,7 @@
 void ensure_lagrange(Ctx *c, int mode);
 
 void msm_stages(Ctx *c, const uint32_t *scalars_raw, uint8_t *out48, size_t n, hipStream_t st, size_t base = 0, bool shared_chip = false,
-                bool lagrange = false);
+                bool lagrange = false, bool redo_cleared = false);
 bool coefficients_to_msm_form(Ctx *c, int mode, size_t n, hipStream_t st, size_t base = 0);
 
 C_KZG_RET commit_batch_device(Ctx *c, uint8_t *out48, const uint8_t *blobs, size_t n, int mode, hipStream_t st,
diff --git a/lambdaworks_kzg_amd/csrc/engine.hip b/lambdaworks_kzg_amd/csrc/engine.hip
--- a/lambdaworks_kzg_amd/csrc/engine.hip
+++ b/lambdaworks_kzg_amd/csrc/engine.hip
@@ -32,6 +32,7 @@
 struct ProfRec {
     const char *name;
     hipEvent_t e0, e1;
+    int dev;
 };
 static std::atomic<bool> g_prof_on{false};
 static std::mutex g_prof_mu;
@@ -42,9 +43,34 @@
 };
 static std::map<std::string, ProfAgg> g_prof_agg;
 
-ProfScope::ProfScope(const char *n, hipStream_t s) : name(n), st(s), e0(nullptr), e1(nullptr), on(g_prof_on.load(std::memory_order_relaxed)) {
+static std::map<int, std::vector<hipEvent_t>> g_prof_pool;
+
+static bool prof_event(hipEvent_t *e, int dev) {
+    {
+        std::lock_guard<std::mutex> lk(g_prof_mu);
+        auto &pool = g_prof_pool[dev];
+        if (!pool.empty()) {
+            *e = pool.back();
+            pool.pop_back();
+            return true;
+        }
+    }
+    return hipEventCreate(e) == hipSuccess;
+}
+
+static void prof_pool_free() {
+    std::lock_guard<std::mutex> lk(g_prof_mu);
+    for (auto &kv : g_prof_pool)
+        for (hipEvent_t e : kv.second) hipEventDestroy(e);
+    g_prof_pool.clear();
+}
+
+ProfScope::ProfScope(const char *n, hipStream_t s)
+    : name(n), st(s), e0(nullptr), e1(nullptr), dev(0), on(g_prof_on.load(std::memory_order_relaxed)) {
     if (!on) return;
-    if (hipEventCreate(&e0) != hipSuccess || hipEventCreate(&e1) != hipSuccess) {
+    if (hipGetDevice(&dev) != hipSuccess || !prof_event(&e0, dev) || !prof_event(&e1, dev)) {
+        if (e0) hipEventDestroy(e0);
+        e0 = nullptr;
         on = false;
         return;
     }
@@ -54,7 +80,7 @@
     if (!on) return;
     hipEventRecord(e1, st);
     std::lock_guard<std::mutex> lk(g_prof_mu);
-    g_prof_pending.push_back({name, e0, e1});
+    g_prof_pending.push_back({name, e0, e1, dev});
 }
 
 static void prof_drain() {
@@ -66,8 +92,9 @@
             a.launches++;
             a.total_ms += ms;
         }
-        hipEventDestroy(r.e0);
-        hipEventDestroy(r.e1);
+        auto &pool = g_prof_pool[r.dev];
+        pool.push_back(r.e0);
+        pool.push_back(r.e1);
     }
     g_prof_pending.clear();
 }
@@ -680,7 +707,18 @@
 }
 
 void msm_stages(Ctx *c, const uint32_t *scalars_raw, uint8_t *out48, size_t n, hipStream_t st, size_t base, bool shared_chip,
-                bool lagrange) {
+                bool lagrange, bool redo_cleared) {
+    Workspace &w = c->ws;
+    if (lagrange ? c->lag.direct_table : c->direct_table) {
+        G1Xyzz29 *sums = w.sums + base;
+        uint32_t *redo = w.bucket_start + base * (size_t)(kNumBuckets + 1);
+        if (!launch_direct_msm_compressed(lagrange ? c->lag.direct_bits : c->direct_bits, lagrange ? c->lag.direct_tab.win_dev : c->direct_tab.win_dev,
+                                          lagrange ? c->lag.direct_row_bytes : c->direct_row_bytes, scalars_raw, w.buckets + base * (size_t)kNumBuckets,
+                                          (G1Xyzz29 *)(w.sorted + base * (size_t)kMaxEntries), redo, sums, out48, n, st,
+                                          (shared_chip || peer_busy(c)) ? 2048 : 0, redo_cleared))
+            launch_finalize_compress(sums, out48, n, st);
+        return;
+    }
     launch_finalize_compress(msm_sums_stage(c, scalars_raw, n, st, base, shared_chip, lagrange), out48, n, st);
 }
 
@@ -761,11 +799,12 @@
 }
 
 static bool coefficients_stage(Ctx *c, const uint8_t *blobs, size_t n, int mode, int32_t *status, hipStream_t st,
-                               size_t base = 0, bool evaluations_ok = false, uint32_t *zero = nullptr, uint32_t zero_words = 0) {
+                               size_t base = 0, bool evaluations_ok = false, uint32_t *zero = nullptr, uint32_t zero_words = 0,
+                               uint32_t *zero2 = nullptr, uint32_t zero2_words = 0) {
     Workspace &w = c->ws;
     uint32_t *scalars = w.scalars + base * (size_t)kBlobElems * 8;
     if (mode == LWKZG_MODE_REFERENCE) {
-        launch_parse_be_reduce(blobs, scalars, n * kBlobElems, st, zero, zero_words);
+        launch_parse_be_reduce(blobs, scalars, n * kBlobElems, st, zero, zero_words, zero2, zero2_words);
     } else if (evaluations_ok ? commit_on_lagrange(c, mode) : proof_in_evaluation_form(c, mode)) {
         launch_copy_le_check(blobs, scalars, status, n, st);
         return true;
@@ -795,11 +834,15 @@
     for (size_t off = 0; off < n; off += kMaxChunk) {
         size_t m = n - off < kMaxChunk ? n - off : kMaxChunk;
         int32_t *stt = status ? status + off : c->ws.status;
-        LWK_HIP(hipMemsetAsync(stt, 0, m * 4, st));
-        const int ways = m >= 256 ? split_ways((commit_on_lagrange(c, mode) ? c->lag.direct_table : c->direct_table) != nullptr) : 1;
+        const bool direct = (commit_on_lagrange(c, mode) ? c->lag.direct_table : c->direct_table) != nullptr;
+        const int ways = m >= 256 ? split_ways(direct) : 1;
+        const bool parse_clears = ways == 1 && mode == LWKZG_MODE_REFERENCE && knobs().commit_tail;
+        if (!parse_clears) LWK_HIP(hipMemsetAsync(stt, 0, m * 4, st));
         if (ways == 1) {
-            const bool lg = coefficients_stage(c, blobs + off * (size_t)kBlobBytes, m, mode, stt, st, 0, true);
-            msm_stages(c, c->ws.scalars, out48 + 48 * off, m, st, 0, false, lg);
+            const bool redo_cleared = parse_clears && direct;
+            const bool lg = coefficients_stage(c, blobs + off * (size_t)kBlobBytes, m, mode, stt, st, 0, true, parse_clears ? (uint32_t *)stt : nullptr,
+                                               parse_clears ? (uint32_t)m : 0, redo_cleared ? c->ws.bucket_start : nullptr, redo_cleared ? (uint32_t)m : 0);
+            msm_stages(c, c->ws.scalars, out48 + 48 * off, m, st, 0, false, lg, redo_cleared);
             continue;
         }
         LWK_HIP(hipEventRecord(c->ev_fork, st));
@@ -1906,6 +1949,7 @@
 }
 void lwkzg_profile_reset(void) {
     prof_drain();
+    prof_pool_free();
     std::lock_guard<std::mutex> lk(g_prof_mu);
     g_prof_agg.clear();
 }
diff --git a/lambdaworks_kzg_amd/csrc/g1.cuh b/lambdaworks_kzg_amd/csrc/g1.cuh
--- a/lambdaworks_kzg_amd/csrc/g1.cuh
+++ b/lambdaworks_kzg_amd/csrc/g1.cuh
@@ -308,24 +308,49 @@
     return g1_in_subgroup_endo<G1Xyzz>(p.x, p.y, fe_from_raw<FpParams>(raw));
 }
 
-LWK_HD void g1_compress_affine(uint8_t out[48], const G1Affine &a) {
+LWK_HD void g1_compress_affine_words(uint32_t o[12], const G1Affine &a) {
     uint32_t rx[12], ry[12], ryn[12];
     fe_to_raw<FpParams>(rx, a.x);
     fe_to_raw<FpParams>(ry, a.y);
     fe_to_raw<FpParams>(ryn, neg(a.y));
-    raw_to_be<12>(out, rx);
-    out[0] |= 0x80;
-    if (!raw_geq<12>(ryn, ry)) out[0] |= 0x20;
+#pragma unroll
+    for (int k = 0; k < 12; k++) o[k] = __builtin_bswap32(rx[11 - k]);
+    o[0] |= 0x80u;
+    if (!raw_geq<12>(ryn, ry)) o[0] |= 0x20u;
+}
+
+template <class X>
+LWK_HD void g1_compress_words(uint32_t o[12], const X &p) {
+    if (p.is_inf()) {
+#pragma unroll
+        for (int k = 0; k < 12; k++) o[k] = 0;
+        o[0] = 0xc0u;
+        return;
+    }
+    g1_compress_affine_words(o, xyzz_to_affine(p));
+}
+
+LWK_HD void g1_words_to_bytes48(uint8_t out[48], const uint32_t o[12]) {
+#pragma unroll
+    for (int k = 0; k < 12; k++) {
+        out[4 * k] = (uint8_t)o[k];
+        out[4 * k + 1] = (uint8_t)(o[k] >> 8);
+        out[4 * k + 2] = (uint8_t)(o[k] >> 16);
+        out[4 * k + 3] = (uint8_t)(o[k] >> 24);
+    }
+}
+
+LWK_HD void g1_compress_affine(uint8_t out[48], const G1Affine &a) {
+    uint32_t o[12];
+    g1_compress_affine_words(o, a);
+    g1_words_to_bytes48(out, o);
 }
 
 template <class X>
 LWK_HD void g1_compress(uint8_t out[48], const X &p) {
-    if (p.is_inf()) {
-        for (int i = 0; i < 48; i++) out[i] = 0;
-        out[0] = 0xc0;
-        return;
-    }
-    g1_compress_affine(out, xyzz_to_affine(p));
+    uint32_t o[12];
+    g1_compress_words(o, p);
+    g1_words_to_bytes48(out, o);
 }
 
 LWK_HD int g1_decompress_nocheck(G1Affine &out, const uint8_t in[48]) {
diff --git a/lambdaworks_kzg_amd/csrc/kernels.h b/lambdaworks_kzg_amd/csrc/kernels.h
--- a/lambdaworks_kzg_amd/csrc/kernels.h
+++ b/lambdaworks_kzg_amd/csrc/kernels.h
@@ -13,10 +13,12 @@
     const char *name;
     hipStream_t st;
     hipEvent_t e0, e1;
+    int dev;
     bool on;
 };
 
-void launch_parse_be_reduce(const uint8_t *blobs, uint32_t *scalars_raw, size_t n_elems, hipStream_t st, uint32_t *zero = nullptr, uint32_t zero_words = 0);
+void launch_parse_be_reduce(const uint8_t *blobs, uint32_t *scalars_raw, size_t n_elems, hipStream_t st, uint32_t *zero = nullptr, uint32_t zero_words = 0,
+                            uint32_t *zero2 = nullptr, uint32_t zero2_words = 0);
 
 void launch_digit_sort(const uint32_t *scalars_raw, uint32_t *sorted, uint32_t *bucket_start, uint32_t *perm,
                        size_t n_blobs, hipStream_t st);
@@ -44,6 +46,9 @@
 void launch_direct_msm(int bits, const uint64_t *win_dev, size_t row_bytes, const uint32_t *scalars_raw, G1Xyzz29 *lane_scratch,
                        G1Xyzz29 *partials, uint32_t *redo, G1Xyzz29 *sums, size_t n_blobs, hipStream_t st, int fill = 0,
                        uint32_t *redo_flag_out = nullptr);
+bool launch_direct_msm_compressed(int bits, const uint64_t *win_dev, size_t row_bytes, const uint32_t *scalars_raw, G1Xyzz29 *lane_scratch,
+                                  G1Xyzz29 *partials, uint32_t *redo, G1Xyzz29 *sums, uint8_t *out48, size_t n_blobs, hipStream_t st,
+                                  int fill = 0, bool redo_cleared = false);
 uint32_t direct_one_blob_counter_words(int bits);
 void launch_direct_msm_only(int bits, const uint64_t *win_dev, size_t row_bytes, const uint32_t *scalars_raw, G1Xyzz29 *sums,
                             const uint32_t *only_if, size_t n_blobs, hipStream_t st);
diff --git a/lambdaworks_kzg_amd/csrc/knobs.h b/lambdaworks_kzg_amd/csrc/knobs.h
--- a/lambdaworks_kzg_amd/csrc/knobs.h
+++ b/lambdaworks_kzg_amd/csrc/knobs.h
@@ -22,6 +22,7 @@
 
     bool direct_asm = true;
     bool fold_asm = true;
+    bool commit_tail = true;
     bool bucket_asm = true;
     int direct_fill = 0;
     int coop = 1;
diff --git a/lambdaworks_kzg_amd/csrc/knobs.hip b/lambdaworks_kzg_amd/csrc/knobs.hip
--- a/lambdaworks_kzg_amd/csrc/knobs.hip
+++ b/lambdaworks_kzg_amd/csrc/knobs.hip
@@ -66,6 +66,7 @@
 
     r.flag(k.direct_asm, "LWKZG_DIRECT_ASM", EXP);
     r.flag(k.fold_asm, "LWKZG_FOLD_ASM", EXP);
+    r.flag(k.commit_tail, "LWKZG_COMMIT_TAIL", EXP);
     r.flag(k.bucket_asm, "LWKZG_BUCKET_ASM", EXP);
     r.num(k.direct_fill, "LWKZG_DIRECT_FILL", EXP);
     r.num(k.coop, "LWKZG_COOP", EXP);
@@ -134,7 +135,7 @@
 }
 
 const char *knob_names_experimental() {
-    return "LWKZG_DIRECT_ASM LWKZG_FOLD_ASM LWKZG_BUCKET_ASM LWKZG_DIRECT_FILL LWKZG_COOP LWKZG_COOP_MAX LWKZG_COOP_RPQ LWKZG_SORT_STAGE "
+    return "LWKZG_DIRECT_ASM LWKZG_FOLD_ASM LWKZG_COMMIT_TAIL LWKZG_BUCKET_ASM LWKZG_DIRECT_FILL LWKZG_COOP LWKZG_COOP_MAX LWKZG_COOP_RPQ LWKZG_SORT_STAGE "
            "LWKZG_REDUCE_LANES LWKZG_HASH_PAIRS LWKZG_HASH_PRIO LWKZG_VALIDATE_COOP LWKZG_VALIDATE_LDS_PAD LWKZG_CKZG_EVAL_PROOFS "
            "LWKZG_MID_PROOF_PIPE LWKZG_MID_PROOF_PIPE_MIN LWKZG_MID_PROOF_PARTS LWKZG_MID_PROOF_CHUNKS LWKZG_HEAVY_SERIAL LWKZG_PROOF_SCHEDULE LWKZG_SPLIT "
            "LWKZG_SLICE0 LWKZG_SET_MODE_IN_PLACE LWKZG_PAIRING_GENERIC_SQR LWKZG_PAIRING_NAIVE LWKZG_PAIRING_NO_PRECOMP "
@@ -151,13 +152,13 @@
         tmp, sizeof tmp,
         "{\"experimental\": %s, \"mode\": %d, \"direct_bits\": %s%d, \"direct_row\": %d, \"coalesce\": %d, \"twin\": %d, "
         "\"small_proof_host\": %zu, \"mid_proof_host\": %zu, \"host_threads\": %d, \"host_warm_ms\": %d, \"host_finish\": %zu, "
-        "\"timing\": %d, \"verbose\": %d, \"direct_asm\": %d, \"fold_asm\": %d, \"bucket_asm\": %d, \"coop\": %d, \"coop_max\": %d, "
+        "\"timing\": %d, \"verbose\": %d, \"direct_asm\": %d, \"fold_asm\": %d, \"commit_tail\": %d, \"bucket_asm\": %d, \"coop\": %d, \"coop_max\": %d, "
         "\"hash_pairs\": %d, \"hash_prio\": %d, \"validate_coop\": %d, \"ckzg_eval_proofs\": %d, \"mid_proof_pipe\": %d, "
         "\"verify_msm\": %d, \"verify_fused\": %d, \"verify_pad_kb\": [%d, %d, %d], \"verify_order\": %d, \"vmsm_list_cap\": %d, "
         "\"host_stage\": %d, \"operational\": \"%s\", \"experimental_names\": \"%s\"}",
         k.experimental ? "true" : "false", k.mode, k.has_direct_bits ? "" : "null, \"direct_bits_unset_default\": ", k.direct_bits, k.direct_row,
         (int)k.coalesce, (int)k.twin, k.small_proof_host, k.mid_proof_host, k.host_threads, k.host_warm_ms, k.host_finish, (int)k.timing,
-        (int)k.verbose, (int)k.direct_asm, (int)k.fold_asm, (int)k.bucket_asm, k.coop, k.coop_max, (int)k.hash_pairs, k.hash_prio,
+        (int)k.verbose, (int)k.direct_asm, (int)k.fold_asm, (int)k.commit_tail, (int)k.bucket_asm, k.coop, k.coop_max, (int)k.hash_pairs, k.hash_prio,
         (int)k.validate_coop, (int)k.ckzg_eval_proofs, (int)k.mid_proof_pipe, k.verify_msm, k.verify_fused, k.verify_pad_kb[0],
         k.verify_pad_kb[1], k.verify_pad_kb[2], k.verify_order, k.vmsm_list_cap, (int)k.host_stage, lwk::knob_names_operational(),
         lwk::knob_names_experimental());
diff --git a/lambdaworks_kzg_amd/csrc/msm.hip b/lambdaworks_kzg_amd/csrc/msm.hip
--- a/lambdaworks_kzg_amd/csrc/msm.hip
+++ b/lambdaworks_kzg_amd/csrc/msm.hip
@@ -9,9 +9,11 @@
 __device__ __forceinline__ uint32_t bswap32(uint32_t v) { return __builtin_bswap32(v); }
 
 __global__ __launch_bounds__(256) void k_parse_be_reduce(const uint4 *__restrict__ in, uint4 *__restrict__ out,
-                                                         size_t n_elems, uint32_t *__restrict__ zero, uint32_t zero_words) {
+                                                         size_t n_elems, uint32_t *__restrict__ zero, uint32_t zero_words,
+                                                         uint32_t *__restrict__ zero2, uint32_t zero2_words) {
     size_t i = (size_t)blockIdx.x * blockDim.x + threadIdx.x;
     if (i < zero_words) zero[i] = 0u;
+    if (i < zero2_words) zero2[i] = 0u;
     if (i >= n_elems) return;
     uint4 hi = in[2 * i], lo = in[2 * i + 1];
     uint32_t s[8];
@@ -34,11 +36,13 @@
     out[2 * i + 1] = make_uint4(s[4], s[5], s[6], s[7]);
 }
 
-void launch_parse_be_reduce(const uint8_t *blobs, uint32_t *scalars_raw, size_t n_elems, hipStream_t st, uint32_t *zero, uint32_t zero_words) {
+void launch_parse_be_reduce(const uint8_t *blobs, uint32_t *scalars_raw, size_t n_elems, hipStream_t st, uint32_t *zero, uint32_t zero_words,
+                            uint32_t *zero2, uint32_t zero2_words) {
     ProfScope p("k_parse_be_reduce", st);
     unsigned grid = (unsigned)((n_elems + 255) / 256);
     hipLaunchKernelGGL(k_parse_be_reduce, dim3(grid), dim3(256), 0, st, (const uint4 *)blobs, (uint4 *)scalars_raw,
-                       n_elems, zero, zero_words < n_elems ? zero_words : (uint32_t)n_elems);
+                       n_elems, zero, zero_words < n_elems ? zero_words : (uint32_t)n_elems, zero2,
+                       zero2_words < n_elems ? zero2_words : (uint32_t)n_elems);
 }
 
 
```

Measured after the change: 111,500, median of 6. +2.2%, better.
